# Nikronic/ndr

Hardware: AMD Instinct MI355X
Metric: matrix-free SpMV GVoxel/s (Q1 fp64, 512x512x512); CG-MG iterations/s reported in cg_mg (higher is better)
Workload: dtype f64; 1 GPU; K(rho) u on a 512x512x512 voxel grid, trilinear hexahedra, fp64, seeded U[0,1] densities (SIMP p=3, Emin=1e-4), u ~ N(0,1); parallelism=1 GPU

## Files before the change

### __graft_entry__.py

```python
import os
import subprocess
import sys

ROOT = os.path.dirname(os.path.abspath(__file__))
if ROOT not in sys.path:
    sys.path.insert(0, ROOT)


def build():
    csrc = os.path.join(ROOT, "ndr_amd", "csrc")
    subprocess.check_call(["make", "-C", csrc, "-j4"])
    for src, kernels in (("kernels_q2", ["k_apply_q2_marchILi0"]),
                         ("kernels_l1_merged", ["k_l1_mergedILi0E", "k_l1_mergedILi1E", "k_l1_mergedILi2E", "k_l1_pair_rowsILi0E", "k_l1_pair_rowsILi1E"]),
                         ("kernels_gs_march", ["k_gs_march_mf0ILi%dELi%dELi%dEEE" % (a, f, m) for a in (0, 1) for f in (0, 1) for m in (0, 1)])):
        asm = os.path.join(csrc, src + ".isa.s")
        subprocess.check_call(["/opt/rocm/bin/hipcc", "-O3", "-std=c++17", "-fPIC", "--offload-arch=gfx950", "-ffp-contract=on",
                               "-S", "--cuda-device-only", "-o", asm, os.path.join(csrc, src + ".hip")],
                              stderr=subprocess.DEVNULL)
        for k in kernels:
            subprocess.check_call([sys.executable, os.path.join(ROOT, "tools", "check_sload_pipeline.py"), asm, k])
    from oracle import vfem_oracle
    vfem_oracle.build_lib()
    from ndr_amd import _lib
    lib = _lib.load()
    assert lib.vfem_version() >= 100
    import ndr_amd


def smoke():
    import numpy as np
    sys.path.insert(0, os.path.join(ROOT, "tests"))
    from helpers import BC_CANTILEVER, make_hip, make_oracle, seeded_density
    from oracle import vfem_oracle as vo
    ne, dom = (32, 16, 16), ([0, 0, 0], [2, 1, 1])
    rho = seeded_density(ne, 88, "proxy")
    t = make_hip(ne, dom, BC_CANTILEVER, rho)
    o = make_oracle(ne, dom, BC_CANTILEVER, rho)
    u = np.random.default_rng(0).standard_normal((o.num_nodes, 3))
    err = np.abs(t.applyK(u) - o.apply_k(u)).max() / np.abs(o.apply_k(u)).max()
    assert err < 1e-11, err
    f = o.build_load_vector()
    mg = t.multigridSolver(2)
    ug = mg.preconditionedConjugateGradient(np.zeros_like(f), f, 100, 1e-6, None, 1, 2, True)
    omg = vo.OracleMG(o, 2, nthreads=4)
    uo = omg.pcg(np.zeros_like(f), f, 100, 1e-6, 1, 2, True)
    cg, co = float(np.sum(f * ug)), float(np.sum(f * uo))
    assert abs(cg - co) < 1e-8 * abs(co), (cg, co)
    assert mg.last_iterations == omg.last_iters
    print("smoke ok: apply err %.2e, compliance %.9f (oracle %.9f), %d PCG iterations" % (err, cg, co, mg.last_iterations))


if __name__ == "__main__":
    build()
    if len(sys.argv) > 1 and sys.argv[1] == "smoke":
        smoke()
```

### include/vfem.h

```cpp
#ifndef VFEM_H
#define VFEM_H

#include <stddef.h>
#include <stdint.h>

#ifdef __cplusplus
extern "C" {
#endif

typedef struct vfem_sim vfem_sim;
typedef struct vfem_mg  vfem_mg;
typedef struct vfem_mlp vfem_mlp;
typedef struct vfem_gsim vfem_gsim;
typedef struct vfem_hom_mg vfem_hom_mg;
typedef struct vfem_gmg vfem_gmg;

const char *vfem_last_error(void);
int  vfem_device_count(void);
int  vfem_set_device(int device);
int  vfem_version(void);

enum {
    VFEM_OPT_APPLY_PLANES = 0,
    VFEM_OPT_GS_VARIANT   = 2,
    VFEM_OPT_APPLY_IMPL   = 4,
    VFEM_OPT_Q2_IMPL      = 6,
    VFEM_OPT_DMA_CHUNKS   = 7,
    VFEM_OPT_DMA_STRIP    = 9,
    VFEM_OPT_DMA_LX       = 11,
    VFEM_OPT_GS_PAIR      = 10,
    VFEM_OPT_L1_DIAG      = 12,
    VFEM_OPT_GS_RESIDENT  = 13,
    VFEM_OPT_L1_SPLIT     = 15,
    VFEM_OPT_STENCIL_SPLIT = 18,
    VFEM_OPT_GS_MARCH     = 19,
    VFEM_OPT_GS_MARCH_CHUNKS = 20,
    VFEM_OPT_L1_STORED    = 21,
    VFEM_OPT_L1_MERGED    = 22,
    VFEM_OPT_Q2_GS_IMPL   = 16,
    VFEM_OPT_TRANSFER_AXIS = 17,
    VFEM_OPT_Q2_L1_VIRTUAL = 14
};

int vfem_malloc(void **ptr, size_t bytes);
int vfem_free(void *ptr);
int vfem_copy_h2d(void *dst, const void *src_host, size_t bytes, void *stream);
int vfem_copy_d2h(void *dst_host, const void *src, size_t bytes, void *stream);
int vfem_copy_d2d(void *dst, const void *src, size_t bytes, void *stream);
int vfem_memset(void *dst, int value, size_t bytes, void *stream);
int vfem_stream_sync(void *stream);

int vfem_sim_create(vfem_sim **out, const double bbox_min_host[3], const double bbox_max_host[3],
                    const int64_t nelems_host[3]);
int vfem_sim_destroy(vfem_sim *sim);
int64_t vfem_sim_num_nodes(const vfem_sim *sim);
int64_t vfem_sim_num_elements(const vfem_sim *sim);

int vfem_sim_set_isotropic(vfem_sim *sim, double young, double poisson);
int vfem_sim_set_elasticity_tensor(vfem_sim *sim, const double D_host[36]);
enum {
    VFEM_PATH_MODE_SPACE    = 1,
    VFEM_PATH_GS_RESIDENT   = 2,
    VFEM_PATH_K0_MIRROR     = 4,
    VFEM_PATH_L1_MIRROR     = 8,
    VFEM_PATH_Q2_MODE_SPACE = 16
};
int vfem_sim_tensor_paths(const vfem_sim *sim);
int vfem_sim_set_simp(vfem_sim *sim, double E0, double Emin, double gamma);
int vfem_sim_set_option(vfem_sim *sim, int key, int value);
int vfem_sim_k0(const vfem_sim *sim, double *K0_host);

int vfem_sim_set_dirichlet(vfem_sim *sim, const uint8_t *mask_host, const double *values_host);
int vfem_sim_set_loads(vfem_sim *sim, const double *f, void *stream);
int vfem_sim_build_load_vector(const vfem_sim *sim, double *f, void *stream);

int vfem_sim_set_densities(vfem_sim *sim, const double *rho, void *stream);
int vfem_sim_set_uniform_density(vfem_sim *sim, double rho, void *stream);
int vfem_sim_get_densities(const vfem_sim *sim, double *rho, void *stream);

int vfem_sim_apply_k(const vfem_sim *sim, const double *u, double *out, int variant, void *stream);
int vfem_sim_apply_k_planes(const vfem_sim *sim, const double *u, double *out, int64_t plane_lo, int64_t plane_hi, void *stream);
int vfem_sim_compliance_gradient(const vfem_sim *sim, const double *u, double *g, void *stream);
int vfem_compliance(const vfem_sim *sim, const double *f, const double *u, double *value_host, void *stream);

int vfem_mg_create(vfem_mg **out, vfem_sim *fine, int num_coarsening_levels);
int vfem_mg_destroy(vfem_mg *mg);

typedef struct {
    int64_t nx;
    int64_t elem_extra_lo;
    int64_t elem_extra_hi;
    int64_t xshift;
    int32_t xparity;
} vfem_slab_level;
int vfem_sim_create_padded(vfem_sim **out, const double bbox_min_host[3], const double bbox_max_host[3], const int64_t nelems_host[3],
                           int64_t extra_lo, int64_t extra_hi);
int64_t vfem_sim_num_stored_elements(const vfem_sim *sim);
int vfem_mg_create_slab(vfem_mg **out, vfem_sim *fine_local, int n_levels, const vfem_slab_level *levels_host,
                        const uint8_t *const *masks_host);
int vfem_mg_create_partial(vfem_mg **out, vfem_sim *fine, int num_coarsening_levels, int first_active_level);
int vfem_mg_smooth_colors(vfem_mg *mg, int level, double *u, const double *b, int forward, int first, int count, void *stream);
int vfem_mg_can_smooth_planes(vfem_mg *mg, int level);
int vfem_mg_smooth_group_planes(vfem_mg *mg, int level, double *u, const double *b, int forward, int group, int64_t plane_lo, int64_t plane_hi,
                                void *stream);
int vfem_mg_cycle_from_level(vfem_mg *mg, int level, double *x, const double *b, int num_smoothing_steps, int fmg, void *stream);
int vfem_mg_num_levels(const vfem_mg *mg);
int vfem_mg_level_dims(const vfem_mg *mg, int level, int64_t nelems_host[3]);
int64_t vfem_mg_level_num_nodes(const vfem_mg *mg, int level);
int vfem_mg_level_dirichlet_mask(const vfem_mg *mg, int level, uint8_t *mask_host);
int vfem_mg_set_symmetric_gauss_seidel(vfem_mg *mg, int symmetric);
int vfem_mg_tensor_paths(const vfem_mg *mg);
const double *vfem_mg_field_ptr(const vfem_mg *mg, int which, int level);

int vfem_mg_update_operators(vfem_mg *mg, void *stream);
int vfem_mg_export_level_ke(vfem_mg *mg, int level, int64_t child_first_layer, int64_t count_x, double *ke_out, void *stream);
int vfem_mg_import_level_ke(vfem_mg *mg, int level, const double *ke, void *stream);
int vfem_mg_apply_k(vfem_mg *mg, int level, const double *u, double *out, void *stream);
int vfem_mg_residual(vfem_mg *mg, int level, const double *u, const double *b, double *r, void *stream);
int vfem_mg_smooth(vfem_mg *mg, int level, double *u, const double *b, int forward, void *stream);
int vfem_mg_smooth_sweeps(vfem_mg *mg, int level, double *u, const double *b, int forward, int sweeps, void *stream);
int vfem_mg_zero_dirichlet(vfem_mg *mg, int level, double *u, void *stream);
int vfem_mg_restrict(vfem_mg *mg, int fine_level, const double *fine, double *coarse, void *stream);
int vfem_mg_interpolate(vfem_mg *mg, int fine_level, const double *coarse, double *fine, int accumulate, void *stream);
int vfem_mg_coarsest_solve(vfem_mg *mg, const double *b, double *x, void *stream);
enum { VFEM_COARSEST_AUTO = 0, VFEM_COARSEST_DENSE = 1, VFEM_COARSEST_PLANES = 2 };
int vfem_mg_set_coarsest_solver(vfem_mg *mg, int mode);
int64_t vfem_mg_coarsest_bytes(const vfem_mg *mg);
int vfem_dense_spd_inverse(int64_t n, double *A, void *stream);

int vfem_band_spd_factor(int64_t n, int64_t w, double *band, void *stream);
int vfem_band_spd_solve(int64_t n, int64_t w, const double *factor, double *x, int64_t nrhs, void *stream);
int vfem_sim_direct_solve(vfem_sim *sim, const double *f, double *u, void *stream);
int64_t vfem_sim_direct_factorizations(const vfem_sim *sim);
int64_t vfem_sim_direct_band_bytes(const vfem_sim *sim);
int vfem_gsim_direct_solve(vfem_gsim *sim, const double *f, double *u, void *stream);
int64_t vfem_gsim_direct_factorizations(const vfem_gsim *sim);
int64_t vfem_gsim_direct_band_bytes(const vfem_gsim *sim);

int vfem_mg_solve(vfem_mg *mg, double *x, const double *f, int num_steps, int num_smoothing_steps,
                  int stiffness_updated, int zero_dirichlet, int fmg, void *stream);

typedef void (*vfem_residual_cb)(void *user, int iteration, double residual_norm);
int vfem_mg_pcg(vfem_mg *mg, double *x, const double *b, int max_iter, double tol,
                int mg_iterations, int mg_smoothing_iterations, int fmg,
                vfem_residual_cb residual_cb, void *cb_user,
                int *iterations_out_host, double *relres_out_host, void *stream);

typedef struct {
    int64_t n_planes, plane_nodes;
    int64_t first_owned, last_owned;
    int64_t xoffn;
    int32_t gl, gr;
    double *x, *b, *r;
} vfem_dist_level;
typedef int (*vfem_halo_fn)(void *user, int level, double *field, int left, int right, int phase);
typedef int (*vfem_allreduce_fn)(void *user, double *device_buffer, int64_t n);
int vfem_mg_pcg_slab(vfem_mg *local, vfem_mg *replicated, int first_replicated_level, const vfem_dist_level *levels_host, int rank,
                     int world, double *replicated_x, double *replicated_b, double *x, const double *b, double *work_d, double *work_Ad,
                     double *scalars8, int max_iter, double tol, int mg_iterations, int mg_smoothing_iterations, int full_multigrid,
                     int overlap_sweeps, vfem_halo_fn halo, vfem_allreduce_fn allreduce, void *callback_user,
                     vfem_residual_cb residual_cb, void *residual_user, int *iterations_out, double *relres_out, void *stream);

int vfem_gsim_create(vfem_gsim **out, int dim, int degree, const double *bbox_min_host, const double *bbox_max_host,
                     const int64_t *nelems_host);
int vfem_gsim_create_padded(vfem_gsim **out, int dim, int degree, const double *bbox_min_host, const double *bbox_max_host,
                            const int64_t *nelems_host, int64_t elem_extra_lo, int64_t elem_extra_hi);
int64_t vfem_gsim_num_stored_elements(const vfem_gsim *sim);
int vfem_gsim_destroy(vfem_gsim *sim);
int64_t vfem_gsim_num_nodes(const vfem_gsim *sim);
int64_t vfem_gsim_num_elements(const vfem_gsim *sim);
int vfem_gsim_ke_size(const vfem_gsim *sim);
int vfem_gsim_set_isotropic(vfem_gsim *sim, double young, double poisson);
int vfem_gsim_set_elasticity_tensor(vfem_gsim *sim, const double *D_host, int n);
int vfem_gsim_tensor_paths(const vfem_gsim *sim);
int vfem_gsim_set_simp(vfem_gsim *sim, double E0, double Emin, double gamma);
int vfem_gsim_k0(const vfem_gsim *sim, double *K0_host);
int vfem_gsim_set_dirichlet(vfem_gsim *sim, const uint8_t *mask_host, const double *values_host);
int vfem_gsim_set_densities(vfem_gsim *sim, const double *rho, void *stream);
int vfem_gsim_get_densities(const vfem_gsim *sim, double *rho, void *stream);
int vfem_gsim_set_option(vfem_gsim *sim, int key, int value);
int vfem_gsim_apply_k(const vfem_gsim *sim, const double *u, double *out, void *stream);
int vfem_gsim_compliance_gradient(const vfem_gsim *sim, const double *u, double *g, void *stream);
int vfem_gsim_compliance(const vfem_gsim *sim, const double *f, const double *u, double *value_host, void *stream);
int vfem_gmg_create(vfem_gmg **out, vfem_gsim *fine, int num_coarsening_levels);
int vfem_gmg_create_slab(vfem_gmg **out, vfem_gsim *fine_local, int n_levels, const vfem_slab_level *levels_host,
                         const uint8_t *const *masks_host);
int vfem_gmg_create_partial(vfem_gmg **out, vfem_gsim *fine, int num_coarsening_levels, int first_active_level);
int vfem_gmg_smooth_colors(vfem_gmg *mg, int level, double *u, const double *b, int forward, int first, int count, void *stream);
int vfem_gmg_cycle_from_level(vfem_gmg *mg, int level, double *x, const double *b, int num_smoothing_steps, int fmg, void *stream);
int vfem_gmg_export_level_ke(vfem_gmg *mg, int level, int64_t child_first_layer, int64_t count_x, double *ke_out, void *stream);
int vfem_gmg_import_level_ke(vfem_gmg *mg, int level, const double *ke, void *stream);
int vfem_gmg_destroy(vfem_gmg *mg);
int vfem_gmg_num_levels(const vfem_gmg *mg);
int vfem_gmg_level_dims(const vfem_gmg *mg, int level, int64_t nelems_host[3]);
int64_t vfem_gmg_level_num_nodes(const vfem_gmg *mg, int level);
int vfem_gmg_level_dirichlet_mask(const vfem_gmg *mg, int level, uint8_t *mask_host);
int vfem_gmg_set_symmetric_gauss_seidel(vfem_gmg *mg, int symmetric);
int vfem_gmg_update_operators(vfem_gmg *mg, void *stream);
int vfem_gmg_apply_k(vfem_gmg *mg, int level, const double *u, double *out, void *stream);
int vfem_gmg_residual(vfem_gmg *mg, int level, const double *u, const double *b, double *r, void *stream);
int vfem_gmg_smooth(vfem_gmg *mg, int level, double *u, const double *b, int forward, void *stream);
int vfem_gmg_zero_dirichlet(vfem_gmg *mg, int level, double *u, void *stream);
int vfem_gmg_restrict(vfem_gmg *mg, int fine_level, const double *fine, double *coarse, void *stream);
// ... 79 lines not shown
```

### ndr_amd/_lib.py

```python
import ctypes
import os
from ctypes import POINTER, c_char_p, c_double, c_float, c_int, c_int64, c_size_t, c_void_p

_HERE = os.path.dirname(os.path.abspath(__file__))
LIB_PATH = os.environ.get("VFEM_LIB") or os.path.join(_HERE, "csrc", "libvfem.so")
_lib = None

RESIDUAL_CB = ctypes.CFUNCTYPE(None, c_void_p, c_int, c_double)


class _SL(ctypes.Structure):
    _fields_ = [("nx", c_int64), ("elem_extra_lo", c_int64), ("elem_extra_hi", c_int64), ("xshift", c_int64), ("xparity", ctypes.c_int32)]


class _DL(ctypes.Structure):
    _fields_ = [("n_planes", c_int64), ("plane_nodes", c_int64), ("first_owned", c_int64), ("last_owned", c_int64), ("xoffn", c_int64),
                ("gl", ctypes.c_int32), ("gr", ctypes.c_int32), ("x", c_void_p), ("b", c_void_p), ("r", c_void_p)]

_HOM = [c_int, POINTER(c_int64), POINTER(c_double), POINTER(c_double), POINTER(c_double), c_double, c_void_p]

SIGNATURES = {
    "vfem_last_error": (c_char_p, []),
    "vfem_device_count": (c_int, []),
    "vfem_set_device": (c_int, [c_int]),
    "vfem_version": (c_int, []),
    "vfem_malloc": (c_int, [POINTER(c_void_p), c_size_t]),
    "vfem_free": (c_int, [c_void_p]),
    "vfem_copy_h2d": (c_int, [c_void_p, c_void_p, c_size_t, c_void_p]),
    "vfem_copy_d2h": (c_int, [c_void_p, c_void_p, c_size_t, c_void_p]),
    "vfem_copy_d2d": (c_int, [c_void_p, c_void_p, c_size_t, c_void_p]),
    "vfem_memset": (c_int, [c_void_p, c_int, c_size_t, c_void_p]),
    "vfem_stream_sync": (c_int, [c_void_p]),
    "vfem_sim_create": (c_int, [POINTER(c_void_p), POINTER(c_double), POINTER(c_double), POINTER(c_int64)]),
    "vfem_sim_destroy": (c_int, [c_void_p]),
    "vfem_sim_num_nodes": (c_int64, [c_void_p]),
    "vfem_sim_num_elements": (c_int64, [c_void_p]),
    "vfem_sim_set_isotropic": (c_int, [c_void_p, c_double, c_double]),
    "vfem_sim_set_elasticity_tensor": (c_int, [c_void_p, c_void_p]),
    "vfem_sim_tensor_paths": (c_int, [c_void_p]),
    "vfem_sim_set_simp": (c_int, [c_void_p, c_double, c_double, c_double]),
    "vfem_sim_set_option": (c_int, [c_void_p, c_int, c_int]),
    "vfem_sim_k0": (c_int, [c_void_p, c_void_p]),
    "vfem_sim_set_dirichlet": (c_int, [c_void_p, c_void_p, c_void_p]),
    "vfem_sim_set_loads": (c_int, [c_void_p, c_void_p, c_void_p]),
    "vfem_sim_build_load_vector": (c_int, [c_void_p, c_void_p, c_void_p]),
    "vfem_sim_set_densities": (c_int, [c_void_p, c_void_p, c_void_p]),
    "vfem_sim_set_uniform_density": (c_int, [c_void_p, c_double, c_void_p]),
    "vfem_sim_get_densities": (c_int, [c_void_p, c_void_p, c_void_p]),
    "vfem_sim_apply_k": (c_int, [c_void_p, c_void_p, c_void_p, c_int, c_void_p]),
    "vfem_sim_apply_k_planes": (c_int, [c_void_p, c_void_p, c_void_p, c_int64, c_int64, c_void_p]),
    "vfem_sim_compliance_gradient": (c_int, [c_void_p, c_void_p, c_void_p, c_void_p]),
    "vfem_compliance": (c_int, [c_void_p, c_void_p, c_void_p, POINTER(c_double), c_void_p]),
    "vfem_mg_create": (c_int, [POINTER(c_void_p), c_void_p, c_int]),
    "vfem_mg_destroy": (c_int, [c_void_p]),
    "vfem_sim_create_padded": (c_int, [POINTER(c_void_p), POINTER(c_double), POINTER(c_double), POINTER(c_int64), c_int64, c_int64]),
    "vfem_sim_num_stored_elements": (c_int64, [c_void_p]),
    "vfem_mg_create_slab": (c_int, [POINTER(c_void_p), c_void_p, c_int, c_void_p, POINTER(c_void_p)]),
    "vfem_mg_create_partial": (c_int, [POINTER(c_void_p), c_void_p, c_int, c_int]),
    "vfem_mg_smooth_colors": (c_int, [c_void_p, c_int, c_void_p, c_void_p, c_int, c_int, c_int, c_void_p]),
    "vfem_mg_can_smooth_planes": (c_int, [c_void_p, c_int]),
    "vfem_mg_smooth_group_planes": (c_int, [c_void_p, c_int, c_void_p, c_void_p, c_int, c_int, c_int64, c_int64, c_void_p]),
    "vfem_mg_cycle_from_level": (c_int, [c_void_p, c_int, c_void_p, c_void_p, c_int, c_int, c_void_p]),
    "vfem_mg_num_levels": (c_int, [c_void_p]),
    "vfem_mg_level_dims": (c_int, [c_void_p, c_int, POINTER(c_int64)]),
    "vfem_mg_level_num_nodes": (c_int64, [c_void_p, c_int]),
    "vfem_mg_level_dirichlet_mask": (c_int, [c_void_p, c_int, c_void_p]),
    "vfem_mg_set_symmetric_gauss_seidel": (c_int, [c_void_p, c_int]),
    "vfem_mg_tensor_paths": (c_int, [c_void_p]),
    "vfem_mg_field_ptr": (c_void_p, [c_void_p, c_int, c_int]),
    "vfem_mg_update_operators": (c_int, [c_void_p, c_void_p]),
    "vfem_mg_export_level_ke": (c_int, [c_void_p, c_int, c_int64, c_int64, c_void_p, c_void_p]),
    "vfem_mg_import_level_ke": (c_int, [c_void_p, c_int, c_void_p, c_void_p]),
    "vfem_mg_apply_k": (c_int, [c_void_p, c_int, c_void_p, c_void_p, c_void_p]),
    "vfem_mg_residual": (c_int, [c_void_p, c_int, c_void_p, c_void_p, c_void_p, c_void_p]),
    "vfem_mg_smooth": (c_int, [c_void_p, c_int, c_void_p, c_void_p, c_int, c_void_p]),
    "vfem_mg_smooth_sweeps": (c_int, [c_void_p, c_int, c_void_p, c_void_p, c_int, c_int, c_void_p]),
    "vfem_mg_zero_dirichlet": (c_int, [c_void_p, c_int, c_void_p, c_void_p]),
    "vfem_mg_restrict": (c_int, [c_void_p, c_int, c_void_p, c_void_p, c_void_p]),
    "vfem_mg_interpolate": (c_int, [c_void_p, c_int, c_void_p, c_void_p, c_int, c_void_p]),
    "vfem_mg_coarsest_solve": (c_int, [c_void_p, c_void_p, c_void_p, c_void_p]),
    "vfem_mg_set_coarsest_solver": (c_int, [c_void_p, c_int]),
    "vfem_mg_coarsest_bytes": (c_int64, [c_void_p]),
    "vfem_dense_spd_inverse": (c_int, [c_int64, c_void_p, c_void_p]),
    "vfem_band_spd_factor": (c_int, [c_int64, c_int64, c_void_p, c_void_p]),
    "vfem_band_spd_solve": (c_int, [c_int64, c_int64, c_void_p, c_void_p, c_int64, c_void_p]),
    "vfem_sim_direct_solve": (c_int, [c_void_p, c_void_p, c_void_p, c_void_p]),
    "vfem_sim_direct_factorizations": (c_int64, [c_void_p]),
    "vfem_sim_direct_band_bytes": (c_int64, [c_void_p]),
    "vfem_gsim_direct_solve": (c_int, [c_void_p, c_void_p, c_void_p, c_void_p]),
    "vfem_gsim_direct_factorizations": (c_int64, [c_void_p]),
    "vfem_gsim_direct_band_bytes": (c_int64, [c_void_p]),
    "vfem_mg_solve": (c_int, [c_void_p, c_void_p, c_void_p, c_int, c_int, c_int, c_int, c_int, c_void_p]),
    "vfem_mg_pcg": (c_int, [c_void_p, c_void_p, c_void_p, c_int, c_double, c_int, c_int, c_int,
                            RESIDUAL_CB, c_void_p, POINTER(c_int), POINTER(c_double), c_void_p]),
    "vfem_mlp_forward_grid_range": (c_int, [c_void_p, POINTER(c_int64), POINTER(c_double), POINTER(c_double), c_int64, c_int64,
                                            c_void_p, c_void_p, c_void_p]),
    "vfem_mlp_forward_grid_range_f32": (c_int, [c_void_p, POINTER(c_int64), POINTER(c_double), POINTER(c_double), c_int64, c_int64,
                                                c_void_p, c_void_p, c_void_p]),
    "vfem_mlp_backward": (c_int, [c_void_p, c_void_p, c_int64, c_void_p, c_float, c_void_p, c_void_p, c_void_p, c_void_p, c_void_p, c_void_p]),
    "vfem_mlp_backward_grid": (c_int, [c_void_p, POINTER(c_int64), POINTER(c_double), POINTER(c_double), c_void_p, c_float,
                                       c_void_p, c_void_p, c_void_p, c_void_p, c_void_p, c_void_p]),
    "vfem_mlp_backward_grid_range": (c_int, [c_void_p, POINTER(c_int64), POINTER(c_double), POINTER(c_double), c_int64, c_int64, c_void_p,
                                             c_float, c_void_p, c_void_p, c_void_p, c_void_p, c_void_p, c_void_p]),
    "vfem_adam_step": (c_int, [c_int64, c_void_p, c_void_p, c_void_p, c_void_p, c_float, c_float, c_float, c_float, c_int, c_void_p]),
    "vfem_gsim_create": (c_int, [POINTER(c_void_p), c_int, c_int, POINTER(c_double), POINTER(c_double), POINTER(c_int64)]),
    "vfem_gsim_create_padded": (c_int, [POINTER(c_void_p), c_int, c_int, POINTER(c_double), POINTER(c_double), POINTER(c_int64),
                                        c_int64, c_int64]),
    "vfem_gsim_num_stored_elements": (c_int64, [c_void_p]),
    "vfem_gmg_create_slab": (c_int, [POINTER(c_void_p), c_void_p, c_int, c_void_p, POINTER(c_void_p)]),
    "vfem_gmg_create_partial": (c_int, [POINTER(c_void_p), c_void_p, c_int, c_int]),
    "vfem_gmg_smooth_colors": (c_int, [c_void_p, c_int, c_void_p, c_void_p, c_int, c_int, c_int, c_void_p]),
    "vfem_gmg_cycle_from_level": (c_int, [c_void_p, c_int, c_void_p, c_void_p, c_int, c_int, c_void_p]),
    "vfem_gmg_export_level_ke": (c_int, [c_void_p, c_int, c_int64, c_int64, c_void_p, c_void_p]),
    "vfem_gmg_import_level_ke": (c_int, [c_void_p, c_int, c_void_p, c_void_p]),
    "vfem_gsim_destroy": (c_int, [c_void_p]),
    "vfem_gsim_num_nodes": (c_int64, [c_void_p]),
    "vfem_gsim_num_elements": (c_int64, [c_void_p]),
    "vfem_gsim_ke_size": (c_int, [c_void_p]),
    "vfem_gsim_set_isotropic": (c_int, [c_void_p, c_double, c_double]),
    "vfem_gsim_set_elasticity_tensor": (c_int, [c_void_p, c_void_p, c_int]),
    "vfem_gsim_tensor_paths": (c_int, [c_void_p]),
    "vfem_gsim_set_simp": (c_int, [c_void_p, c_double, c_double, c_double]),
    "vfem_gsim_k0": (c_int, [c_void_p, c_void_p]),
    "vfem_gsim_set_dirichlet": (c_int, [c_void_p, c_void_p, c_void_p]),
    "vfem_gsim_set_densities": (c_int, [c_void_p, c_void_p, c_void_p]),
    "vfem_gsim_get_densities": (c_int, [c_void_p, c_void_p, c_void_p]),
    "vfem_gsim_set_option": (c_int, [c_void_p, c_int, c_int]),
    "vfem_gsim_apply_k": (c_int, [c_void_p, c_void_p, c_void_p, c_void_p]),
    "vfem_gsim_compliance_gradient": (c_int, [c_void_p, c_void_p, c_void_p, c_void_p]),
    "vfem_gsim_compliance": (c_int, [c_void_p, c_void_p, c_void_p, POINTER(c_double), c_void_p]),
    "vfem_gmg_create": (c_int, [POINTER(c_void_p), c_void_p, c_int]),
    "vfem_gmg_destroy": (c_int, [c_void_p]),
    "vfem_gmg_num_levels": (c_int, [c_void_p]),
    "vfem_gmg_level_dims": (c_int, [c_void_p, c_int, POINTER(c_int64)]),
    "vfem_gmg_level_num_nodes": (c_int64, [c_void_p, c_int]),
    "vfem_gmg_level_dirichlet_mask": (c_int, [c_void_p, c_int, c_void_p]),
    "vfem_gmg_set_symmetric_gauss_seidel": (c_int, [c_void_p, c_int]),
    "vfem_gmg_update_operators": (c_int, [c_void_p, c_void_p]),
    "vfem_gmg_apply_k": (c_int, [c_void_p, c_int, c_void_p, c_void_p, c_void_p]),
    "vfem_gmg_residual": (c_int, [c_void_p, c_int, c_void_p, c_void_p, c_void_p, c_void_p]),
    "vfem_gmg_smooth": (c_int, [c_void_p, c_int, c_void_p, c_void_p, c_int, c_void_p]),
    "vfem_gmg_zero_dirichlet": (c_int, [c_void_p, c_int, c_void_p, c_void_p]),
    "vfem_gmg_restrict": (c_int, [c_void_p, c_int, c_void_p, c_void_p, c_void_p]),
    "vfem_gmg_interpolate": (c_int, [c_void_p, c_int, c_void_p, c_void_p, c_int, c_void_p]),
    "vfem_gmg_solve": (c_int, [c_void_p, c_void_p, c_void_p, c_int, c_int, c_int, c_int, c_int, c_void_p]),
    "vfem_gmg_pcg": (c_int, [c_void_p, c_void_p, c_void_p, c_int, c_double, c_int, c_int, c_int, RESIDUAL_CB, c_void_p,
                             POINTER(c_int), POINTER(c_double), c_void_p]),
    "vfem_box_filter": (c_int, [POINTER(c_int64), c_int, c_void_p, c_void_p, c_int, c_void_p]),
    "vfem_box_filter_slab": (c_int, [POINTER(c_int64), c_int64, c_int64, c_int64, c_int64, c_int, c_void_p, c_void_p, c_int,
                                     c_void_p]),
    "vfem_projection": (c_int, [c_int64, c_double, c_void_p, c_void_p, c_void_p]),
    "vfem_projection_backprop": (c_int, [c_int64, c_double, c_void_p, c_void_p, c_void_p, c_void_p]),
    "vfem_oc_candidate": (c_int, [c_int64, c_void_p, c_void_p, c_void_p, c_double, c_double, c_void_p, c_void_p]),
    "vfem_mean": (c_int, [c_int64, c_void_p, POINTER(c_double), c_void_p]),
    "vfem_langelaar_apply": (c_int, [POINTER(c_int64), c_double, c_double, c_double, c_void_p, c_void_p, c_void_p, c_void_p]),
    "vfem_langelaar_backprop": (c_int, [POINTER(c_int64), c_double, c_double, c_double, c_void_p, c_void_p, c_void_p, c_void_p,
                                        c_void_p, c_void_p, c_void_p]),
    "vfem_mg_pcg_slab": (c_int, [c_void_p, c_void_p, c_int, c_void_p, c_int, c_int, c_void_p, c_void_p, c_void_p, c_void_p, c_void_p, c_void_p,
                                 c_void_p, c_int, c_double, c_int, c_int, c_int, c_int, c_void_p, c_void_p, c_void_p, RESIDUAL_CB, c_void_p,
# ... 66 lines not shown
```

### ndr_amd/csrc/coef_rows.h

```cpp
#pragma once
#include "device_utils.h"
#include "l1_merged_core.h"

namespace vfem {

template <int OFF>
__device__ __forceinline__ void srow_issue(const double *p, d8_t &a, double &b) {
    asm volatile("s_load_dwordx16 %0, %2, %3\n\ts_load_dwordx2 %1, %2, %4" : "=&s"(a), "=&s"(b) : "s"(p), "n"(OFF), "n"(OFF + 64));
}
__device__ __forceinline__ void srow_wait(d8_t &a, double &b) { asm volatile("s_waitcnt lgkmcnt(0)" : "+s"(a), "+s"(b)); }
__device__ __forceinline__ void srow_wait(d8_t &a, double &b, double &tie) { asm volatile("s_waitcnt lgkmcnt(0)" : "+s"(a), "+s"(b), "+v"(tie)); }

template <bool MID> constexpr int row_pos(int w) { return MID ? (w == 3 ? 0 : w == 2 ? 1 : w == 0 ? 2 : 3) : 7 - w; }
template <bool MID> constexpr int row_kind(int pos) { return MID ? (pos == 0 ? 3 : pos == 1 ? 2 : pos == 2 ? 0 : 1) : 7 - pos; }

template <int NROWS, class SEQ>
struct RowPipe {
    const double *tab;
    d8_t a0, a1;
    double b0, b1;
    __device__ __forceinline__ void prime() { srow_issue<SEQ::at(0)>(tab, a0, b0); }
    template <int R>
    __device__ __forceinline__ void take(double c[9], double &tie) {
        static_assert(R >= 0 && R < NROWS, "row outside the sequence");
        if constexpr (R % 2 == 0) {
            srow_wait(a0, b0, tie);
            if constexpr (R + 1 < NROWS) srow_issue<SEQ::at(R + 1 < NROWS ? R + 1 : 0)>(tab, a1, b1);
            c[0] = a0[0]; c[1] = a0[1]; c[2] = a0[2]; c[3] = a0[3]; c[4] = a0[4]; c[5] = a0[5]; c[6] = a0[6]; c[7] = a0[7]; c[8] = b0;
        } else {
            srow_wait(a1, b1, tie);
            if constexpr (R + 1 < NROWS) srow_issue<SEQ::at(R + 1 < NROWS ? R + 1 : 0)>(tab, a0, b0);
            c[0] = a1[0]; c[1] = a1[1]; c[2] = a1[2]; c[3] = a1[3]; c[4] = a1[4]; c[5] = a1[5]; c[6] = a1[6]; c[7] = a1[7]; c[8] = b1;
        }
    }
    template <int R>
    __device__ __forceinline__ void take(double c[9]) {
        static_assert(R >= 0 && R < NROWS, "row outside the sequence");
        if constexpr (R % 2 == 0) {
            srow_wait(a0, b0);
            if constexpr (R + 1 < NROWS) srow_issue<SEQ::at(R + 1 < NROWS ? R + 1 : 0)>(tab, a1, b1);
            c[0] = a0[0]; c[1] = a0[1]; c[2] = a0[2]; c[3] = a0[3]; c[4] = a0[4]; c[5] = a0[5]; c[6] = a0[6]; c[7] = a0[7]; c[8] = b0;
        } else {
            srow_wait(a1, b1);
            if constexpr (R + 1 < NROWS) srow_issue<SEQ::at(R + 1 < NROWS ? R + 1 : 0)>(tab, a0, b0);
            c[0] = a1[0]; c[1] = a1[1]; c[2] = a1[2]; c[3] = a1[3]; c[4] = a1[4]; c[5] = a1[5]; c[6] = a1[6]; c[7] = a1[7]; c[8] = b1;
        }
    }
};

template <bool MID>
struct L1PartRows { static constexpr int at(int r) { return ((r / 4) * 8 + row_kind<MID>(r % 4)) * l1m::TAB_ROW * 8; } };
template <bool MID>
struct DevCoef {
    RowPipe<32, L1PartRows<MID>> pipe;
    __device__ __forceinline__ explicit DevCoef(const double *tab) : pipe{tab} {}
    __device__ __forceinline__ void prime() { pipe.prime(); }
    template <int G, int W>
    __device__ __forceinline__ void get(double c[9]) { pipe.template take<G * 4 + row_pos<MID>(W)>(c); }
};

struct L0NodeRows {
    static constexpr int at(int r) { return (r < 4 ? 7 - r : r < 8 ? row_kind<true>(r - 4) : 7 - (r - 8)) * l1m::TAB_ROW * 8; }
};
template <bool MID, int BASE, class Hook>
struct L0Coef {
    RowPipe<12, L0NodeRows> &pipe;
    double &tie;
    Hook after_first;
    template <int G, int W>
    __device__ __forceinline__ void get(double c[9]) {
        static_assert(G == 0, "level 0 has one class");
        pipe.template take<BASE + row_pos<MID>(W)>(c, tie);
        after_first(std::integral_constant<int, row_pos<MID>(W)>{});
    }
};
template <bool MID, int BASE, class Hook>
__device__ __forceinline__ L0Coef<MID, BASE, Hook> l0_coef(RowPipe<12, L0NodeRows> &pipe, double &tie, Hook hook) { return L0Coef<MID, BASE, Hook>{pipe, tie, hook}; }


}
```

### ndr_amd/csrc/generic.hip

```cpp
#include "mg_cycle.h"
#include "device_utils.h"
#include "q2_modes.h"
#include "gs_colors.h"

#include <algorithm>
#include <cmath>
#include <cstring>
#include <memory>

namespace vfem {

struct GDims {
    int N, p;
    int ne[3], nn[3];
    int npe, ke;
    long long nnodes, nelems;
};

static GDims make_gdims(int N, int p, const long long *ne) {
    GDims d{};
    d.N = N; d.p = p; d.npe = 1; d.nnodes = 1; d.nelems = 1;
    for (int a = 0; a < 3; ++a) {
        d.ne[a] = a < N ? (int) ne[a] : 1;
        d.nn[a] = a < N ? p * d.ne[a] + 1 : 1;
// ... 841 lines not shown
        throw Error("the element matrices of the first active level have not been imported (vfem_gmg_import_level_ke)");
    const int l_first = mg->first_active > 0 ? mg->first_active + 1 : 1;
    const int l_last = mg->slab ? mg->L - 1 : mg->L;
    mg->l1_virtual = N == 3 && sim->d.p == 2 && mg->first_active == 0 && mg->external_ke_level != 0 && mg->L >= 2 &&
                     (sim->q2_l1_virtual == 1 ||
                      (sim->q2_l1_virtual == 2 && (double) stored_dims(mg, 1).nelems * 81 * 81 * sizeof(double) > 1.5e9));
    if (mg->l1_virtual) mg->lv[1].Ke.release();
    for (int l = l_first; l <= l_last; ++l) {
        GLevel &lv = mg->lv[l];
        const size_t kk = (size_t) lv.d.ke * lv.d.ke;
        const GDims cd = stored_dims(mg, l), fd = stored_dims(mg, l - 1);
        if (fd.ne[0] != 2 * cd.ne[0]) throw Error("stored element layers of consecutive levels must halve exactly");
        if (mg->l1_virtual && l == 1) continue;
        lv.Ke.alloc((size_t) cd.nelems * kk);
        if (mg->l1_virtual && l == 2) { coarsen_through_virtual_level1(mg, 0, cd.ne[0], lv.Ke.p, s); continue; }
        const bool from_moduli = l == 1 && mg->external_ke_level != 0;
        g_coarsen(mg, fd, cd, from_moduli, from_moduli ? sim->E.p : mg->lv[l - 1].Ke.p, lv.Ke.p, s);
    }
    if (mg->slab) { mg->operators_valid = true; return; }
    GLevel &cl = mg->lv[mg->L];
    const GDims &d = cl.d;
    const long long n = (long long) N * d.nnodes;
    if (mg->L > 0) mg->coarsest.refuse_if_too_large(n, nullptr);
    else if (n > DENSE_COARSEST_MAX_DOFS) {
        mg->coarsest.release();
        mg->operators_valid = true;
        return;
    }
    const size_t kk = (size_t) d.ke * d.ke;
    std::vector<double> Ke((size_t) d.nelems * kk);
    if (mg->L == 0 && mg->external_ke_level != 0) {
        std::vector<double> E((size_t) d.nelems);
        VFEM_HIP(hipMemcpyAsync(E.data(), sim->E_local(), E.size() * sizeof(double), hipMemcpyDeviceToHost, s));
        VFEM_HIP(hipStreamSynchronize(s));
        for (long long e = 0; e < d.nelems; ++e)
            for (size_t q = 0; q < kk; ++q) Ke[e * kk + q] = E[e] * sim->K0[q];
    } else {
        VFEM_HIP(hipMemcpyAsync(Ke.data(), cl.Ke_local(), Ke.size() * sizeof(double), hipMemcpyDeviceToHost, s));
        VFEM_HIP(hipStreamSynchronize(s));
    }
    std::vector<double> A((size_t) n * n, 0.0);
    const int q1 = d.p + 1;
    std::vector<long long> dofs(d.ke);
    for (long long e = 0; e < d.nelems; ++e) {
        int eb[3] = {0, 0, 0};
        { long long m = e; for (int a = N - 1; a >= 0; --a) { eb[a] = d.p * (int) (m % d.ne[a]); m /= d.ne[a]; } }
        for (int ln = 0; ln < d.npe; ++ln) {
            int m = ln, g[3] = {0, 0, 0};
            for (int a = N - 1; a >= 0; --a) { g[a] = eb[a] + m % q1; m /= q1; }
            long long node = g[0];
            for (int a = 1; a < N; ++a) node = node * d.nn[a] + g[a];
            for (int c = 0; c < N; ++c) dofs[N * ln + c] = N * node + c;
        }
        for (int i = 0; i < d.ke; ++i)
            for (int j = 0; j < d.ke; ++j) A[(size_t) dofs[i] * n + dofs[j]] += Ke[e * kk + (size_t) i * d.ke + j];
    }
    for (long long r = 0; r < n; ++r)
        if ((cl.hmask[r / N] >> (r % N)) & 1) {
            for (long long c = 0; c < n; ++c) { A[(size_t) r * n + c] = 0.0; A[(size_t) c * n + r] = 0.0; }
            A[(size_t) r * n + r] = 1.0;
        }
    double *Adev = mg->coarsest.dense_matrix(n, s);
    VFEM_HIP(hipStreamSynchronize(s));
    VFEM_HIP(hipMemcpy(Adev, A.data(), A.size() * sizeof(double), hipMemcpyHostToDevice));
    mg->coarsest.factor_dense(N, cl.mask.p, s);
    VFEM_HIP(hipStreamSynchronize(s));
    mg->operators_valid = true;
}

namespace {
struct GenericOps {
    vfem_gmg *mg;
    hipStream_t s;
    GLevel &lv(int l) const { return mg->lv[l]; }

    int last_level() const { return mg->L; }
    void last_level_cycle(bool) { mg->coarsest.solve(b(mg->L), x(mg->L), s); }
    bool symmetric() const { return mg->symmetric_gs; }
    double *x(int l) const { return lv(l).x.p; }
    double *b(int l) const { return lv(l).b.p; }
    void enforce_dirichlet(int l, bool residual_system, bool) {
        g_dirichlet(lv(l).d, lv(l).mask.p, (l == 0 && !residual_system) ? mg->fine->dvals.p : nullptr, x(l), s);
    }
    void smooth(int l, int forward, int n) { for (int i = 0; i < n; ++i) gmg_smooth(mg, l, x(l), b(l), forward, s); }
    void residual(int l) { gmg_apply(mg, l, x(l), b(l), 1, lv(l).r.p, s); }
    void restrict_residual(int l) { gmg_restrict(mg, l, lv(l).r.p, b(l + 1), s); lv(l + 1).x.zero(s); }
    void restrict_rhs(int l) { gmg_restrict(mg, l, b(l), b(l + 1), s); }
    void prolong_correction(int l) { gmg_prolong(mg, l, x(l + 1), x(l), 1, s); }
    bool prolong_start(int l, bool) { gmg_prolong(mg, l, x(l + 1), x(l), 0, s); return false; }

    long long n_dofs() const { return (long long) lv(0).d.N * lv(0).d.nnodes; }
    mg_cycle::CgWork cg() const { return {n_dofs(), mg->pd.p, mg->pAd.p, mg->scal.p, s}; }
    double *s_vector(bool preconditioned) const { return preconditioned ? x(0) : mg->ps.p; }
    void dot(const double *a, const double *b, double *out) { launch_dot(n_dofs(), a, b, mg->scratch.p, out, s); }
    void initial_residual(const double *x, const double *b, double *r) { gmg_apply(mg, 0, x, b, 1, r, s); }
    void shift_and_dot_rs(const double *r, double *sv, double *sc) {
        g_dirichlet(lv(0).d, lv(0).mask.p, nullptr, sv, s);
        launch_shift_scalar(sc, s);
        dot(r, sv, sc + 0);
    }
    void apply_dot(const double *d, double *Ad, double *out) { gmg_apply(mg, 0, d, nullptr, 2, Ad, s); dot(d, Ad, out); }
    void step_dot(double *x, double *r, const double *d, const double *Ad, double *sc) { launch_pcg_step(n_dofs(), x, r, d, Ad, sc, s); dot(r, r, sc + 3); }
};
}

extern "C" {

int vfem_gsim_create_padded(vfem_gsim **out, int dim, int degree, const double *bbmin, const double *bbmax, const int64_t *ne,
                            int64_t ex_lo, int64_t ex_hi) {
    VFEM_TRY
    if (dim != 2 && dim != 3) throw Error("dimension must be 2 or 3");
    if (degree != 1 && degree != 2) throw Error("No template instantiation matching degreesPerDimension!");
    long long n[3] = {1, 1, 1};
    for (int a = 0; a < dim; ++a) {
        if (ne[a] < 1 || ne[a] > 4096) throw Error("elements per dimension must be in [1, 4096]");
        n[a] = ne[a];
    }
    std::unique_ptr<vfem_gsim> sim(new vfem_gsim);
    sim->d = make_gdims(dim, degree, n);
    for (int a = 0; a < dim; ++a) {
        sim->h[a] = (bbmax[a] - bbmin[a]) / (double) ne[a];
        if (!(sim->h[a] > 0)) throw Error("empty domain bounding box");
    }
    sim->update_k0();
    if (ex_lo < 0 || ex_hi < 0 || ((ex_lo || ex_hi) && dim != 3)) throw Error("element padding needs a 3-D grid and non-negative layer counts");
    sim->ex_lo = ex_lo; sim->ex_hi = ex_hi;
    sim->rho.alloc((size_t) sim->stored_elems()); sim->rho.zero(nullptr);
    sim->E.alloc((size_t) sim->stored_elems());
    sim->update_E(nullptr);
    sim->hmask.assign((size_t) sim->d.nnodes, 0);
    sim->dmask.alloc((size_t) sim->d.nnodes); sim->dmask.zero(nullptr);
    sim->dvals.alloc((size_t) sim->d.nnodes * dim); sim->dvals.zero(nullptr);
    VFEM_HIP(hipDeviceSynchronize());
    *out = sim.release();
    VFEM_CATCH
}
int vfem_gsim_create(vfem_gsim **out, int dim, int degree, const double *bbmin, const double *bbmax, const int64_t *ne) {
    return vfem_gsim_create_padded(out, dim, degree, bbmin, bbmax, ne, 0, 0);
}
int vfem_gsim_destroy(vfem_gsim *sim) { VFEM_TRY delete sim; VFEM_CATCH }
int64_t vfem_gsim_num_stored_elements(const vfem_gsim *sim) { return sim->stored_elems(); }
int64_t vfem_gsim_num_nodes(const vfem_gsim *sim) { return sim->d.nnodes; }
int64_t vfem_gsim_num_elements(const vfem_gsim *sim) { return sim->d.nelems; }
int vfem_gsim_ke_size(const vfem_gsim *sim) { return sim->d.ke; }
int vfem_gsim_set_isotropic(vfem_gsim *sim, double young, double poisson) {
    VFEM_TRY
    sim->lambda = sim->d.N == 2 ? poisson * young / (1.0 - poisson * poisson)
                                : poisson * young / ((1.0 + poisson) * (1.0 - 2.0 * poisson));
    sim->mu = young / (2.0 + 2.0 * poisson);
    sim->general_tensor = false;
    sim->update_k0();
    ++sim->operator_version;
    VFEM_CATCH
}
int vfem_gsim_set_elasticity_tensor(vfem_gsim *sim, const double *D, int n) {
    VFEM_TRY
    if (n != (sim->d.N == 3 ? 6 : 3)) throw Error("the flattened tensor of a " + std::to_string(sim->d.N) + "-D simulator is " +
                                                  (sim->d.N == 3 ? "6 x 6" : "3 x 3"));
    check_flattened_tensor(D, n);
    for (int i = 0; i < n; ++i)
        for (int j = 0; j < n; ++j) sim->D[i * n + j] = 0.5 * (D[i * n + j] + D[j * n + i]);
    sim->general_tensor = true;
    sim->update_k0();
    ++sim->operator_version;
    VFEM_CATCH
}
int vfem_gsim_tensor_paths(const vfem_gsim *sim) { return sim->q2_fast ? VFEM_PATH_Q2_MODE_SPACE : 0; }
// ... 327 lines not shown
```

### ndr_amd/csrc/gs_colors.h

```cpp
#pragma once
#include <type_traits>

namespace vfem {

struct GsColor { int start[3], inc[3], cnt[3]; };

template <class F>
void for_each_gs_color(int N, int p, const int nn[3], int forward, int first, int count, F &&f) {
    int ncol = 1;
    for (int a = 0; a < N; ++a) ncol *= p + 1;
    for (int i = first; i < first + count && i < ncol; ++i) {
        int m = forward ? i : ncol - 1 - i;
        GsColor col{{0, 0, 0}, {1, 1, 1}, {1, 1, 1}};
        bool empty = false;
        for (int a = N - 1; a >= 0; --a) {
            const int la = m % (p + 1); m /= p + 1;
            col.start[a] = la;
            col.inc[a] = (1 + (la == 0 || la == p ? 1 : 0)) * p;
            col.cnt[a] = la > nn[a] - 1 ? 0 : (nn[a] - 1 - la) / col.inc[a] + 1;
            empty = empty || col.cnt[a] == 0;
        }
        if (!empty) f(col);
    }
}

template <class F>
void with_bits3(int bits, F &&f) {
    auto pick = [](bool bit, auto &&g) { if (!bit) g(std::integral_constant<int, 0>{}); else g(std::integral_constant<int, 1>{}); };
    pick(bits & 4, [&](auto x) { pick(bits & 2, [&](auto y) { pick(bits & 1, [&](auto z) { f(x, y, z); }); }); });
}
inline int parity_bits(const GsColor &c) { return 4 * (c.start[0] & 1) + 2 * (c.start[1] & 1) + (c.start[2] & 1); }

}
```

### ndr_amd/csrc/hom_mg.hip

```cpp
#include "hom_mg.h"
#include "mg_cycle.h"

#include <memory>

using namespace vfem;

struct HomMgLevel {
    HomGrid g;
    DevBuf<double> A;
    DevBuf<double> Dinv;
    DevBuf<double> x, b, r;
};

struct vfem_hom_mg {
    HomCall call;
    std::vector<HomMgLevel> lv;
    DevBuf<double> Minv0, r0;
    DevBuf<uint8_t> pin;
    CoarsestSolver coarsest;
    int N() const { return call.p.N; }
    int L() const { return (int) lv.size() - 1; }
    HomBlocks blocks(int l) const { return l == 0 ? HomBlocks{call.p.stencil, call.p.E} : HomBlocks{lv[l].A.p, nullptr}; }
    HomDinv dinv(int l) const {
        const long long nn = (long long) N() * N();
        return l == 0 ? HomDinv{Minv0.p, nn, 1} : HomDinv{lv[l].Dinv.p, 1, lv[l].g.pn};
    }
    size_t vec(int l) const { return (size_t) lv[l].g.S * lv[l].g.pn * lv[l].g.N; }
    long long bytes() const {
        size_t n = call.tables.n + Minv0.n + r0.n;
        for (const HomMgLevel &v : lv) n += v.A.n + v.Dinv.n + v.x.n + v.b.n + v.r.n;
        return (long long) (n * sizeof(double)) + coarsest.bytes() + (long long) pin.n;
    }
};

namespace {

std::string dims_text(const HomGrid &g) {
    std::string t = std::to_string(g.n[0]);
    for (int d = 1; d < g.N; ++d) t += "x" + std::to_string(g.n[d]);
    return t;
}

bool can_colour(const HomGrid &g) {
    for (int d = 0; d < g.N; ++d)
        if (g.n[d] % 2) return false;
    return true;
}

void check_level(const vfem_hom_mg *h, int l, const char *who, int last) {
    if (!h) throw Error(std::string(who) + ": null handle");
    if (l < 0 || l > last) throw Error(std::string(who) + ": level " + std::to_string(l) + " out of range");
}

void sweep(vfem_hom_mg *h, int l, double *x, const double *b, int forward, hipStream_t s) {
    const int nc = 1 << h->N();
    for (int k = 0; k < nc; ++k)
        launch_hom_mg_sweep_colour(h->lv[l].g, h->blocks(l), h->dinv(l), forward ? k : nc - 1 - k, x, b, s);
}

struct HomOps {
    vfem_hom_mg *h;
    const double *B;
    double *X;
    hipStream_t s;
    int last_level() const { return h->L(); }
    bool symmetric() const { return true; }
    const HomGrid &g(int l) const { return h->lv[l].g; }
    double *x(int l) const { return l == 0 ? X : h->lv[l].x.p; }
    const double *b(int l) const { return l == 0 ? B : h->lv[l].b.p; }
    double *r(int l) const { return l == 0 ? h->r0.p : h->lv[l].r.p; }
    void last_level_cycle(bool) {
        if (h->coarsest.held != CoarsestSolver::DENSE) throw Error("the coarsest level holds no dense inverse");
        launch_hom_mg_gemv(g(h->L()), h->coarsest.Ainv.p, b(h->L()), x(h->L()), s);
    }
    void enforce_dirichlet(int, bool, bool) {}
    void smooth(int l, int forward, int n) { for (int k = 0; k < n; ++k) sweep(h, l, x(l), b(l), forward, s); }
    void residual(int l) { launch_hom_mg_residual(g(l), h->blocks(l), x(l), b(l), r(l), s); }
    void restrict_residual(int l) {
        launch_hom_mg_restrict(g(l), g(l + 1), r(l), h->lv[l + 1].b.p, s);
        if (l + 1 < h->L()) VFEM_HIP(hipMemsetAsync(x(l + 1), 0, h->vec(l + 1) * sizeof(double), s));
    }
    void prolong_correction(int l) { launch_hom_mg_prolong_add(g(l), g(l + 1), x(l + 1), x(l), s); }
};

void cycle_from_zero(vfem_hom_mg *h, const double *B, double *X, int smoothing, hipStream_t s) {
    if (h->L() > 0) VFEM_HIP(hipMemsetAsync(X, 0, h->vec(0) * sizeof(double), s));
    HomOps o{h, B, X, s};
    mg_cycle::vcycle(o, 0, smoothing, true);
}

void check_smoothing(int smoothing, const char *who) {
    if (smoothing < 1 || smoothing > 16) throw Error(std::string(who) + ": smoothing must be in [1, 16]");
}

}

extern "C" {

int vfem_hom_mg_create(vfem_hom_mg **out, int dim, const int64_t *nelems_host, const double *K0_host, const double *L_host,
                       const double *D_host, double vol, const double *E, int max_coarsenings, void *stream) {
    VFEM_TRY
    if (!out) throw Error("vfem_hom_mg_create: null argument");
    *out = nullptr;
    hipStream_t s = S(stream);
    std::unique_ptr<vfem_hom_mg> h(new vfem_hom_mg);
    hom_setup(h->call, "vfem_hom_mg_create", dim, nelems_host, K0_host, L_host, D_host, vol, E, s);
    const HomProblem &p = h->call.p;
    const int N = p.N;
    HomGrid g = p;
    std::string sizes = dims_text(g);
    h->lv.emplace_back();
    h->lv.back().g = g;
    while (max_coarsenings < 0 || (int) h->lv.size() - 1 < max_coarsenings) {
        bool ok = true;
        for (int d = 0; d < N; ++d) ok = ok && g.n[d] % 2 == 0 && g.n[d] >= 4;
        if (!ok) break;
        g.pn = 1;
        for (int d = 0; d < N; ++d) { g.n[d] /= 2; g.pn *= g.n[d]; }
        h->lv.emplace_back();
        h->lv.back().g = g;
        sizes += ", " + dims_text(g);
    }
    const int L = h->L();
    const long long nc = (long long) g.pn * N;
    if (nc > DENSE_COARSEST_MAX_DOFS)
        throw Error("vfem_hom_mg_create: the coarsest level of the hierarchy " + sizes + " has " + std::to_string(nc) +
                    " dofs, above the limit of " + std::to_string(DENSE_COARSEST_MAX_DOFS) +
                    " of the dense coarsest-level solve (a level is coarsened only while every extent is even and at least 4)");
    const int noff = N == 2 ? 9 : 27;
    if (L > 0) {
        h->Minv0.alloc((size_t) p.pn * N * N);
        h->r0.alloc(h->vec(0));
        launch_hom_jacobi(p, h->Minv0.p, s);
    }
    for (int l = 1; l <= L; ++l) {
        HomMgLevel &v = h->lv[l];
        v.A.alloc((size_t) noff * N * N * v.g.pn);
        v.Dinv.alloc((size_t) N * N * v.g.pn);
        v.x.alloc(h->vec(l));
        v.b.alloc(h->vec(l));
        if (l < L) v.r.alloc(h->vec(l));
        launch_hom_mg_galerkin(h->lv[l - 1].g, v.g, h->blocks(l - 1), v.A.p, s);
        launch_hom_mg_dinv(v.g, v.A.p, v.Dinv.p, s);
    }
    std::vector<uint8_t> mask((size_t) g.pn, 0);
    mask[0] = (uint8_t) ((1 << N) - 1);
    h->pin.alloc(mask.size());
    VFEM_HIP(hipMemcpyAsync(h->pin.p, mask.data(), mask.size(), hipMemcpyHostToDevice, s));
    double *M = h->coarsest.dense_matrix(nc, s);
    launch_hom_mg_dense(g, h->blocks(L), M, s);
    h->coarsest.factor_dense(N, h->pin.p, s);
    VFEM_HIP(hipStreamSynchronize(s));
    h->coarsest.work = DenseWork();
    *out = h.release();
    VFEM_CATCH
}

int vfem_hom_mg_destroy(vfem_hom_mg *h) {
    VFEM_TRY
// ... 81 lines not shown
```

### ndr_amd/csrc/kernels_l1_merged.hip

```cpp
#include "vfem_internal.h"
#include "device_utils.h"
#include "l1_merged_core.h"
#include "coef_rows.h"


namespace vfem {

namespace {

typedef unsigned int u4_t __attribute__((ext_vector_type(4)));
typedef unsigned int u2_t __attribute__((ext_vector_type(2)));

constexpr unsigned OOB = 0x7ffffff0u;

__device__ __forceinline__ __amdgpu_buffer_rsrc_t plane_rsrc(const double *base, long long plane_doubles, int plane, int planes) {
    const bool ok = plane >= 0 && plane < planes;
    const double *p = base + (long long) (ok ? plane : 0) * plane_doubles;
    return __builtin_amdgcn_make_buffer_rsrc(const_cast<double *>(p), 0, ok ? (int) (plane_doubles * 8) : 0, 0x00020000);
}

__device__ __forceinline__ void load_nodes(__amdgpu_buffer_rsrc_t r, const Dims &d, int j, int k, double (&un)[3][9]) {
#pragma unroll
    for (int oy = -1; oy <= 1; ++oy)
#pragma unroll
        for (int oz = -1; oz <= 1; ++oz) {
            const int jj = j + oy, kk = k + oz;
            const bool ok = jj >= 0 && jj < d.NY && kk >= 0 && kk < d.NZ;
            const unsigned off = ok ? (unsigned) (jj * d.NZ + kk) * 24u : OOB;
#ifdef L1M_NOLOAD
            const u4_t v = {off, 0x3ff00000u, off, 0x3ff00000u}; const u2_t w = {off, 0x3ff00000u}; (void) r;
#else
            const u4_t v = __builtin_amdgcn_raw_buffer_load_b128(r, off, 0, 0);
            const u2_t w = __builtin_amdgcn_raw_buffer_load_b64(r, off + 16, 0, 0);
#endif
            un[oy + 1][3 * (oz + 1) + 0] = mkd(v.x, v.y);
            un[oy + 1][3 * (oz + 1) + 1] = mkd(v.z, v.w);
            un[oy + 1][3 * (oz + 1) + 2] = mkd(w.x, w.y);
        }
}
typedef double d2_t __attribute__((ext_vector_type(2)));
struct ModuliLds {
    double (*sE)[16][64];
    int lane;
    template <int G>
    __device__ __forceinline__ void window(int px, double (&a)[2][2]) const {
        constexpr int gy = (G >> 1) & 1, gz = G & 1;
#pragma unroll
        for (int dy = 0; dy < 2; ++dy)
#pragma unroll
            for (int dz = 0; dz < 2; ++dz) a[dy][dz] = sE[px][4 * l1m::class_index(dy, gy) + l1m::class_index(dz, gz)][lane];
    }
};
__device__ __forceinline__ void stage_moduli(__amdgpu_buffer_rsrc_t r, const unsigned (&off)[4][2], double (*plane)[64], int lane) {
    u4_t v[4][2];
#pragma unroll
    for (int py = 0; py < 4; ++py)
#pragma unroll
        for (int h = 0; h < 2; ++h) {
#ifdef L1M_NOLOAD
            v[py][h] = u4_t{off[py][h], 0x3ff00000u, off[py][h] + 1, 0x3ff00000u}; (void) r;
#else
            v[py][h] = __builtin_amdgcn_raw_buffer_load_b128(r, off[py][h], 0, 0);
#endif
        }
#pragma unroll
    for (int py = 0; py < 4; ++py)
#pragma unroll
        for (int h = 0; h < 2; ++h) {
            plane[4 * py + 2 * h][lane] = mkd(v[py][h].x, v[py][h].y);
            plane[4 * py + 2 * h + 1][lane] = mkd(v[py][h].z, v[py][h].w);
        }
}

template <int SIDE, int G>
__device__ __forceinline__ void side_classes(const ModuliLds &m, const double (&un)[3][9], DevCoef<false> &cf, double S[3]) {
#ifdef L1M_NOCOMP
    if constexpr (G == 0) { for (auto &r : un) for (double v : r) S[1] += v; }
#else
    double a[2][2];
    m.template window<G>(SIDE ? 2 + ((G >> 2) & 1) : 1 - ((G >> 2) & 1), a);
    l1m::side_class<SIDE, G>(a, un, cf, S);
#endif
    if constexpr (G + 1 < 8) side_classes<SIDE, G + 1>(m, un, cf, S);
}
template <int G>
__device__ __forceinline__ void mid_classes(const ModuliLds &m, const double (&un)[3][9], DevCoef<true> &cf, double S[3], double M[6]) {
#ifdef L1M_NOCOMP
    if constexpr (G == 0) { for (auto &r : un) for (double v : r) S[1] += v; M[0] = M[3] = M[5] = 1.0; }
#else
    double a0[2][2], a1[2][2];
    m.template window<G>(1 - ((G >> 2) & 1), a0);
    m.template window<G>(2 + ((G >> 2) & 1), a1);
    l1m::mid_class<G>(a0, a1, un, cf, S, M);
#endif
    if constexpr (G + 1 < 8) mid_classes<G + 1>(m, un, cf, S, M);
}

template <int MODE>
__device__ __forceinline__ void node_group(const Dims &d, const double *__restrict__ tab, const double *__restrict__ E, const double *u,
                                           const double *__restrict__ b, const uint8_t *__restrict__ mask, double *out, int i, int j, int k,
                                           bool live, int role, int lane, int forward, double (&part)[2][3][64], double (*sE)[16][64]) {
    double un[3][9];
    load_nodes(plane_rsrc(u, 3LL * d.NY * d.NZ, i + role - 1, d.NX), d, j, k, un);
    const long long n = ((long long) i * d.NY + j) * d.NZ + k;
    double bn[3] = {0.0, 0.0, 0.0};
    uint8_t mk8 = 0;
    if (MODE != 1 && role == 1) {
#pragma unroll
        for (int c = 0; c < 3; ++c) bn[c] = b[3 * n + c];
        mk8 = mask ? mask[n] : 0;
    }
    if (role != 1) {
        unsigned eoff[4][2];
        const int nzf = 2 * d.nz;
#pragma unroll
        for (int py = 0; py < 4; ++py)
#pragma unroll
            for (int h = 0; h < 2; ++h) {
                const bool ok = (py < 2 ? j >= 1 : j <= d.ny - 1) && (h == 0 ? k >= 1 : k <= d.nz - 1);
                eoff[py][h] = ok ? (unsigned) ((2 * j - 2 + py) * nzf + 2 * k - 2 + 2 * h) * 8u : OOB;
            }
        const long long eplane = 4LL * d.ny * d.nz;
        const int p0 = role == 0 ? 0 : 2;
        const bool ok = role == 0 ? i > 0 : i < d.NX - 1;
        stage_moduli(plane_rsrc(E, eplane, ok ? 2 * i - 2 + p0 : -1, 2 * d.nx), eoff, sE[p0], lane);
        stage_moduli(plane_rsrc(E, eplane, ok ? 2 * i - 1 + p0 : -1, 2 * d.nx), eoff, sE[p0 + 1], lane);
    }
    __syncthreads();
    const ModuliLds m{sE, lane};
    double S[3] = {0.0, 0.0, 0.0}, M6[6] = {0.0, 0.0, 0.0, 0.0, 0.0, 0.0};
    if (role == 1) {
        DevCoef<true> cf(tab);
#ifndef L1M_NOCOMP
        cf.prime();
#endif
        mid_classes<0>(m, un, cf, S, M6);
    } else if (role == 0) {
        DevCoef<false> cf(tab);
#ifndef L1M_NOCOMP
        cf.prime();
#endif
        side_classes<0, 0>(m, un, cf, S);
    } else {
        DevCoef<false> cf(tab);
#ifndef L1M_NOCOMP
        cf.prime();
#endif
        side_classes<1, 0>(m, un, cf, S);
    }
    if (role != 1) {
#pragma unroll
        for (int c = 0; c < 3; ++c) part[role >> 1][c][lane] = S[c];
    }
    __syncthreads();
    if (role != 1 || !live) return;
#pragma unroll
    for (int c = 0; c < 3; ++c) S[c] = (part[0][c][lane] + S[c]) + part[1][c][lane];
    const double uc[3] = {un[1][3], un[1][4], un[1][5]};
    const double M[9] = {M6[0], M6[1], M6[2], M6[1], M6[3], M6[4], M6[2], M6[4], M6[5]};
    if (MODE == 1) {
#pragma unroll
        for (int c = 0; c < 3; ++c) out[3 * n + c] = S[c] + (M[3 * c] * uc[0] + M[3 * c + 1] * uc[1] + M[3 * c + 2] * uc[2]);
        return;
    }
    double bms[3];
#pragma unroll
    for (int c = 0; c < 3; ++c) bms[c] = bn[c] - (S[c] + (M[3 * c] * uc[0] + M[3 * c + 1] * uc[1] + M[3 * c + 2] * uc[2]));
    if (MODE == 2) {
#pragma unroll
        for (int c = 0; c < 3; ++c) out[3 * n + c] = ((mk8 >> c) & 1) ? 0.0 : bms[c];
        return;
    }
    double ud[3];
    gs_solve(bms, M, mk8, forward != 0, ud);
#pragma unroll
    for (int c = 0; c < 3; ++c) out[3 * n + c] = uc[c] + ud[c];
}

#ifndef L1M_WAVES
#define L1M_WAVES 3
#endif
template <int MODE>
__global__ void __launch_bounds__(192, L1M_WAVES) k_l1_merged(Dims d, const double *__restrict__ tab, const double *__restrict__ E,
                                                   const double *u, const double *__restrict__ b, const uint8_t *__restrict__ mask,
                                                   double *out, int cx, int cy, int cz, int forward, int ka, int kskip) {
    __shared__ double part[2][3][64];
    __shared__ double sE[4][16][64];
    const int lane = threadIdx.x, role = __builtin_amdgcn_readfirstlane(threadIdx.y);
    int i, j, k;
    bool live;
    if (MODE == 0) {
        const int cnty = (d.NY - 1 - cy) / 2 + 1, cntz = (d.NZ - 1 - cz) / 2 + 1 - kskip;
        const int q = blockIdx.x * 64 + lane;
        live = q < cnty * cntz;
        const int qq = live ? q : cnty * cntz - 1, jq = qq / cntz, r = qq - jq * cntz;
        k = 2 * (r < ka ? r : r + kskip) + cz; j = 2 * jq + cy; i = 2 * blockIdx.z + cx;
    } else {
        const int q = blockIdx.x * 64 + lane;
        live = q < d.NY * d.NZ;
        const int qq = live ? q : d.NY * d.NZ - 1;
        j = qq / d.NZ; k = qq - j * d.NZ; i = blockIdx.z;
    }
    node_group<MODE>(d, tab, E, u, b, mask, out, i, j, k, live, role, lane, forward, part, sE);
}

template <int FZ>
__global__ void __launch_bounds__(192, L1M_WAVES) k_l1_pair_rows(Dims d, const double *__restrict__ tab, const double *__restrict__ E, double *u,
                                                                 const double *__restrict__ b, const uint8_t *__restrict__ mask, int cx, int cy,
                                                                 int nseg) {
    __shared__ double part[2][3][64];
    __shared__ double sE[4][16][64];
    const int lane = threadIdx.x, role = __builtin_amdgcn_readfirstlane(threadIdx.y);
    const int i = 2 * blockIdx.z + cx, j = 2 * blockIdx.y + cy;
#pragma unroll 1
    for (int s = 0; s < 2 * nseg; ++s) {
        const int k = (FZ == 0 ? 2 : 1) + 128 * (s >> 1) + 2 * lane - (s & 1);
        const bool live = k >= 0 && k < d.NZ;
        node_group<0>(d, tab, E, u, b, mask, u, i, j, live ? k : FZ, live, role, lane, FZ == 0, part, sE);
        __builtin_amdgcn_fence(__ATOMIC_RELEASE, "workgroup");
        __syncthreads();
        __builtin_amdgcn_fence(__ATOMIC_ACQUIRE, "workgroup");
    }
}

}

void build_l1_merged_table(const double *cK0_0, double *tab ) { l1m::build_table(cK0_0, tab); }

bool l1_merged_usable(const Dims &d) {
    return d.nx >= 1 && d.ny >= 1 && d.nz >= 1 && 24LL * d.NY * d.NZ < 0x7f000000LL && 32LL * d.ny * d.nz < 0x7f000000LL;
}

void launch_l1_merged_sweep(const Dims &d, const double *tab, const double *E, double *u, const double *b, const uint8_t *mask,
                            int forward, int xparity, int first, int count, hipStream_t s, int pair) {
    for (int ci = first; ci < first + count; ++ci) {
        const int lni = forward ? ci : 7 - ci;
        const int cx = ((lni >> 2) & 1) ^ (xparity & 1), cy = (lni >> 1) & 1, cz = lni & 1;
        if (cx > d.NX - 1 || cy > d.NY - 1 || cz > d.NZ - 1) continue;
        const int cntx = (d.NX - 1 - cx) / 2 + 1, cnty = (d.NY - 1 - cy) / 2 + 1, cntz = (d.NZ - 1 - cz) / 2 + 1;
        const int fz = cz, ka = fz == 0 ? 1 : 0, nseg = (cntz - ka) / 64;
        if (pair && ci % 2 == 0 && ci + 1 < first + count && nseg >= 1) {
            const int walked = 64 * nseg, cntb = (d.NZ - 1 - (1 - fz)) / 2 + 1;
            if (cntz > walked)
                k_l1_merged<0><<<dim3((cnty * (cntz - walked) + 63) / 64, 1, cntx), dim3(64, 3, 1), 0, s>>>(d, tab, E, u, b, mask, u, cx, cy, fz, forward, ka, walked);
            if (fz == 0) k_l1_pair_rows<0><<<dim3(1, cnty, cntx), dim3(64, 3, 1), 0, s>>>(d, tab, E, u, b, mask, cx, cy, nseg);
            else         k_l1_pair_rows<1><<<dim3(1, cnty, cntx), dim3(64, 3, 1), 0, s>>>(d, tab, E, u, b, mask, cx, cy, nseg);
            if (cntb > walked)
                k_l1_merged<0><<<dim3((cnty * (cntb - walked) + 63) / 64, 1, cntx), dim3(64, 3, 1), 0, s>>>(d, tab, E, u, b, mask, u, cx, cy, 1 - fz, forward, 0, walked);
            ++ci;
            continue;
        }
        k_l1_merged<0><<<dim3((cnty * cntz + 63) / 64, 1, cntx), dim3(64, 3, 1), 0, s>>>(d, tab, E, u, b, mask, u, cx, cy, cz, forward, 0, 0);
    }
    VFEM_HIP(hipGetLastError());
}

void launch_l1_merged_apply(const Dims &d, const double *tab, const double *E, const double *u, const double *b, const uint8_t *mask,
                            int res, double *out, hipStream_t s) {
    const dim3 grd((d.NY * d.NZ + 63) / 64, 1, d.NX), blk(64, 3, 1);
    if (res) k_l1_merged<2><<<grd, blk, 0, s>>>(d, tab, E, u, b, mask, out, 0, 0, 0, 0, 0, 0);
    else     k_l1_merged<1><<<grd, blk, 0, s>>>(d, tab, E, u, b, mask, out, 0, 0, 0, 0, 0, 0);
    VFEM_HIP(hipGetLastError());
}

}
```

### ndr_amd/csrc/kernels_mg.hip

```cpp
#include "vfem_internal.h"
#include "device_utils.h"
#include "gs_coef.h"


#include <algorithm>
#include <cmath>
#include <type_traits>
#include <utility>

namespace vfem {

__device__ __forceinline__ long long nidx(const Dims &d, int i, int j, int k) {
    return ((long long) i * d.NY + j) * d.NZ + k;
}
__device__ __forceinline__ long long eidx(const Dims &d, int i, int j, int k) {
    return ((long long) i * d.ny + j) * d.nz + k;
}

template <int KIND, bool WITH_M>
__device__ __forceinline__ void mf_node(const Dims &d, const double *__restrict__ K, const double *__restrict__ E,
                                        const double *__restrict__ u, int i, int j, int k, double S[3], double M[9]) {
    S[0] = S[1] = S[2] = 0.0;
    if (WITH_M) {
#pragma unroll
        for (int q = 0; q < 9; ++q) M[q] = 0.0;
    }
    const long long sx = (long long) d.NY * d.NZ, sy = d.NZ;
#pragma unroll
    for (int slot = 0; slot < 8; ++slot) {
        const int di = (slot >> 2) & 1, dj = (slot >> 1) & 1, dk = slot & 1;
        const int ex = i - 1 + di, ey = j - 1 + dj, ez = k - 1 + dk;
        if (ex < 0 || ex >= d.nx || ey < 0 || ey >= d.ny || ez < 0 || ez >= d.nz) continue;
        const int li = ((1 - di) * 2 + (1 - dj)) * 2 + (1 - dk);
        const long long base = nidx(d, ex, ey, ez);
        double ue[24];
#pragma unroll
        for (int m = 0; m < 8; ++m) {
            const long long nm = base + ((m >> 2) & 1) * sx + ((m >> 1) & 1) * sy + (m & 1);
            ue[3 * m + 0] = u[3 * nm + 0];
            ue[3 * m + 1] = u[3 * nm + 1];
            ue[3 * m + 2] = u[3 * nm + 2];
        }
        if (KIND == 0) {
            const double Ee = E[eidx(d, ex, ey, ez)];
#pragma unroll
            for (int r = 0; r < 3; ++r) {
                const double *row = K + (3 * li + r) * 24;
                double acc = 0.0;
#pragma unroll
                for (int c = 0; c < 24; ++c) acc = fma(row[c], ue[c], acc);
                S[r] = fma(Ee, acc, S[r]);
                if (WITH_M) {
#pragma unroll
                    for (int c = 0; c < 3; ++c) M[r * 3 + c] = fma(Ee, row[3 * li + c], M[r * 3 + c]);
                }
            }
        } else {
            const long long nyf = 2LL * d.ny, nzf = 2LL * d.nz;
            for (int f = 0; f < 8; ++f) {
                const int fx = (f >> 2) & 1, fy = (f >> 1) & 1, fz = f & 1;
                const double Ef = E[((2LL * ex + fx) * nyf + (2LL * ey + fy)) * nzf + (2LL * ez + fz)];
                const double *Kf = K + f * 576;
#pragma unroll
                for (int r = 0; r < 3; ++r) {
                    const double *row = Kf + (3 * li + r) * 24;
                    double acc = 0.0;
#pragma unroll
                    for (int c = 0; c < 24; ++c) acc = fma(row[c], ue[c], acc);
                    S[r] = fma(Ef, acc, S[r]);
                    if (WITH_M) {
#pragma unroll
                        for (int c = 0; c < 3; ++c) M[r * 3 + c] = fma(Ef, row[3 * li + c], M[r * 3 + c]);
                    }
                }
            }
        }
    }
}

template <int KIND, bool RES>
__global__ void __launch_bounds__(256) k_apply_gather(Dims d, const double *__restrict__ K, const double *__restrict__ E,
                                                      const double *__restrict__ u, const double *__restrict__ b,
                                                      const uint8_t *__restrict__ mask, double *__restrict__ out) {
    const int q = blockIdx.x * 256 + threadIdx.y * 64 + threadIdx.x;
    if (q >= d.NY * d.NZ) return;
// ... 618 lines not shown
#pragma unroll
            for (int q = 0; q < 9; ++q) A[q] = a[(long long) q * scnt];
#pragma unroll
            for (int r = 0; r < 3; ++r) S[r] += A[3 * r] * u0 + A[3 * r + 1] * u1 + A[3 * r + 2] * u2;
        }
        return;
    }
    static_for<27>([&](auto nbc) {
        constexpr int nb = decltype(nbc)::value, di = nb / 9 - 1, dj = (nb / 3) % 3 - 1, dk = nb % 3 - 1;
        int ii = i + di, jj = j + dj, kk = k + dk;
        if (di < 0) ii = ii < 0 ? 0 : ii;
        if (di > 0) ii = ii > d.NX - 1 ? d.NX - 1 : ii;
        if (dj < 0) jj = jj < 0 ? 0 : jj;
        if (dj > 0) jj = jj > d.NY - 1 ? d.NY - 1 : jj;
        if (dk < 0) kk = kk < 0 ? 0 : kk;
        if (dk > 0) kk = kk > d.NZ - 1 ? d.NZ - 1 : kk;
        const long long m = nidx(d, ii, jj, kk);
        const double u0 = u[3 * m], u1 = u[3 * m + 1], u2 = u[3 * m + 2];
        const double *a = St + sbase + (long long) nb * 9 * scnt;
        double A[9];
#pragma unroll
        for (int q = 0; q < 9; ++q) A[q] = a[(long long) q * scnt];
#pragma unroll
        for (int r = 0; r < 3; ++r) S[r] += A[3 * r] * u0 + A[3 * r + 1] * u1 + A[3 * r + 2] * u2;
        if (WITH_M && nb == 13) {
#pragma unroll
            for (int q = 0; q < 9; ++q) M[q] = A[q];
            if (uself) { uself[0] = u0; uself[1] = u1; uself[2] = u2; }
        }
    });
}

template <bool RES>
__global__ void __launch_bounds__(256) k_apply_stencil(Dims d, const double *__restrict__ St, const double *__restrict__ u,
                                                       const double *__restrict__ b, const uint8_t *__restrict__ mask,
                                                       double *__restrict__ out) {
    const int q = blockIdx.x * 256 + threadIdx.y * 64 + threadIdx.x;
    if (q >= d.NY * d.NZ) return;
    const int j = q / d.NZ, k = q - j * d.NZ, i = blockIdx.z;
    const long long n = nidx(d, i, j, k);
    double S[3], M[9];
    stencil_node<false>(d, St, u, i, j, k, n, S, M);
    if (RES) {
        const uint8_t m = mask ? mask[n] : 0;
#pragma unroll
        for (int c = 0; c < 3; ++c) out[3 * n + c] = ((m >> c) & 1) ? 0.0 : b[3 * n + c] - S[c];
    } else {
#pragma unroll
        for (int c = 0; c < 3; ++c) out[3 * n + c] = S[c];
    }
}

void launch_apply_stencil(const Dims &d, const double *S, const double *u, const double *b, const uint8_t *mask,
                          int res, double *out, hipStream_t s) {
    dim3 blk(64, 4, 1), grd((d.NY * d.NZ + 255) / 256, 1, d.NX);
    if (res) k_apply_stencil<true><<<grd, blk, 0, s>>>(d, S, u, b, mask, out);
    else     k_apply_stencil<false><<<grd, blk, 0, s>>>(d, S, u, b, mask, out);
    VFEM_HIP(hipGetLastError());
}

__global__ void __launch_bounds__(256) k_gs_color_stencil(Dims d, const double *__restrict__ St, double *__restrict__ u,
                                                          const double *__restrict__ b, const uint8_t *__restrict__ mask,
                                                          int cx, int cy, int cz, int forward) {
    const int cntx = (d.NX - 1 - cx) / 2 + 1, cnty = (d.NY - 1 - cy) / 2 + 1, cntz = (d.NZ - 1 - cz) / 2 + 1;
    const long long q = (long long) blockIdx.x * 256 + threadIdx.y * 64 + threadIdx.x;
    if (q >= (long long) cntx * cnty * cntz) return;
    const int iq = (int) (q / ((long long) cnty * cntz)), rem = (int) (q - (long long) iq * cnty * cntz), jq = rem / cntz;
    const int i = 2 * iq + cx, j = 2 * jq + cy, k = 2 * (rem - jq * cntz) + cz;
    const long long n = nidx(d, i, j, k);
    double bv[3], uself[3];
#pragma unroll
    for (int c = 0; c < 3; ++c) bv[c] = b[3 * n + c];
    const uint8_t mk = mask[n];
    double S[3], M[9];
    stencil_node<true>(d, St, u, i, j, k, n, S, M, uself);
    double bms[3], ud[3];
#pragma unroll
    for (int c = 0; c < 3; ++c) bms[c] = bv[c] - S[c];
    gs_solve(bms, M, mk, forward != 0, ud);
#pragma unroll
    for (int c = 0; c < 3; ++c) u[3 * n + c] = uself[c] + ud[c];
}

template <int W>
__device__ __forceinline__ void stencil_plane(const Dims &d, const double *__restrict__ St, const double *__restrict__ u, int i, int j, int k,
                                              long long sbase, long long scnt, double S[3], double M[9], double uself[3]) {
    static_for<9>([&](auto tc) {
        constexpr int nb = 9 * W + decltype(tc)::value, di = W - 1, dj = (nb / 3) % 3 - 1, dk = nb % 3 - 1;
        int ii = i + di, jj = j + dj, kk = k + dk;
        if (di < 0) ii = ii < 0 ? 0 : ii;
        if (di > 0) ii = ii > d.NX - 1 ? d.NX - 1 : ii;
        if (dj < 0) jj = jj < 0 ? 0 : jj;
        if (dj > 0) jj = jj > d.NY - 1 ? d.NY - 1 : jj;
        if (dk < 0) kk = kk < 0 ? 0 : kk;
        if (dk > 0) kk = kk > d.NZ - 1 ? d.NZ - 1 : kk;
        const long long m = nidx(d, ii, jj, kk);
        const double u0 = u[3 * m], u1 = u[3 * m + 1], u2 = u[3 * m + 2];
        const double *a = St + sbase + (long long) nb * 9 * scnt;
        double A[9];
#pragma unroll
        for (int q = 0; q < 9; ++q) A[q] = a[(long long) q * scnt];
#pragma unroll
        for (int r = 0; r < 3; ++r) S[r] += A[3 * r] * u0 + A[3 * r + 1] * u1 + A[3 * r + 2] * u2;
        if (nb == 13) {
#pragma unroll
            for (int q = 0; q < 9; ++q) M[q] = A[q];
            uself[0] = u0; uself[1] = u1; uself[2] = u2;
        }
    });
}
__global__ void __launch_bounds__(192) k_gs_color_stencil_split(Dims d, const double *__restrict__ St, double *__restrict__ u,
                                                                const double *__restrict__ b, const uint8_t *__restrict__ mask,
                                                                int cx, int cy, int cz, int forward) {
    __shared__ double part[2][3][64];
    const int lane = threadIdx.x, w = __builtin_amdgcn_readfirstlane(threadIdx.y);
    const int cntx = (d.NX - 1 - cx) / 2 + 1, cnty = (d.NY - 1 - cy) / 2 + 1, cntz = (d.NZ - 1 - cz) / 2 + 1;
    const unsigned q0 = blockIdx.x * 64u + (unsigned) lane, total = (unsigned) cntx * (unsigned) cnty * (unsigned) cntz;
    const bool live = q0 < total;
    const unsigned q = live ? q0 : total - 1u, pc = (unsigned) cnty * (unsigned) cntz;
    const int iq = (int) (q / pc), rem = (int) (q - (unsigned) iq * pc), jq = rem / cntz;
    const int i = 2 * iq + cx, j = 2 * jq + cy, k = 2 * (rem - jq * cntz) + cz;
    const long long n = nidx(d, i, j, k);
    long long sbase, scnt;
    cm_index(d, i, j, k, sbase, scnt);
    double S[3] = {0.0, 0.0, 0.0}, M[9], uself[3] = {0.0, 0.0, 0.0};
    if (w == 0) stencil_plane<0>(d, St, u, i, j, k, sbase, scnt, S, M, uself);
    else if (w == 1) stencil_plane<1>(d, St, u, i, j, k, sbase, scnt, S, M, uself);
    else stencil_plane<2>(d, St, u, i, j, k, sbase, scnt, S, M, uself);
    if (w != 1) {
#pragma unroll
        for (int c = 0; c < 3; ++c) part[w >> 1][c][lane] = S[c];
    }
    __syncthreads();
    if (w != 1 || !live) return;
#pragma unroll
    for (int c = 0; c < 3; ++c) S[c] = (part[0][c][lane] + S[c]) + part[1][c][lane];
    double bms[3], ud[3];
#pragma unroll
    for (int c = 0; c < 3; ++c) bms[c] = b[3 * n + c] - S[c];
    gs_solve(bms, M, mask[n], forward != 0, ud);
#pragma unroll
    for (int c = 0; c < 3; ++c) u[3 * n + c] = uself[c] + ud[c];
}

__global__ void __launch_bounds__(256) k_stencil_node_major(long long ntiles, const double *__restrict__ St, double *__restrict__ Sn) {
    const long long t = (long long) blockIdx.x * 256 + threadIdx.x;
    if (t >= ntiles * 243 * 64) return;
    const long long tile = t / (243 * 64);
    const int e = (int) ((t / 64) % 243), lane = (int) (t % 64);
    Sn[(tile * 64 + lane) * 243 + e] = St[t];
}
void launch_stencil_node_major(const Dims &d, const double *St, double *Sn, hipStream_t s) {
    const long long ntiles = stencil_storage_doubles(d) / (243 * 64);
    k_stencil_node_major<<<dim3((unsigned) ((ntiles * 243 * 64 + 255) / 256)), dim3(256), 0, s>>>(ntiles, St, Sn);
    VFEM_HIP(hipGetLastError());
}

__global__ void __launch_bounds__(256) k_gs_color_stencil_wave(Dims d, const double *__restrict__ Sn, double *__restrict__ u,
                                                               const double *__restrict__ b, const uint8_t *__restrict__ mask,
                                                               int cx, int cy, int cz, int forward) {
    const int cnty = (d.NY - 1 - cy) / 2 + 1, cntz = (d.NZ - 1 - cz) / 2 + 1;
    const int kq = blockIdx.x * 4 + threadIdx.y, jq = blockIdx.y, iq = blockIdx.z;
    if (kq >= cntz) return;
    const int lane = threadIdx.x;
    const int i = 2 * iq + cx, j = 2 * jq + cy, k = 2 * kq + cz;
    const long long n = nidx(d, i, j, k);
    const double *row = Sn + (cm_colour_start(d, cx, cy, cz) + ((long long) iq * cnty + jq) * cntz + kq) * 243;
    const double bn0 = b[3 * n], bn1 = b[3 * n + 1], bn2 = b[3 * n + 2], un0 = u[3 * n], un1 = u[3 * n + 1], un2 = u[3 * n + 2];
    const uint8_t fixed = mask[n];
    double p0 = 0.0, p1 = 0.0, p2 = 0.0, centre = 0.0;
#pragma unroll
    for (int sidx = 0; sidx < 4; ++sidx) {
        const int e = lane + 64 * sidx;
        if (e < 243) {
            const int nb = e / 9, qq = e - 9 * nb, r = qq / 3, c = qq - 3 * r;
            const int ii = min(max(i + nb / 9 - 1, 0), d.NX - 1), jj = min(max(j + (nb / 3) % 3 - 1, 0), d.NY - 1), kk = min(max(k + nb % 3 - 1, 0), d.NZ - 1);
            const double a = row[e];
            const double t = a * u[3 * nidx(d, ii, jj, kk) + c];
            p0 += r == 0 ? t : 0.0; p1 += r == 1 ? t : 0.0; p2 += r == 2 ? t : 0.0;
            if (sidx == 1) centre = a;
        }
    }
#pragma unroll
    for (int o = 32; o > 0; o >>= 1) { p0 += __shfl_xor(p0, o); p1 += __shfl_xor(p1, o); p2 += __shfl_xor(p2, o); }
    double M[9];
#pragma unroll
    for (int qq = 0; qq < 9; ++qq) M[qq] = __shfl(centre, 53 + qq);
    if (lane != 0) return;
    double bms[3] = {bn0 - p0, bn1 - p1, bn2 - p2}, ud[3];
    gs_solve(bms, M, fixed, forward != 0, ud);
    u[3 * n] = un0 + ud[0]; u[3 * n + 1] = un1 + ud[1]; u[3 * n + 2] = un2 + ud[2];
}

void launch_gs_sweep_stencil(const Dims &d, const double *S, double *u, const double *b, const uint8_t *mask,
                             int forward, int xparity, int first, int count, hipStream_t s, const double *Sn, int stencil_split) {
    for (int ci = first; ci < first + count; ++ci) {
        const int lni = forward ? ci : 7 - ci;
        const int cx = ((lni >> 2) & 1) ^ (xparity & 1), cy = (lni >> 1) & 1, cz = lni & 1;
        if (cx > d.NX - 1) continue;
        const int cntx = (d.NX - 1 - cx) / 2 + 1, cnty = (d.NY - 1 - cy) / 2 + 1, cntz = (d.NZ - 1 - cz) / 2 + 1;
        const long long cnt = (long long) cntx * cnty * cntz;
        dim3 blk(64, 4, 1), grd((unsigned) ((cnt + 255) / 256), 1, 1);
        if (Sn) k_gs_color_stencil_wave<<<dim3((unsigned) ((cntz + 3) / 4), (unsigned) cnty, (unsigned) cntx), blk, 0, s>>>(d, Sn, u, b, mask, cx, cy, cz, forward);
        else if (stencil_split && cnt < (1LL << 31)) k_gs_color_stencil_split<<<dim3((unsigned) ((cnt + 63) / 64)), dim3(64, 3, 1), 0, s>>>(d, S, u, b, mask, cx, cy, cz, forward);
        else k_gs_color_stencil<<<grd, blk, 0, s>>>(d, S, u, b, mask, cx, cy, cz, forward);
    }
    VFEM_HIP(hipGetLastError());
}

__global__ void __launch_bounds__(256) k_restrict(Dims c, int FX, int shift, const double *__restrict__ fine,
                                                  double *__restrict__ coarse, double *__restrict__ zeroed) {
    const int k = blockIdx.x * 64 + threadIdx.x, j = blockIdx.y * 4 + threadIdx.y, i = 2 * blockIdx.z;
    if (j >= c.NY) return;
    const int FY = 2 * c.ny + 1, FZ = 2 * c.nz + 1;
    const bool live = k < c.NZ, lo = live && k > 0, hi = live && 2 * k + 1 < FZ, first = threadIdx.x == 0;
    const bool second = i + 1 < c.NX;
    double a[3] = {0.0, 0.0, 0.0}, a2[3] = {0.0, 0.0, 0.0};
#pragma unroll
    for (int pl = 0; pl < 5; ++pl) {
        const int fi = 2 * i + shift - 1 + pl;
        if (fi < 0 || fi >= FX || (pl > 2 && !second)) continue;
#pragma unroll
        for (int dj = -1; dj <= 1; ++dj) {
            const int fj = 2 * j + dj;
            if (fj < 0 || fj >= FY) continue;
            const double *p = fine + 3 * (((long long) fi * FY + fj) * FZ + (live ? 2 * k : 0));
            double f0[3], f1[3], fm[3];
#pragma unroll
            for (int cc = 0; cc < 3; ++cc) {
                f0[cc] = p[cc];
                f1[cc] = hi ? p[3 + cc] : 0.0;
            }
#pragma unroll
            for (int cc = 0; cc < 3; ++cc) {
                fm[cc] = lane_below(f1[cc]);
                if (first && lo) fm[cc] = p[cc - 3];
            }
            if (pl <= 2) {
                const double w = (pl != 1 ? 0.5 : 1.0) * (dj ? 0.5 : 1.0);
#pragma unroll
                for (int cc = 0; cc < 3; ++cc) {
                    if (lo) a[cc] = fma(0.5 * w, fm[cc], a[cc]);
                    a[cc] = fma(w, f0[cc], a[cc]);
                    if (hi) a[cc] = fma(0.5 * w, f1[cc], a[cc]);
                }
            }
            if (pl >= 2 && second) {
                const double w = (pl != 3 ? 0.5 : 1.0) * (dj ? 0.5 : 1.0);
#pragma unroll
                for (int cc = 0; cc < 3; ++cc) {
                    if (lo) a2[cc] = fma(0.5 * w, fm[cc], a2[cc]);
                    a2[cc] = fma(w, f0[cc], a2[cc]);
                    if (hi) a2[cc] = fma(0.5 * w, f1[cc], a2[cc]);
                }
            }
        }
    }
    if (!live) return;
    const long long n = nidx(c, i, j, k);
    coarse[3 * n] = a[0]; coarse[3 * n + 1] = a[1]; coarse[3 * n + 2] = a[2];
    if (zeroed) { zeroed[3 * n] = 0.0; zeroed[3 * n + 1] = 0.0; zeroed[3 * n + 2] = 0.0; }
    if (second) {
        const long long n2 = nidx(c, i + 1, j, k);
        coarse[3 * n2] = a2[0]; coarse[3 * n2 + 1] = a2[1]; coarse[3 * n2 + 2] = a2[2];
        if (zeroed) { zeroed[3 * n2] = 0.0; zeroed[3 * n2 + 1] = 0.0; zeroed[3 * n2 + 2] = 0.0; }
    }
}

void launch_restrict(const Dims &c, int fineNX, int shift, const double *fine, double *coarse, hipStream_t s, double *zeroed) {
    dim3 blk(64, 4, 1), grd((c.NZ + 63) / 64, (c.NY + 3) / 4, (c.NX + 1) / 2);
    k_restrict<<<grd, blk, 0, s>>>(c, fineNX, shift, fine, coarse, zeroed);
    VFEM_HIP(hipGetLastError());
}

template <bool ACC>
__global__ void __launch_bounds__(256) k_prolong_rows(Dims c, int shift, const double *__restrict__ coarse, double *__restrict__ fine,
                                                      const uint8_t *__restrict__ fixed) {
    __shared__ __align__(16) double sh[4][384];
    const int FY = 2 * c.ny + 1, FZ = 2 * c.nz + 1;
    const int lane = threadIdx.x, wv = __builtin_amdgcn_readfirstlane(threadIdx.y);
    const int j = blockIdx.y * 4 + wv, i = blockIdx.z, chunk = blockIdx.x;
    if (j >= FY) return;
    const int ig = i - shift;
    const int i0 = ig >> 1, j0 = j >> 1, oi = ig & 1, oj = j & 1;
    const int k0 = 64 * chunk + lane;
    const bool live = k0 < c.NZ, up = k0 + 1 < c.NZ;
    const double w0 = (oi ? 0.5 : 1.0) * (oj ? 0.5 : 1.0), w1 = 0.5 * w0;
// ... 414 lines not shown
```

### ndr_amd/csrc/mg.hip

```cpp
#include "mg_cycle.h"

#include <algorithm>
#include <cstring>
#include <memory>

using namespace vfem;

void vfem::coarsen_dirichlet_mask(int N, int p, const int fine_nn[3], const std::vector<uint8_t> &fm, const int coarse_ne[3],
                                  std::vector<uint8_t> &cm) {
    long long nf_total = 1, nc_total = 1;
    int cnn[3] = {1, 1, 1};
    for (int a = 0; a < N; ++a) { cnn[a] = p * coarse_ne[a] + 1; nf_total *= fine_nn[a]; nc_total *= cnn[a]; }
    cm.assign((size_t) nc_total, 0);
    for (long long nf = 0; nf < nf_total; ++nf) {
        const uint8_t m = fm[nf];
        if (!m) continue;
        int g[3] = {0, 0, 0};
        { long long q = nf; for (int a = N - 1; a >= 0; --a) { g[a] = (int) (q % fine_nn[a]); q /= fine_nn[a]; } }
        int lo[3] = {0, 0, 0}, hi[3] = {0, 0, 0};
        bool any = false;
        for (int a = 0; a < N; ++a) {
            const int e = std::min(g[a] / (2 * p), coarse_ne[a] - 1), t = g[a] - 2 * p * e;
            if (t == 0) { lo[a] = hi[a] = p * e; any = true; }
            else if (t == 2 * p) { lo[a] = hi[a] = p * e + p; any = true; }
            else { lo[a] = p * e; hi[a] = p * e + p; }
        }
        if (!any) throw Error("Dirichlet constraints on internal nodes are not supported");
        for (int a0 = lo[0]; a0 <= hi[0]; ++a0)
            for (int a1 = lo[1]; a1 <= hi[1]; ++a1)
                for (int a2 = lo[2]; a2 <= hi[2]; ++a2) {
                    const int gg[3] = {a0, a1, a2};
                    long long node = gg[0];
                    for (int a = 1; a < N; ++a) node = node * cnn[a] + gg[a];
                    cm[node] |= m;
                }
    }
}

void vfem::galerkin_project(const double *K, int ke, int N, int npe, const double *Phi, double *T, double *out) {
    for (int i = 0; i < ke; ++i)
        for (int j = 0; j < ke; ++j) {
            const int m = j / N, b = j % N;
            double v = 0.0;
            for (int qn = 0; qn < npe; ++qn) v += K[(size_t) i * ke + N * qn + b] * Phi[qn * npe + m];
            T[(size_t) i * ke + j] = v;
        }
    for (int i = 0; i < ke; ++i)
        for (int j = 0; j < ke; ++j) {
            const int n = i / N, a = i % N;
            double v = 0.0;
            for (int pn = 0; pn < npe; ++pn) v += Phi[pn * npe + n] * T[(size_t) (N * pn + a) * ke + j];
            out[(size_t) i * ke + j] = v;
        }
}


static const double *level_K(const vfem_mg *mg, int l) {
    return l == 0 ? mg->fine->dK0.p : mg->cK0.p;
}
static const double *level_E(const vfem_mg *mg, int l) {
    const vfem_sim *sim = mg->fine;
    if (l == 0) return sim->Ep();
    return sim->E.p + 2 * mg->lv[1].ex_lo * (long long) sim->d.ny * sim->d.nz;
}

static bool level_uses_stencil(const vfem_mg *mg, int l) {
    const MgLevel &L = mg->lv[l];
    return L.kind == OP_STENCIL || (l == 1 && L.kind == OP_MF1 && mg->fine->tune.l1_stored == 1 && L.S.p);
}
static bool level_uses_half_stencil(const vfem_mg *mg, int l) {
    const MgLevel &L = mg->lv[l];
    return l == 1 && L.kind == OP_MF1 && mg->fine->tune.l1_stored == 2 && L.Sh.p;
}

static bool level_uses_merged_rows(const vfem_mg *mg, int l) {
    const MgLevel &L = mg->lv[l];
    return l == 1 && L.kind == OP_MF1 && mg->mf1_sym && mg->fine->tune.l1_merged && mg->fine->tune.gs_variant == 0 && mg->l1mtab.p &&
           l1_merged_usable(L.d);
}

void vfem::mg_apply(vfem_mg *mg, int l, const double *u, const double *b, int res, double *out, hipStream_t s) {
    MgLevel &L = mg->lv[l];
    if (level_uses_half_stencil(mg, l)) launch_apply_stencil_half(L.d, L.Sh.p, u, b, L.maskp, res, out, s);
    else if (level_uses_stencil(mg, l)) launch_apply_stencil(L.d, L.S.p, u, b, L.maskp, res, out, s);
    else if (L.kind == OP_MF0 && mg->fine->fast_ok) {
        const vfem_sim *sim = mg->fine;
        const Tuning &t = sim->tune;
        if (t.apply_impl == 0 &&
            launch_apply_dma(L.d, sim->Dm, level_E(mg, 0), sim->E.p + sim->n_store(), u, out, s, 0, -1, t.dma_chunks, t.dma_strip,
                             res ? b : nullptr, res ? L.maskp : nullptr, t.dma_lx)) return;
        launch_apply_fast(L.d, sim->Dm, level_E(mg, 0), u, b, L.maskp, res, out, s, t.apply_pd);
    }
    else if (level_uses_merged_rows(mg, l)) launch_l1_merged_apply(L.d, mg->l1mtab.p, level_E(mg, l), u, b, L.maskp, res, out, s);
    else launch_apply_gather(L.d, L.kind, level_K(mg, l), level_E(mg, l), u, b, L.maskp, res, out, s);
}

void vfem::mg_smooth(vfem_mg *mg, int l, double *u, const double *b, int forward, hipStream_t s, int first, int count) {
    MgLevel &L = mg->lv[l];
    if (level_uses_half_stencil(mg, l)) launch_gs_sweep_stencil_half(L.d, L.Sh.p, u, b, L.maskp, forward, L.xparity, first, count, s);
    else if (level_uses_stencil(mg, l)) launch_gs_sweep_stencil(L.d, L.S.p, u, b, L.maskp, forward, L.xparity, first, count, s, L.Sn.p, mg->fine->tune.stencil_split);
    else if (level_uses_merged_rows(mg, l)) launch_l1_merged_sweep(L.d, mg->l1mtab.p, level_E(mg, l), u, b, L.maskp, forward, L.xparity, first, count, s,
                                                                   mg->fine->tune.l1_merged == 2);
    else launch_gs_sweep_mf(L.d, L.kind, level_K(mg, l), l == 0 ? mg->fine->dGsTab.p : mg->mf1diag.p, level_E(mg, l), u, b, L.maskp,
                            forward, L.xparity, first, count, s, mg->fine->tune, mg->mf1_sym,
                            (l == 1 && mg->fine->tune.l1_diag) ? L.Mdiag.p : nullptr);
}

static bool gs_march_wanted(const MgLevel &L, const Tuning &t) {
    return t.gs_march == 2 || (t.gs_march == 1 && L.d.nn >= 800000);
}

static const double *march_table(const vfem_sim *sim) {
    return sim->k0_mirror_ok ? sim->dGsTab.p + GS_TABLE_DOUBLES + 84 : nullptr;
}

static bool level0_marches(const vfem_mg *mg, int l) {
    const vfem_sim *sim = mg->fine;
    const Tuning &t = sim->tune;
    return l == 0 && mg->lv[0].kind == OP_MF0 && gs_march_wanted(mg->lv[0], t) && t.gs_variant == 0 && t.gs_resident && sim->dGsTab.p &&
           sim->k0_mirror_ok;
}

static void gs_solve_data(vfem_mg *mg, hipStream_t s) {
    MgLevel &L = mg->lv[0];
    const vfem_sim *sim = mg->fine;
    if (L.gs_sd.p && L.gs_sd_version == sim->operator_version) return;
    L.gs_sd.reserve((size_t) L.d.nn * 3);
    launch_gs_solve_data(L.d, sim->dK0.p, level_E(mg, 0), L.maskp, L.gs_sd.p, s);
    L.gs_sd_version = sim->operator_version;
}

static void mg_smooth_n(vfem_mg *mg, int l, double *u, const double *b, int forward, int n, hipStream_t s) {
    MgLevel &L = mg->lv[l];
    const vfem_sim *sim = mg->fine;
    const Tuning &t = sim->tune;
    if (!(level0_marches(mg, l) && n > 0)) {
        for (int i = 0; i < n; ++i) mg_smooth(mg, l, u, b, forward, s);
        return;
    }
    L.tmp.reserve((size_t) L.d.nn * 3);
    gs_solve_data(mg, s);
    double *cur[2] = {u, u};
    for (int i = 0; i < n; ++i)
        for (int half = 0; half < 2; ++half) {
            const int cx = forward ? half : 1 - half;
            const int cxl = cx ^ (L.xparity & 1);
            if (cxl > L.d.NX - 1) continue;
            double *dst = cur[cxl] == u ? L.tmp.p : u;
            if (!launch_gs_march_mf0(L.d, march_table(sim), level_E(mg, 0), cur[cxl], cur[1 - cxl], dst, b, L.gs_sd.p,
                                     cxl, forward, t.gs_march_chunks, s, 0, -1)) {
                for (int par = 0; par < 2; ++par)
                    if (cur[par] != u) { launch_copy_planes(L.d, par, cur[par], u, s); cur[par] = u; }
                mg_smooth(mg, l, u, b, forward, s, 4 * half, 4);
                continue;
            }
            cur[cxl] = dst;
        }
    for (int par = 0; par < 2; ++par)
        if (cur[par] != u) launch_copy_planes(L.d, par, cur[par], u, s);
}

bool vfem::mg_smooth_half(vfem_mg *mg, int l, double *u, const double *b, int forward, int half, hipStream_t s, int plane_lo, int plane_hi) {
    MgLevel &L = mg->lv[l];
    const vfem_sim *sim = mg->fine;
    const Tuning &t = sim->tune;
    if (!level0_marches(mg, l)) return false;
    const int cx = forward ? half : 1 - half;
    const int cxl = cx ^ (L.xparity & 1);
    if (cxl > L.d.NX - 1) return true;
    L.tmp.reserve((size_t) L.d.nn * 3);
    gs_solve_data(mg, s);
    if (!launch_gs_march_mf0(L.d, march_table(sim), level_E(mg, 0), u, u, L.tmp.p, b, L.gs_sd.p,
                             cxl, forward, t.gs_march_chunks, s, plane_lo, plane_hi)) return false;
    launch_copy_planes(L.d, cxl, L.tmp.p, u, s, plane_lo, plane_hi);
    return true;
}

static void factor_coarsest(vfem_mg *mg, hipStream_t s) {
    const int L = mg->L;
    MgLevel &cl = mg->lv[L];
    CoarsestSolver &cs = mg->coarsest;
    const long long n = 3 * cl.d.nn;
    const bool planes = cs.wants_planes(n);
    cs.refuse_if_too_large(n, planes ? &cl.d : nullptr);
    const double *Sc = cl.S.p;
    DevBuf<double> tmpS;
    if (L < 2) {
        tmpS.alloc((size_t) stencil_storage_doubles(cl.d));
        launch_stencil_from_mf(cl.d, L == 0 ? OP_MF0 : OP_MF1, level_K(mg, L), level_E(mg, L), tmpS.p, s);
        Sc = tmpS.p;
    }
    if (planes) cs.factor_planes(cl.d, Sc, cl.maskp, s);
    else {
        launch_dense_from_stencil(cl.d, Sc, cl.maskp, cs.dense_matrix(n, s), s);
        cs.factor_dense(3, cl.maskp, s);
    }
    VFEM_HIP(hipStreamSynchronize(s));
}

static void build_reference_tables(vfem_mg *mg);

void vfem::update_operators(vfem_mg *mg, hipStream_t s) {
    vfem_sim *sim = mg->fine;
    if (mg->operators_valid && mg->operators_version == sim->operator_version) return;
    ScopedTimer tm("updateElementStiffnessMatrices");
    if (mg->material_version != sim->material_version) {
        VFEM_HIP(hipStreamSynchronize(s));
        build_reference_tables(mg);
    }
    const int L = mg->slab ? mg->L - 1 : mg->L;
    for (int l = mg->external_ke_level > 0 ? mg->external_ke_level + 1 : 2; l <= L; ++l) {
        MgLevel &lv = mg->lv[l];
        lv.Ke.alloc((size_t) lv.da.ne * 576);
        if (l == 2) launch_coarsen_ke(lv.da, 3, mg->c2K0.p, sim->E.p, nullptr, lv.Ke.p, s);
        else        launch_coarsen_ke(lv.da, 2, nullptr, nullptr, mg->lv[l - 1].Ke.p, lv.Ke.p, s);
    }
    if (mg->L >= 1 && mg->first_active <= 1 && mg->mf1_sym && sim->tune.l1_diag) {
        MgLevel &l1 = mg->lv[1];
        l1.Mdiag.alloc((size_t) l1.d.nn * 9);
        launch_mf1_diag(l1.d, mg->mf1diag.p, level_E(mg, 1), l1.Mdiag.p, s);
    }
    if (mg->L >= 1 && mg->first_active <= 1 && !mg->slab) {
        MgLevel &l1 = mg->lv[1];
        if (sim->tune.l1_stored == 1 && l1.kind == OP_MF1 && L >= 2) {
            l1.S.alloc((size_t) stencil_storage_doubles(l1.d));
            launch_stencil_from_mf(l1.d, OP_MF1, level_K(mg, 1), level_E(mg, 1), l1.S.p, s);
            l1.Sn.release();
            l1.Sh.release();
        } else if (sim->tune.l1_stored == 2 && l1.kind == OP_MF1 && L >= 2) {
            l1.Sh.alloc((size_t) stencil_half_storage_doubles(l1.d));
            launch_stencil_half_from_mf1(l1.d, level_K(mg, 1), level_E(mg, 1), l1.Sh.p, s);
            l1.S.release();
        } else if (l1.kind == OP_MF1) { l1.S.release(); l1.Sh.release(); }
    }
    for (int l = std::max(2, mg->first_active); l <= L; ++l) {
        MgLevel &lv = mg->lv[l];
        lv.S.alloc((size_t) stencil_storage_doubles(lv.d));
        launch_stencil_from_ke(lv.d, lv.Ke.p + lv.ex_lo * (long long) lv.d.ny * lv.d.nz * 576, lv.S.p, s);
        if (lv.d.nn <= WAVE_SWEEP_MAX_NODES) {
            lv.Sn.alloc((size_t) stencil_storage_doubles(lv.d));
            launch_stencil_node_major(lv.d, lv.S.p, lv.Sn.p, s);
        } else lv.Sn.release();
    }
    if (!mg->slab) factor_coarsest(mg, s);
    mg->operators_valid = true;
    mg->operators_version = sim->operator_version;
}

namespace {
struct TunedOps {
    vfem_mg *mg;
    hipStream_t s;
    MgLevel &lv(int l) const { return mg->lv[(size_t) l]; }

    int last_level() const { return mg->L; }
    void last_level_cycle(bool) { mg->coarsest.solve(lv(mg->L).b.p, lv(mg->L).x.p, s); }
    bool symmetric() const { return mg->symmetric_gs; }
    double *x(int l) const { return lv(l).x.p; }
    double *b(int l) const { return lv(l).b.p; }
    void enforce_dirichlet(int l, bool residual_system, bool dirichlet_zeroed) {
        if (!(dirichlet_zeroed && residual_system))
            launch_enforce_dirichlet(lv(l).d.nn, lv(l).maskp, l == 0 ? mg->fine->dvals.p : nullptr, x(l), residual_system ? 1 : 0, s);
    }
    void smooth(int l, int forward, int n) { mg_smooth_n(mg, l, x(l), b(l), forward, n, s); }
    void residual(int l) { mg_apply(mg, l, x(l), b(l), 1, lv(l).r.p, s); }
    void restrict_residual(int l) { launch_restrict(lv(l + 1).d, lv(l).d.NX, lv(l + 1).xshift, lv(l).r.p, b(l + 1), s, x(l + 1)); }
    void restrict_rhs(int l) { launch_restrict(lv(l + 1).d, lv(l).d.NX, lv(l + 1).xshift, b(l), b(l + 1), s); }
    void prolong_correction(int l) { launch_prolong(lv(l + 1).d, lv(l).d.NX, lv(l + 1).xshift, x(l + 1), x(l), 1, s); }
    bool prolong_start(int l, bool residual_system) {
        launch_prolong(lv(l + 1).d, lv(l).d.NX, lv(l + 1).xshift, x(l + 1), x(l), 0, s, residual_system ? lv(l).maskp : nullptr);
        return residual_system;
    }
    long long n_dofs() const { return 3 * lv(0).d.nn; }
    mg_cycle::CgWork cg() const { return {n_dofs(), mg->pd.p, mg->pAd.p, mg->scal.p, s}; }
    double *s_vector(bool preconditioned) const { return preconditioned ? x(0) : mg->ps.p; }
    void dot(const double *a, const double *b, double *out) { launch_dot(n_dofs(), a, b, mg->scratch.p, out, s); }
    void initial_residual(const double *x, const double *b, double *r) { mg_apply(mg, 0, x, b, 1, r, s); }
    void shift_and_dot_rs(const double *r, double *sv, double *sc) {
        launch_shift_scalar(sc, s);
        launch_dot_zero_dirichlet(n_dofs(), r, sv, lv(0).maskp, mg->scratch.p, sc + 0, s);
    }
    void apply_dot(const double *d, double *Ad, double *out) {
        mg_apply(mg, 0, d, nullptr, 0, Ad, s);
        launch_dot_zero_dirichlet(n_dofs(), d, Ad, lv(0).maskp, mg->scratch.p, out, s);
    }
    void step_dot(double *x, double *r, const double *d, const double *Ad, double *sc) { launch_pcg_step_dot(n_dofs(), x, r, d, Ad, sc, mg->scratch.p, sc + 3, s); }
};
}

void vfem::cycle_from_level(vfem_mg *mg, int l, int nsmooth, bool fmg, hipStream_t s) {
    TunedOps o{mg, s};
    mg_cycle::cycles(o, l, 1, nsmooth, true, fmg);
}

static void build_reference_tables(vfem_mg *mg) {
    vfem_sim *fine = mg->fine;
    double phi[8][64];
    for (int g = 0; g < 8; ++g)
        for (int fn = 0; fn < 8; ++fn)
            for (int cn = 0; cn < 8; ++cn) {
                double v = 1.0;
                for (int dd = 0; dd < 3; ++dd) {
                    const int sh = 2 - dd;
                    const double p = 0.5 * ((fn >> sh) & 1) + 0.5 * ((g >> sh) & 1);
                    v *= ((cn >> sh) & 1) ? p : (1.0 - p);
                }
                phi[g][fn * 8 + cn] = v;
            }
    std::vector<double> c(8 * 576), c2((size_t) 64 * 576), T(576);
    for (int g = 0; g < 8; ++g) galerkin_project(fine->K0, 24, 3, 8, phi[g], T.data(), c.data() + (size_t) g * 576);
    for (int g = 0; g < 8; ++g)
        for (int f = 0; f < 8; ++f)
            galerkin_project(c.data() + (size_t) f * 576, 24, 3, 8, phi[g], T.data(), c2.data() + (size_t) (g * 8 + f) * 576);
    mg->cK0.alloc(c.size());
    VFEM_HIP(hipMemcpy(mg->cK0.p, c.data(), c.size() * sizeof(double), hipMemcpyHostToDevice));
    mg->c2K0.alloc(c2.size());
    VFEM_HIP(hipMemcpy(mg->c2K0.p, c2.data(), c2.size() * sizeof(double), hipMemcpyHostToDevice));
    mg->mf1_sym = coarsened_matrices_are_mirror_images(c.data());
    {
        double dt[96];
        build_mf1_diag_table(c.data(), dt);
        mg->mf1diag.alloc(96);
        VFEM_HIP(hipMemcpy(mg->mf1diag.p, dt, sizeof(dt), hipMemcpyHostToDevice));
        double mt[L1M_TABLE_DOUBLES];
        build_l1_merged_table(c.data(), mt);
        mg->l1mtab.alloc(L1M_TABLE_DOUBLES);
        VFEM_HIP(hipMemcpy(mg->l1mtab.p, mt, sizeof(mt), hipMemcpyHostToDevice));
    }
    mg->material_version = fine->material_version;
}

static void finish_mg_create(vfem_mg *mg) {
    vfem_sim *fine = mg->fine;
    build_reference_tables(mg);
    for (int l = mg->first_active; l <= mg->L; ++l) {
        MgLevel &lv = mg->lv[(size_t) l];
        lv.x.alloc((size_t) lv.d.nn * 3); lv.b.alloc((size_t) lv.d.nn * 3); lv.r.alloc((size_t) lv.d.nn * 3);
        lv.x.zero(nullptr); lv.b.zero(nullptr); lv.r.zero(nullptr);
    }
    if (mg->first_active == 0 && !mg->slab) {
        const size_t n3 = (size_t) fine->d.nn * 3;
        mg->pd.alloc(n3); mg->pAd.alloc(n3); mg->ps.alloc(n3);
    }
    mg->scal.alloc(16); mg->scratch.alloc(REDUCE_SCRATCH_DOUBLES);
    mg->scal.zero(nullptr);
    VFEM_HIP(hipDeviceSynchronize());
}
// ... 95 lines not shown
int64_t vfem_mg_level_num_nodes(const vfem_mg *mg, int level) {
    if (level < 0 || level > mg->L) return -1;
    return mg->lv[(size_t) level].d.nn;
}
int vfem_mg_level_dirichlet_mask(const vfem_mg *mg, int level, uint8_t *mask_host) {
    VFEM_TRY
    const MgLevel &lv = mg->lv.at((size_t) level);
    std::memcpy(mask_host, lv.hmask.data(), lv.hmask.size());
    VFEM_CATCH
}
int vfem_mg_set_symmetric_gauss_seidel(vfem_mg *mg, int symmetric) { mg->symmetric_gs = symmetric != 0; return 0; }
int vfem_mg_tensor_paths(const vfem_mg *mg) {
    return vfem_sim_tensor_paths(mg->fine) | (mg->mf1_sym ? VFEM_PATH_L1_MIRROR : 0);
}
const double *vfem_mg_field_ptr(const vfem_mg *mg, int which, int level) {
    if (which == 2) return mg->lv[0].b.p;
    if (level < 0 || level > mg->L) return nullptr;
    return which == 0 ? mg->lv[(size_t) level].x.p : mg->lv[(size_t) level].b.p;
}

int vfem_mg_update_operators(vfem_mg *mg, void *stream) { VFEM_TRY update_operators(mg, S(stream)); VFEM_CATCH }

int vfem_mg_export_level_ke(vfem_mg *mg, int level, int64_t child_first_layer, int64_t count_x, double *ke_out, void *stream) {
    VFEM_TRY
    check_level(mg, level);
    if (level < 2) throw Error("element matrices exist from level 2 on (level 1 is virtual)");
    if (count_x < 0 || child_first_layer < 0) throw Error("negative layer range");
    update_operators(mg, S(stream));
    const MgLevel &lv = mg->lv[(size_t) level];
    const Dims c(count_x, lv.d.ny, lv.d.nz);
    if (level == 2) {
        const vfem_sim *sim = mg->fine;
        if (child_first_layer + 4 * count_x > sim->d.nx + sim->ex_lo + sim->ex_hi) throw Error("layer range outside the fine element array");
        launch_coarsen_ke(c, 3, mg->c2K0.p, sim->E.p + child_first_layer * (long long) sim->d.ny * sim->d.nz, nullptr, ke_out, S(stream));
    } else {
        const MgLevel &ch = mg->lv[(size_t) level - 1];
        if (!ch.Ke.p) throw Error("the child level holds no element matrices");
        if (child_first_layer + 2 * count_x > ch.da.nx) throw Error("layer range outside the child level's element array");
        launch_coarsen_ke(c, 2, nullptr, nullptr, ch.Ke.p + child_first_layer * (long long) ch.da.ny * ch.da.nz * 576, ke_out, S(stream));
    }
    VFEM_CATCH
}
int vfem_mg_import_level_ke(vfem_mg *mg, int level, const double *ke, void *stream) {
    VFEM_TRY
    check_level(mg, level);
    if (level < 2 || level != mg->first_active) throw Error("element matrices can be supplied for the first active level (>= 2) of a partial hierarchy");
    MgLevel &lv = mg->lv[(size_t) level];
    lv.Ke.alloc((size_t) lv.da.ne * 576);
    VFEM_HIP(hipMemcpyAsync(lv.Ke.p, ke, (size_t) lv.da.ne * 576 * sizeof(double), hipMemcpyDeviceToDevice, S(stream)));
    mg->external_ke_level = level;
    mg->operators_valid = false;
    VFEM_CATCH
}

int vfem_mg_apply_k(vfem_mg *mg, int level, const double *u, double *out, void *stream) {
    VFEM_TRY
    check_level(mg, level);
    if (level >= 1) update_operators(mg, S(stream));
    mg_apply(mg, level, u, nullptr, 0, out, S(stream));
    VFEM_CATCH
}
int vfem_mg_residual(vfem_mg *mg, int level, const double *u, const double *b, double *r, void *stream) {
    VFEM_TRY
    check_level(mg, level);
    if (level >= 1) update_operators(mg, S(stream));
    mg_apply(mg, level, u, b, 1, r, S(stream));
    VFEM_CATCH
}
int vfem_mg_smooth(vfem_mg *mg, int level, double *u, const double *b, int forward, void *stream) {
    VFEM_TRY
    check_level(mg, level);
    if (level >= 1) update_operators(mg, S(stream));
    mg_smooth_n(mg, level, u, b, forward, 1, S(stream));
    VFEM_CATCH
}
int vfem_mg_smooth_sweeps(vfem_mg *mg, int level, double *u, const double *b, int forward, int sweeps, void *stream) {
    VFEM_TRY
    check_level(mg, level);
    if (sweeps < 0) throw Error("negative sweep count");
    if (level >= 1) update_operators(mg, S(stream));
    mg_smooth_n(mg, level, u, b, forward, sweeps, S(stream));
    VFEM_CATCH
}
int vfem_mg_zero_dirichlet(vfem_mg *mg, int level, double *u, void *stream) {
    VFEM_TRY
    check_level(mg, level);
    launch_zero_dirichlet(mg->lv[(size_t) level].d.nn, mg->lv[(size_t) level].maskp, u, S(stream));
    VFEM_CATCH
}
int vfem_mg_restrict(vfem_mg *mg, int fine_level, const double *fine, double *coarse, void *stream) {
    VFEM_TRY
    check_level(mg, fine_level + 1);
    launch_restrict(mg->lv[(size_t) fine_level + 1].d, mg->lv[(size_t) fine_level].d.NX, mg->lv[(size_t) fine_level + 1].xshift, fine, coarse, S(stream));
    VFEM_CATCH
}
int vfem_mg_interpolate(vfem_mg *mg, int fine_level, const double *coarse, double *fine, int accumulate, void *stream) {
    VFEM_TRY
    check_level(mg, fine_level + 1);
    launch_prolong(mg->lv[(size_t) fine_level + 1].d, mg->lv[(size_t) fine_level].d.NX, mg->lv[(size_t) fine_level + 1].xshift, coarse, fine, accumulate, S(stream));
    VFEM_CATCH
}
int vfem_mg_coarsest_solve(vfem_mg *mg, const double *b, double *x, void *stream) {
    VFEM_TRY
    update_operators(mg, S(stream));
    mg->coarsest.solve(b, x, S(stream));
    VFEM_CATCH
}
int vfem_mg_set_coarsest_solver(vfem_mg *mg, int mode) {
    VFEM_TRY
    if (mg->coarsest.set_mode(mode)) mg->operators_valid = false;
    VFEM_CATCH
}
int64_t vfem_mg_coarsest_bytes(const vfem_mg *mg) {
    if (!mg->operators_valid || mg->slab) return 0;
    return mg->coarsest.bytes();
}

int vfem_mg_smooth_colors(vfem_mg *mg, int level, double *u, const double *b, int forward, int first, int count, void *stream) {
    VFEM_TRY
    check_level(mg, level);
    if (first < 0 || count < 0 || first + count > 8) throw Error("colour range out of [0, 8)");
    if (level >= 1) update_operators(mg, S(stream));
    if (first % 4 == 0 && count == 4 && mg_smooth_half(mg, level, u, b, forward, first / 4, S(stream))) return 0;
    mg_smooth(mg, level, u, b, forward, S(stream), first, count);
    VFEM_CATCH
}
int vfem_mg_can_smooth_planes(vfem_mg *mg, int level) {
    return (mg && level <= mg->L && level0_marches(mg, level)) ? 1 : 0;
}
int vfem_mg_smooth_group_planes(vfem_mg *mg, int level, double *u, const double *b, int forward, int group, int64_t plane_lo, int64_t plane_hi,
                                void *stream) {
    VFEM_TRY
    check_level(mg, level);
    if (group < 0 || group > 1) throw Error("colour group must be 0 or 1");
    if (plane_lo < 0 || plane_hi > mg->lv[(size_t) level].d.NX - 1) throw Error("plane range outside the level's node grid");
    if (plane_lo > plane_hi) return 0;
    if (!mg_smooth_half(mg, level, u, b, forward, group, S(stream), (int) plane_lo, (int) plane_hi))
        throw Error("plane-range sweeps need the marching finest-level kernel (vfem_mg_can_smooth_planes)");
    VFEM_CATCH
}
int vfem_mg_cycle_from_level(vfem_mg *mg, int level, double *x, const double *b, int nsmooth, int fmg, void *stream) {
    VFEM_TRY
    check_level(mg, level);
    if (level < mg->first_active) throw Error("level below the first active level of this hierarchy");
    if (mg->slab) throw Error("slab hierarchies are cycled by the distributed driver");
    hipStream_t s = S(stream);
    update_operators(mg, s);
    TunedOps o{mg, s};
    mg_cycle::cycles_on(o, level, 3 * mg->lv[(size_t) level].d.nn, x, b, 1, nsmooth, true, fmg != 0, s);
    VFEM_CATCH
}

int vfem_mg_solve(vfem_mg *mg, double *x, const double *f, int num_steps, int nsmooth, int stiffness_updated,
                  int zero_dirichlet, int fmg, void *stream) {
    VFEM_TRY
    ScopedTimer tm("MG Solver");
    hipStream_t s = S(stream);
    (void) stiffness_updated;
    update_operators(mg, s);
    if (num_steps == 0) return 0;
    TunedOps o{mg, s};
    mg_cycle::cycles_on(o, 0, o.n_dofs(), x, f, num_steps, nsmooth, zero_dirichlet != 0, fmg != 0, s);
    VFEM_CATCH
}

int vfem_mg_pcg(vfem_mg *mg, double *x, const double *b, int max_iter, double tol, int mg_iterations,
// ... 16 lines not shown
```

### ndr_amd/csrc/mg_cycle.h

```cpp
#pragma once
#include "vfem_host.h"

#include <cmath>

namespace vfem {
namespace mg_cycle {

struct CgWork { long long n; double *d, *Ad, *sc; hipStream_t s; };

template <class Ops> void vcycle(Ops &o, int l, int nsmooth, bool residual_system, bool dirichlet_zeroed = false) {
    if (l == o.last_level()) { o.last_level_cycle(false); return; }
    o.enforce_dirichlet(l, residual_system, dirichlet_zeroed);
    o.smooth(l, 1, nsmooth);
    o.residual(l);
    o.restrict_residual(l);
    vcycle(o, l + 1, nsmooth, true, true);
    o.prolong_correction(l);
    o.smooth(l, o.symmetric() ? 0 : 1, nsmooth);
}

template <class Ops> void full_multigrid(Ops &o, int l, int nsmooth, bool residual_system) {
    if (l == o.last_level()) { o.last_level_cycle(true); return; }
    o.restrict_rhs(l);
    full_multigrid(o, l + 1, nsmooth, residual_system);
    const bool zeroed = o.prolong_start(l, residual_system);
    vcycle(o, l, nsmooth, residual_system, zeroed);
}

template <class Ops> void cycles(Ops &o, int l, int n, int nsmooth, bool residual_system, bool fmg) {
    if (fmg) full_multigrid(o, l, nsmooth, residual_system);
    for (int i = fmg ? 1 : 0; i < n; ++i) vcycle(o, l, nsmooth, residual_system);
}

template <class Ops>
void cycles_on(Ops &o, int l, long long n, double *x, const double *b, int cycles_n, int nsmooth, bool residual_system, bool fmg, hipStream_t s) {
    const size_t bytes = (size_t) n * sizeof(double);
    VFEM_HIP(hipMemcpyAsync(o.b(l), b, bytes, hipMemcpyDeviceToDevice, s));
    if (!fmg) VFEM_HIP(hipMemcpyAsync(o.x(l), x, bytes, hipMemcpyDeviceToDevice, s));
    cycles(o, l, cycles_n, nsmooth, residual_system, fmg);
    VFEM_HIP(hipMemcpyAsync(x, o.x(l), bytes, hipMemcpyDeviceToDevice, s));
}

template <class Ops>
void pcg(Ops &o, double *x, const double *b, int max_iter, double tol, int mg_iterations, int mg_smoothing, bool fmg,
         vfem_residual_cb residual_cb, void *cb_user, int *iters_out, double *relres_out) {
    const CgWork w = o.cg();
    hipStream_t s = w.s;
    const size_t bytes = (size_t) w.n * sizeof(double);
    double *r = o.b(0), *d = w.d, *Ad = w.Ad, *sc = w.sc, *sv = o.s_vector(mg_smoothing != 0), host_sc[2];
    o.dot(b, b, sc + 4);
    o.initial_residual(x, b, r);
    o.dot(r, r, sc + 3);
    VFEM_HIP(hipMemcpyAsync(host_sc, sc + 3, 2 * sizeof(double), hipMemcpyDeviceToHost, s));
    VFEM_HIP(hipStreamSynchronize(s));
    double rr = host_sc[0], bb = host_sc[1];
    int it = 0;
    while (it < max_iter && rr > tol * tol * bb) {
        ++it;
        if (mg_smoothing == 0) {
            VFEM_HIP(hipMemcpyAsync(sv, r, bytes, hipMemcpyDeviceToDevice, s));
        } else {
            if (!fmg) VFEM_HIP(hipMemsetAsync(o.x(0), 0, bytes, s));
            cycles(o, 0, mg_iterations, mg_smoothing, true, fmg);
        }
        o.shift_and_dot_rs(r, sv, sc);
        launch_pcg_direction(w.n, sv, d, sc, it == 1, s);
        o.apply_dot(d, Ad, sc + 2);
        o.step_dot(x, r, d, Ad, sc);
        VFEM_HIP(hipMemcpyAsync(host_sc, sc + 3, sizeof(double), hipMemcpyDeviceToHost, s));
        VFEM_HIP(hipStreamSynchronize(s));
        rr = host_sc[0];
        if (!(rr == rr)) throw Error("PCG produced NaN residual");
        if (residual_cb) residual_cb(cb_user, it, std::sqrt(rr));
    }
    if (iters_out) *iters_out = it;
    if (relres_out) *relres_out = bb > 0 ? std::sqrt(rr / bb) : 0.0;
}

}
}
```

### ndr_amd/csrc/mg_slab.hip

```cpp
#include "mg_cycle.h"

using namespace vfem;

namespace {
struct DistDriver {
    vfem_mg *loc, *rep;
    int T, rank, world, nsmooth;
    bool overlap;
    const vfem_dist_level *g;
    double *xT, *bT, *work_d, *work_Ad, *scalars;
    vfem_halo_fn halo_fn;
    vfem_allreduce_fn allreduce_fn;
    void *user;
    hipStream_t s;

    void halo(int l, double *f, bool left = true, bool right = true, int phase = 0) {
        if (world == 1 || !(g[l].gl || g[l].gr)) return;
        if (halo_fn(user, l, f, left ? 1 : 0, right ? 1 : 0, phase) != 0) throw Error("halo exchange callback failed");
    }
    void allreduce(double *buf, long long n) {
        if (world > 1 && allreduce_fn(user, buf, (int64_t) n) != 0) throw Error("all-reduce callback failed");
    }
    void dot(const double *a, const double *b, double *out) {
        const vfem_dist_level &G = g[0];
        const long long lo = G.first_owned, hi = G.last_owned + (rank == world - 1 ? 1 : 0), per = 3 * G.plane_nodes;
        launch_dot((hi - lo) * per, a + lo * per, b + lo * per, loc->scratch.p, out, s);
        allreduce(out, 1);
    }
    void smooth_colors(int l, double *x, const double *b, int forward, int first) {
        if (!mg_smooth_half(loc, l, x, b, forward, first / 4, s)) mg_smooth(loc, l, x, b, forward, s, first, 4);
    }
    void smooth(int l, double *x, const double *b, int forward) {
        const vfem_dist_level &G = g[l];
        const bool by_planes = overlap && vfem_mg_can_smooth_planes(loc, l);
        for (int group = 0; group < 2; ++group) {
            const int cx = forward ? group : 1 - group;
            const bool send_left = G.gl && ((G.xoffn + G.first_owned + 1) & 1) == cx;
            const bool send_right = G.gr && ((G.xoffn + G.last_owned - 1) & 1) == cx;
            if (!(send_left || send_right) || world == 1) { smooth_colors(l, x, b, forward, 4 * group); continue; }
            if (!by_planes) {
                smooth_colors(l, x, b, forward, 4 * group);
                halo(l, x, send_left, send_right, 0);
                continue;
            }
            auto sweep = [&](long long lo, long long hi) {
                if (lo > hi) return;
                if (!mg_smooth_half(loc, l, x, b, forward, group, s, (int) lo, (int) hi)) throw Error("plane-range sweep unavailable");
            };
            const long long lo_plane = G.first_owned + 1, hi_plane = G.last_owned - 1;
            long long inner_lo = G.first_owned, inner_hi = G.last_owned;
            if (send_left) { sweep(lo_plane, lo_plane); inner_lo = lo_plane + 1; }
            if (send_right && !(send_left && hi_plane == lo_plane)) { sweep(hi_plane, hi_plane); inner_hi = hi_plane - 1; }
            else if (send_right) inner_hi = hi_plane - 1;
            halo(l, x, send_left, send_right, 1);
            sweep(inner_lo, inner_hi);
            halo(l, x, send_left, send_right, 2);
        }
    }
    void coarse_cycle(bool fmg) {
        const vfem_dist_level &G = g[T];
        MgLevel &R = rep->lv[(size_t) T];
        const long long lo = G.first_owned, hi = G.last_owned + (rank == world - 1 ? 1 : 0), per = 3 * G.plane_nodes;
        const size_t bytes = (size_t) R.d.nn * 3 * sizeof(double);
        VFEM_HIP(hipMemsetAsync(bT, 0, bytes, s));
        VFEM_HIP(hipMemcpyAsync(bT + (G.xoffn + lo) * per, G.b + lo * per, (size_t) ((hi - lo) * per) * sizeof(double), hipMemcpyDeviceToDevice, s));
        allreduce(bT, (long long) R.d.nn * 3);
        VFEM_HIP(hipMemcpyAsync(R.b.p, bT, bytes, hipMemcpyDeviceToDevice, s));
        if (!fmg) R.x.zero(s);
        cycle_from_level(rep, T, nsmooth, fmg, s);
        VFEM_HIP(hipMemcpyAsync(G.x, R.x.p + G.xoffn * per, (size_t) (G.n_planes * per) * sizeof(double), hipMemcpyDeviceToDevice, s));
    }
    MgLevel &lv(int l) const { return loc->lv[(size_t) l]; }
    int last_level() const { return T; }
    void last_level_cycle(bool fmg) { coarse_cycle(fmg); }
    bool symmetric() const { return loc->symmetric_gs; }
    double *x(int l) const { return g[l].x; }
    double *b(int l) const { return g[l].b; }
    void enforce_dirichlet(int l, bool, bool) { launch_zero_dirichlet(lv(l).d.nn, lv(l).maskp, x(l), s); }
    void smooth(int l, int forward, int n) { for (int i = 0; i < n; ++i) smooth(l, x(l), b(l), forward); }
    void residual(int l) { mg_apply(loc, l, x(l), b(l), 1, g[l].r, s); halo(l, g[l].r); }
    void restrict_residual(int l) { launch_restrict(lv(l + 1).d, lv(l).d.NX, lv(l + 1).xshift, g[l].r, b(l + 1), s, x(l + 1)); }
    void restrict_rhs(int l) { halo(l, b(l)); launch_restrict(lv(l + 1).d, lv(l).d.NX, lv(l + 1).xshift, b(l), b(l + 1), s); }
    void prolong_correction(int l) { launch_prolong(lv(l + 1).d, lv(l).d.NX, lv(l + 1).xshift, x(l + 1), x(l), 1, s); halo(l, x(l)); }
    bool prolong_start(int l, bool) { launch_prolong(lv(l + 1).d, lv(l).d.NX, lv(l + 1).xshift, x(l + 1), x(l), 0, s); halo(l, x(l)); return false; }

    long long n_dofs() const { return 3 * lv(0).d.nn; }
    mg_cycle::CgWork cg() const { return {n_dofs(), work_d, work_Ad, scalars, s}; }
    double *s_vector(bool) const { return x(0); }
    void initial_residual(double *x, const double *b, double *r) { halo(0, x); mg_apply(loc, 0, x, b, 1, r, s); }
    void shift_and_dot_rs(const double *r, double *sv, double *sc) {
        launch_zero_dirichlet(lv(0).d.nn, lv(0).maskp, sv, s);
        launch_shift_scalar(sc, s);
        dot(r, sv, sc + 0);
    }
    void apply_dot(double *d, double *Ad, double *out) {
        halo(0, d);
        mg_apply(loc, 0, d, nullptr, 0, Ad, s);
        launch_zero_dirichlet(lv(0).d.nn, lv(0).maskp, Ad, s);
        dot(d, Ad, out);
    }
    void step_dot(double *x, double *r, const double *d, const double *Ad, double *sc) { launch_pcg_step(n_dofs(), x, r, d, Ad, sc, s); dot(r, r, sc + 3); }
};
}
extern "C" {

int vfem_mg_pcg_slab(vfem_mg *local, vfem_mg *replicated, int first_replicated_level, const vfem_dist_level *levels, int rank, int world,
                     double *replicated_x, double *replicated_b, double *x, const double *b, double *work_d, double *work_Ad, double *scalars,
                     int max_iter, double tol, int mg_iterations, int mg_smoothing, int fmg, int overlap_sweeps,
                     vfem_halo_fn halo, vfem_allreduce_fn allreduce, void *cb_user, vfem_residual_cb residual_cb, void *residual_user,
                     int *iters_out, double *relres_out, void *stream) {
    VFEM_TRY
    if (!local || !local->slab) throw Error("vfem_mg_pcg_slab: the local hierarchy must come from vfem_mg_create_slab");
    const int T = first_replicated_level;
    if (T < 1 || T != local->L) throw Error("vfem_mg_pcg_slab: the local hierarchy must end at the first replicated level");
    if (!replicated || replicated->slab || T > replicated->L || T < replicated->first_active) throw Error("vfem_mg_pcg_slab: level not active in the replicated hierarchy");
    if (world > 1 && (!halo || !allreduce)) throw Error("vfem_mg_pcg_slab: callbacks missing");
    for (int l = 0; l <= T; ++l) {
        const MgLevel &L = local->lv[(size_t) l];
        if (levels[l].n_planes != L.d.NX || levels[l].plane_nodes != (int64_t) L.d.NY * L.d.NZ) throw Error("vfem_mg_pcg_slab: level geometry does not match the hierarchy");
        if (!levels[l].x || !levels[l].b || (l < T && !levels[l].r)) throw Error("vfem_mg_pcg_slab: work vector missing");
    }
    DistDriver D{local, replicated, T, rank, world, mg_smoothing, overlap_sweeps != 0, levels, replicated_x, replicated_b, work_d, work_Ad, scalars,
                 halo, allreduce, cb_user, S(stream)};
    launch_zero_dirichlet(local->lv[0].d.nn, local->lv[0].maskp, x, D.s);
    update_operators(local, D.s);
    update_operators(replicated, D.s);
    mg_cycle::pcg(D, x, b, max_iter, tol, mg_iterations, mg_smoothing, fmg != 0, residual_cb, residual_user, iters_out, relres_out);
    VFEM_CATCH
}

}
```

### ndr_amd/csrc/sim.hip

```cpp
#include "vfem_host.h"
#include "gs_coef.h"

#include <cmath>
#include <cstring>
#include <memory>

using namespace vfem;

void vfem_sim::update_k0() {
    static const double Mm[2][2] = {{1.0 / 3, 1.0 / 6}, {1.0 / 6, 1.0 / 3}};
    static const double Dd[2][2] = {{1.0, -1.0}, {-1.0, 1.0}};
    static const double Gg[2][2] = {{-0.5, -0.5}, {0.5, 0.5}};
    const double vol = h[0] * h[1] * h[2];
    auto I = [&](int n, int m, int p, int q) {
        double v = 1.0 / (h[p] * h[q]);
        for (int dd = 0; dd < 3; ++dd) {
            const int a = (n >> (2 - dd)) & 1, b = (m >> (2 - dd)) & 1;
            if (dd == p && dd == q) v *= Dd[a][b];
            else if (dd == p)       v *= Gg[a][b];
            else if (dd == q)       v *= Gg[b][a];
            else                    v *= Mm[a][b];
        }
        return v;
    };
// ... 118 lines not shown
int vfem_sim_create_padded(vfem_sim **out, const double bbmin[3], const double bbmax[3], const int64_t ne[3], int64_t extra_lo,
                           int64_t extra_hi) {
    VFEM_TRY
    for (int dd = 0; dd < 3; ++dd)
        if (ne[dd] < 1 || ne[dd] > 4096) throw Error("elements per dimension must be in [1, 4096]");
    if (extra_lo < 0 || extra_hi < 0) throw Error("negative padding");
    std::unique_ptr<vfem_sim> sim(new vfem_sim);
    sim->d = Dims(ne[0], ne[1], ne[2]);
    for (int dd = 0; dd < 3; ++dd) {
        sim->h[dd] = (bbmax[dd] - bbmin[dd]) / (double) ne[dd];
        if (!(sim->h[dd] > 0)) throw Error("empty domain bounding box");
    }
    sim->update_k0();
    sim->ex_lo = extra_lo; sim->ex_hi = extra_hi;
    sim->rho.alloc((size_t) sim->n_store());   sim->rho.zero(nullptr);
    sim->E.alloc((size_t) sim->n_store());
    launch_simp(sim->n_store(), sim->rho.p, sim->E0, sim->Emin, sim->gamma, sim->E.p, nullptr);
    sim->dmask.alloc((size_t) sim->d.nn); sim->dmask.zero(nullptr);
    sim->dvals.alloc((size_t) sim->d.nn * 3); sim->dvals.zero(nullptr);
    sim->loads.alloc((size_t) sim->d.nn * 3); sim->loads.zero(nullptr);
    sim->hmask.assign((size_t) sim->d.nn, 0);
    sim->hvals.assign((size_t) sim->d.nn * 3, 0.0);
    VFEM_HIP(hipDeviceSynchronize());
    *out = sim.release();
    VFEM_CATCH
}
int vfem_sim_create(vfem_sim **out, const double bbmin[3], const double bbmax[3], const int64_t ne[3]) {
    return vfem_sim_create_padded(out, bbmin, bbmax, ne, 0, 0);
}
int vfem_sim_destroy(vfem_sim *sim) { VFEM_TRY delete sim; VFEM_CATCH }
int64_t vfem_sim_num_nodes(const vfem_sim *sim) { return sim->d.nn; }
int64_t vfem_sim_num_elements(const vfem_sim *sim) { return sim->d.ne; }
int64_t vfem_sim_num_stored_elements(const vfem_sim *sim) { return sim->n_store(); }

int vfem_sim_set_isotropic(vfem_sim *sim, double young, double poisson) {
    VFEM_TRY
    sim->lambda = poisson * young / ((1.0 + poisson) * (1.0 - 2.0 * poisson));
    sim->mu = young / (2.0 + 2.0 * poisson);
    sim->general_tensor = false;
    sim->update_k0();
    ++sim->operator_version;
    VFEM_CATCH
}
int vfem_sim_set_elasticity_tensor(vfem_sim *sim, const double D[36]) {
    VFEM_TRY
    check_flattened_tensor(D, 6);
    for (int i = 0; i < 6; ++i)
        for (int j = 0; j < 6; ++j) sim->D[i * 6 + j] = 0.5 * (D[i * 6 + j] + D[j * 6 + i]);
    sim->general_tensor = true;
    sim->update_k0();
    ++sim->operator_version;
    VFEM_CATCH
}
int vfem_sim_tensor_paths(const vfem_sim *sim) {
    return (sim->fast_ok ? VFEM_PATH_MODE_SPACE : 0) | (sim->gs_resident_ok ? VFEM_PATH_GS_RESIDENT : 0) |
           (sim->k0_mirror_ok ? VFEM_PATH_K0_MIRROR : 0);
}
int vfem_sim_set_simp(vfem_sim *sim, double E0, double Emin, double gamma) {
    VFEM_TRY
    sim->E0 = E0; sim->Emin = Emin; sim->gamma = gamma;
    ++sim->operator_version;
    launch_simp(sim->n_store(), sim->rho.p, E0, Emin, gamma, sim->E.p, nullptr);
    VFEM_HIP(hipDeviceSynchronize());
    VFEM_CATCH
}
int vfem_sim_set_option(vfem_sim *sim, int key, int value) {
    VFEM_TRY
    Tuning &t = sim->tune;
    switch (key) {
        case VFEM_OPT_APPLY_PLANES:  if (value < 2 || value > 4) throw Error("planes in flight must be 2..4"); t.apply_pd = value; break;
        case VFEM_OPT_GS_VARIANT:    t.gs_variant = value != 0; break;
        case VFEM_OPT_APPLY_IMPL:    t.apply_impl = value != 0; break;
        case VFEM_OPT_DMA_CHUNKS:    if (value < 0) throw Error("negative chunk count"); t.dma_chunks = value; break;
        case VFEM_OPT_DMA_STRIP:     if (value < 0 || value > 2) throw Error("strip mode must be 0..2"); t.dma_strip = value; break;
        case VFEM_OPT_DMA_LX:        if (value < 0 || value > 2) throw Error("line-exclusive tiling mode must be 0..2"); t.dma_lx = value; break;
        case VFEM_OPT_GS_PAIR:       t.gs_pair = value != 0; break;
        case VFEM_OPT_GS_RESIDENT:   t.gs_resident = (value != 0 && sim->gs_resident_ok) ? 1 : 0; break;
        case VFEM_OPT_L1_SPLIT:      if (value != 1 && value != 2 && value != 4 && value != 8) throw Error("level-1 slot split 1, 2, 4 or 8"); t.l1_split = value; break;
        case VFEM_OPT_STENCIL_SPLIT: t.stencil_split = value != 0; break;
        case VFEM_OPT_GS_MARCH:      if (value < 0 || value > 2) throw Error("marching sweep mode 0..2"); t.gs_march = value; break;
        case VFEM_OPT_GS_MARCH_CHUNKS: if (value < 0) throw Error("negative chunk count"); t.gs_march_chunks = value; break;
        case VFEM_OPT_L1_STORED:     if (value < 0 || value > 2) throw Error("level-1 storage mode 0..2"); t.l1_stored = value; ++sim->operator_version; break;
        case VFEM_OPT_L1_MERGED:     if (value < 0 || value > 2) throw Error("level-1 row mode 0..2"); t.l1_merged = value; break;
        case VFEM_OPT_L1_DIAG:       t.l1_diag = value != 0; ++sim->operator_version; break;
        default: throw Error("unknown simulator option " + std::to_string(key));
    }
    VFEM_CATCH
}
int vfem_sim_k0(const vfem_sim *sim, double *K0_host) {
    VFEM_TRY std::memcpy(K0_host, sim->K0, sizeof(sim->K0)); VFEM_CATCH
}
int vfem_sim_set_dirichlet(vfem_sim *sim, const uint8_t *mask_host, const double *values_host) {
    VFEM_TRY
    sim->hmask.assign(mask_host, mask_host + sim->d.nn);
    sim->nonzero_dirichlet = false;
    if (values_host) {
        sim->hvals.assign(values_host, values_host + 3 * sim->d.nn);
        for (long long n = 0; n < sim->d.nn; ++n)
            for (int c = 0; c < 3; ++c)
                if (((sim->hmask[n] >> c) & 1) && sim->hvals[3 * n + c] != 0.0) sim->nonzero_dirichlet = true;
    } else sim->hvals.assign((size_t) sim->d.nn * 3, 0.0);
    ++sim->operator_version;
    VFEM_HIP(hipMemcpy(sim->dmask.p, sim->hmask.data(), (size_t) sim->d.nn, hipMemcpyHostToDevice));
    VFEM_HIP(hipMemcpy(sim->dvals.p, sim->hvals.data(), (size_t) sim->d.nn * 3 * sizeof(double), hipMemcpyHostToDevice));
    VFEM_CATCH
}
int vfem_sim_set_loads(vfem_sim *sim, const double *f, void *stream) {
    VFEM_TRY
    VFEM_HIP(hipMemcpyAsync(sim->loads.p, f, (size_t) sim->d.nn * 3 * sizeof(double), hipMemcpyDeviceToDevice, S(stream)));
    VFEM_CATCH
}
int vfem_sim_build_load_vector(const vfem_sim *sim, double *f, void *stream) {
    VFEM_TRY
    VFEM_HIP(hipMemcpyAsync(f, sim->loads.p, (size_t) sim->d.nn * 3 * sizeof(double), hipMemcpyDeviceToDevice, S(stream)));
    VFEM_CATCH
}
int vfem_sim_set_densities(vfem_sim *sim, const double *rho, void *stream) {
    VFEM_TRY
    VFEM_HIP(hipMemcpyAsync(sim->rho.p, rho, (size_t) sim->n_store() * sizeof(double), hipMemcpyDeviceToDevice, S(stream)));
    ++sim->operator_version;
    launch_simp(sim->n_store(), sim->rho.p, sim->E0, sim->Emin, sim->gamma, sim->E.p, S(stream));
    VFEM_CATCH
}
int vfem_sim_set_uniform_density(vfem_sim *sim, double rho, void *stream) {
    VFEM_TRY
    if (rho > 1.0 || rho < 0.0)
        throw Error("Density value (" + std::to_string(rho) + ") has to be in between 0 and 1");
    ++sim->operator_version;
    launch_fill(sim->n_store(), rho, sim->rho.p, S(stream));
    launch_simp(sim->n_store(), sim->rho.p, sim->E0, sim->Emin, sim->gamma, sim->E.p, S(stream));
    VFEM_CATCH
}
int vfem_sim_get_densities(const vfem_sim *sim, double *rho, void *stream) {
    VFEM_TRY
    VFEM_HIP(hipMemcpyAsync(rho, sim->rho.p, (size_t) sim->n_store() * sizeof(double), hipMemcpyDeviceToDevice, S(stream)));
    VFEM_CATCH
}
int vfem_sim_apply_k(const vfem_sim *sim, const double *u, double *out, int variant, void *stream) {
    VFEM_TRY
    ScopedTimer tm("applyK");
    if (variant != 1 && sim->fast_ok) {
        bool done = false;
        if (variant == 0 && sim->tune.apply_impl == 0)
            done = launch_apply_dma(sim->d, sim->Dm, sim->Ep(), sim->E.p + sim->n_store(), u, out, S(stream), 0, -1,
                                    sim->tune.dma_chunks, sim->tune.dma_strip, nullptr, nullptr, sim->tune.dma_lx);
        if (!done) launch_apply_fast(sim->d, sim->Dm, sim->Ep(), u, nullptr, nullptr, 0, out, S(stream), sim->tune.apply_pd);
    }
    else launch_apply_gather(sim->d, OP_MF0, sim->dK0.p, sim->Ep(), u, nullptr, nullptr, 0, out, S(stream));
    VFEM_CATCH
}
int vfem_sim_apply_k_planes(const vfem_sim *sim, const double *u, double *out, int64_t plane_lo, int64_t plane_hi, void *stream) {
    VFEM_TRY
    if (plane_lo < 0 || plane_hi > sim->d.NX - 1) throw Error("plane range outside the node grid");
    if (plane_lo > plane_hi) return 0;
    if (!sim->fast_ok) throw Error("plane-range apply needs the mode-space kernel (box voxels, isotropic or grid-aligned orthotropic tensor)");
    if (!launch_apply_dma(sim->d, sim->Dm, sim->Ep(), sim->E.p + sim->n_store(), u, out, S(stream), (int) plane_lo, (int) plane_hi,
                          sim->tune.dma_chunks, sim->tune.dma_strip, nullptr, nullptr, sim->tune.dma_lx))
        throw Error("plane-range apply needs 8-byte aligned device buffers");
    VFEM_CATCH
}
int vfem_sim_compliance_gradient(const vfem_sim *sim, const double *u, double *g, void *stream) {
    VFEM_TRY
    launch_compliance_gradient(sim->d, sim->dK0.p, sim->rhop(), sim->E0, sim->Emin, sim->gamma, u, g, S(stream));
    VFEM_CATCH
}
int vfem_compliance(const vfem_sim *sim, const double *f, const double *u, double *value_host, void *stream) {
// ... 19 lines not shown
```

### ndr_amd/csrc/vfem_host.h

```cpp
#pragma once
#include "vfem_internal.h"

#include <chrono>

#define VFEM_TRY try {
#define VFEM_CATCH                                                                              \
    } catch (const std::exception &e) { vfem::set_error(e.what()); return 1; }                  \
      catch (...) { vfem::set_error("unknown error"); return 1; }                               \
    return 0;

static inline hipStream_t S(void *s) { return (hipStream_t) s; }

namespace vfem {

void timer_add(const char *name, double seconds);
struct ScopedTimer {
    const char *name;
    std::chrono::steady_clock::time_point t0;
    explicit ScopedTimer(const char *n) : name(n), t0(std::chrono::steady_clock::now()) {}
    ~ScopedTimer() { timer_add(name, std::chrono::duration<double>(std::chrono::steady_clock::now() - t0).count()); }
};

constexpr size_t REDUCE_SCRATCH_DOUBLES = 2048;
double compliance(long long n, const double *f, const double *u, hipStream_t s);

void check_flattened_tensor(const double *D, int n);

void galerkin_project(const double *K, int ke, int N, int npe, const double *Phi, double *scratch, double *out);

void coarsen_dirichlet_mask(int N, int p, const int fine_nn[3], const std::vector<uint8_t> &fine_mask, const int coarse_ne[3],
                            std::vector<uint8_t> &coarse_mask);

void mg_apply(vfem_mg *mg, int l, const double *u, const double *b, int res, double *out, hipStream_t s);
void mg_smooth(vfem_mg *mg, int l, double *u, const double *b, int forward, hipStream_t s, int first = 0, int count = 8);
bool mg_smooth_half(vfem_mg *mg, int l, double *u, const double *b, int forward, int half, hipStream_t s, int plane_lo = 0, int plane_hi = -1);
void update_operators(vfem_mg *mg, hipStream_t s);
void cycle_from_level(vfem_mg *mg, int l, int nsmooth, bool fmg, hipStream_t s);

}
```

### ndr_amd/csrc/vfem_internal.h

```cpp
#pragma once
#include <hip/hip_runtime.h>
#include <cstdint>
#include <cstdio>
#include <stdexcept>
#include <string>
#include <vector>

#include "../../include/vfem.h"

namespace vfem {

void set_error(const std::string &msg);

struct Error : std::runtime_error { using std::runtime_error::runtime_error; };

#define VFEM_HIP(expr)                                                                         \
    do {                                                                                       \
        hipError_t e_ = (expr);                                                                \
        if (e_ != hipSuccess)                                                                  \
            throw ::vfem::Error(std::string(#expr) + ": " + hipGetErrorString(e_));            \
    } while (0)

struct Dims {
    int nx, ny, nz;
    int NX, NY, NZ;
    long long nn, ne;
    Dims() = default;
    Dims(long long ex, long long ey, long long ez)
        : nx((int) ex), ny((int) ey), nz((int) ez), NX((int) ex + 1), NY((int) ey + 1), NZ((int) ez + 1),
          nn((ex + 1) * (ey + 1) * (ez + 1)), ne(ex * ey * ez) {}
};

template <class T>
struct DevBuf {
    T *p = nullptr;
    size_t n = 0;
    DevBuf() = default;
    DevBuf(const DevBuf &) = delete;
    DevBuf &operator=(const DevBuf &) = delete;
    DevBuf(DevBuf &&o) noexcept : p(o.p), n(o.n) { o.p = nullptr; o.n = 0; }
    DevBuf &operator=(DevBuf &&o) noexcept { if (this != &o) { release(); p = o.p; n = o.n; o.p = nullptr; o.n = 0; } return *this; }
    ~DevBuf() { release(); }
    void release() { if (p) { (void) hipFree(p); p = nullptr; n = 0; } }
    void alloc(size_t count) {
        if (count == n && p) return;
        release();
        if (count == 0) return;
        VFEM_HIP(hipMalloc((void **) &p, count * sizeof(T)));
        n = count;
    }
    void reserve(size_t count) { if (!(p && n >= count)) alloc(count); }
    void zero(hipStream_t s) { if (p) VFEM_HIP(hipMemsetAsync(p, 0, n * sizeof(T), s)); }
};

enum OpKind {
    OP_MF0 = 0,
    OP_MF1 = 1,
    OP_STENCIL = 2,
};

void launch_simp(long long n, const double *rho, double E0, double Emin, double gamma, double *E, hipStream_t s);
void launch_fill(long long n, double v, double *x, hipStream_t s);

void launch_apply_gather(const Dims &d, OpKind kind, const double *K, const double *E, const double *u,
                         const double *b, const uint8_t *mask, int res, double *out, hipStream_t s);
void launch_apply_stencil(const Dims &d, const double *S, const double *u, const double *b, const uint8_t *mask,
                          int res, double *out, hipStream_t s);
struct Tuning {
    int apply_impl = 0;
    int apply_pd = 2;
    int dma_chunks = 0;
    int dma_strip = 1;
    int dma_lx = 0;
    int gs_variant = 0;
    int gs_pair = 1;
    int gs_resident = 0;
    int l1_split = 4;
    int stencil_split = 1;
    int gs_march = 1;
    int gs_march_chunks = 0;
    int l1_stored = 0;
    int l1_merged = 2;
    int l1_diag = 0;
};
#ifdef VFEM_ABLATION
extern int g_ablate_apply, g_ablate_store, g_ablate_mlp;
inline int ablate_apply() { return g_ablate_apply; }
inline int ablate_store() { return g_ablate_store; }
inline int ablate_mlp() { return g_ablate_mlp; }
#else
constexpr int ablate_apply() { return 0; }
constexpr int ablate_store() { return 0; }
constexpr int ablate_mlp() { return 0; }
#endif

void launch_apply_fast(const Dims &d, const double *Dm_host, const double *E, const double *u, const double *b,
                       const uint8_t *mask, int mode, double *out, hipStream_t s, int planes_in_flight = 2);
bool launch_apply_dma(const Dims &d, const double *Dm_host, const double *E, const double *E_alloc_end, const double *u,
                      double *out, hipStream_t s, int plane_lo = 0, int plane_hi = -1, int chunks = 0, int strip = 1,
                      const double *rhs = nullptr, const uint8_t *fixed = nullptr, int line_exclusive = 0);

void launch_gs_sweep_mf(const Dims &d, OpKind kind, const double *K, const double *gs_tab, const double *E, double *u,
                        const double *b, const uint8_t *mask, int forward, int xparity, int first, int count, hipStream_t s,
                        const Tuning &tune, bool mf1_sym, const double *mf1_diag = nullptr);
bool launch_gs_march_mf0(const Dims &d, const double *neighbour_kind_table, const double *E, const double *uR, const double *uO, double *dst, const double *b,
                         const double *solve_data, int cxl, int forward, int chunks, hipStream_t s, int plane_lo = 0, int plane_hi = -1);
void launch_gs_solve_data(const Dims &d, const double *K0, const double *E, const uint8_t *mask, double *sd, hipStream_t s);
void launch_copy_planes(const Dims &d, int par, const double *src, double *dst, hipStream_t s, int plane_lo = 0, int plane_hi = -1);
void launch_mf1_diag(const Dims &d, const double *Dtab, const double *E, double *Mdiag, hipStream_t s);
void build_gs_table(const double *K0, double *tab );
constexpr int GS_TABLE_DOUBLES = 72 * 12;
bool build_gs_coef(const double *K0, double *coef );
bool coarsened_matrices_are_mirror_images(const double *cK0_host );
void build_mf1_diag_table(const double *cK0_0, double *tab );
constexpr int L1M_TABLE_DOUBLES = 8 * 8 * 12;
void build_l1_merged_table(const double *cK0_0, double *tab );
bool l1_merged_usable(const Dims &d);
void launch_l1_merged_sweep(const Dims &d, const double *tab, const double *E, double *u, const double *b, const uint8_t *mask,
                            int forward, int xparity, int first, int count, hipStream_t s, int pair = 1);
void launch_l1_merged_apply(const Dims &d, const double *tab, const double *E, const double *u, const double *b, const uint8_t *mask,
                            int res, double *out, hipStream_t s);
void launch_gs_sweep_stencil(const Dims &d, const double *S, double *u, const double *b, const uint8_t *mask,
                             int forward, int xparity, int first, int count, hipStream_t s, const double *S_node_major = nullptr,
                             int stencil_split = 1);
long long stencil_half_storage_doubles(const Dims &d);
void launch_stencil_half_from_mf1(const Dims &d, const double *cK0, const double *Efine, double *Sh, hipStream_t s);
void launch_gs_sweep_stencil_half(const Dims &d, const double *Sh, double *u, const double *b, const uint8_t *mask,
                                  int forward, int xparity, int first, int count, hipStream_t s);
void launch_apply_stencil_half(const Dims &d, const double *Sh, const double *u, const double *b, const uint8_t *mask, int res, double *out,
                               hipStream_t s);
void launch_stencil_node_major(const Dims &d, const double *St, double *Sn, hipStream_t s);
constexpr long long WAVE_SWEEP_MAX_NODES = 40000;

void launch_restrict(const Dims &coarse, int fineNX, int shift, const double *fine, double *coarse_out, hipStream_t s, double *zeroed = nullptr);
void launch_prolong(const Dims &coarse, int fineNX, int shift, const double *coarse_in, double *fine, int accumulate, hipStream_t s,
                    const uint8_t *fixed = nullptr);

void launch_zero_dirichlet(long long nn, const uint8_t *mask, double *u, hipStream_t s);
void launch_enforce_dirichlet(long long nn, const uint8_t *mask, const double *vals, double *u, int zero, hipStream_t s);

void launch_coarsen_ke(const Dims &c, int mode, const double *cK0, const double *Efine, const double *Kef,
                       double *Kec, hipStream_t s);
long long stencil_storage_doubles(const Dims &d);
void launch_stencil_from_ke(const Dims &d, const double *Ke, double *S, hipStream_t s);
void launch_stencil_from_mf(const Dims &d, OpKind kind, const double *K, const double *E, double *S, hipStream_t s);
void launch_dense_from_stencil(const Dims &d, const double *S, const uint8_t *mask, double *A, hipStream_t s);
void launch_dense_finish_inverse(long long n, int N, const uint8_t *mask, double *A, hipStream_t s);
void launch_plane_rows_from_stencil(const Dims &d, const double *S, const uint8_t *mask, double *R, hipStream_t s);
void launch_gemv_sym(long long n, const double *A, const double *x, double *y, hipStream_t s);

void launch_compliance_gradient(const Dims &d, const double *K0, const double *rho, double E0, double Emin,
                                double gamma, const double *u, double *g, hipStream_t s);

void launch_dot(long long n, const double *a, const double *b, double *scratch, double *out, hipStream_t s);
void launch_dot_zero_dirichlet(long long n3, const double *a, double *b_masked_in_place, const uint8_t *mask, double *scratch, double *out, hipStream_t s);
void launch_pcg_step_dot(long long n3, double *x, double *r, const double *dv, const double *Ad, const double *sc, double *scratch,
                         double *rr_out, hipStream_t s);
void launch_pcg_direction(long long n, const double *sv, double *dv, const double *sc, int first, hipStream_t s);
void launch_pcg_step(long long n, double *x, double *r, const double *dv, const double *Ad, const double *sc,
                     hipStream_t s);
void launch_shift_scalar(double *sc, hipStream_t s);

void launch_box_filter(int nx, int ny, int nz, int r, const double *in, double *out, int transpose, hipStream_t s);
void launch_box_filter_slab(int nx, int ny, int nz, int x_first, int nx_global, int out_first, int out_layers, int r,
                            const double *in, double *out, int transpose, hipStream_t s);
void launch_projection(long long n, double beta, const double *x, const double *g, double *out, int mode, hipStream_t s);
void launch_oc_candidate(long long n, const double *x0, const double *dJ, const double *dc, double lambda, double m, double *out, hipStream_t s);
void launch_sum(long long n, const double *a, double *scratch, double *out, hipStream_t s);
void launch_langelaar_apply(int nx, int ny, int nz, double eps, double p, double q, const double *in, double *out, double *smax,
                            hipStream_t s);
void launch_langelaar_backprop(int nx, int ny, int nz, double eps, double p, double q, const double *g, const double *vars,
                               const double *out, const double *smax, double *work, double *grad, hipStream_t s);

void launch_apply_q2(int nx, int ny, int nz, const double *K0, const double *E, const double *u, double *out, hipStream_t s);
void launch_apply_q2_pencil(int nx, int ny, int nz, const double *mode_table, const double *E, const double *u, double *out, hipStream_t s);
void launch_apply_q2_march(int nx, int ny, int nz, const double *mode_table, const double *E, const double *u, double *out, hipStream_t s);
void launch_gs_sweep_q2_level0(int nx, int ny, int nz, const double *K0, const double *E, double *u, const double *b,
                               const uint8_t *mask, int forward, hipStream_t s, int first = 0, int count = 27);
struct DenseWork { DevBuf<double> L, X, Tm, D; DevBuf<int> info; };
void dense_spd_inverse(long long n, double *A, DenseWork &w, hipStream_t s);
struct PlaneSolver {
    Dims d;
    DevBuf<double> T;
    DevBuf<double> R;
    DevBuf<double> W;
    DevBuf<double> z, t;
    long long m() const { return 3LL * d.NY * d.NZ; }
    long long bytes() const { return (long long) ((T.n + R.n) * sizeof(double)); }
    void release() { T.release(); R.release(); W.release(); z.release(); t.release(); }
};
constexpr long long PLANE_SPD_MAX_BYTES = 8LL << 30;
long long plane_spd_bytes_needed(const Dims &d);
void plane_spd_factor(PlaneSolver &ps, const Dims &d, const double *S, const uint8_t *mask, DenseWork &w, hipStream_t s);
void plane_spd_solve(PlaneSolver &ps, const double *b, double *x, hipStream_t s);
constexpr long long DENSE_COARSEST_MAX_DOFS = 40000;
struct CoarsestSolver {
    int mode = VFEM_COARSEST_AUTO;
    enum Held { NONE, DENSE, PLANES } held = NONE;
    long long n = 0;
    DevBuf<double> Ainv;
    DenseWork work;
    PlaneSolver planes;
    bool set_mode(int m);
    bool wants_planes(long long dofs) const { return mode == VFEM_COARSEST_PLANES || (mode == VFEM_COARSEST_AUTO && dofs > DENSE_COARSEST_MAX_DOFS); }
    void refuse_if_too_large(long long dofs, const Dims *plane_grid) const;
    double *dense_matrix(long long dofs, hipStream_t s);
    void factor_dense(int N, const uint8_t *mask, hipStream_t s);
// ... 137 lines not shown
```

Measured before the change: 79.69 GVoxel/s.

## Skip zero-neighbour terms in first coarse-level Gauss-Seidel sweep from zero start

When a coarse multigrid level starts from a zeroed iterate, the first forward Gauss-Seidel sweep now uses specialised kernels that skip neighbour blocks which are still zero for the current colour. This applies to the merged level-1 row kernels and the stencil path. The aim is to cut loads and flops during pre-smoothing in the V-cycle. It adds many template instantiations and a new option, and the SpMV throughput metric itself is likely unaffected.

```diff
diff --git a/__graft_entry__.py b/__graft_entry__.py
--- a/__graft_entry__.py
+++ b/__graft_entry__.py
@@ -11,7 +11,9 @@
     csrc = os.path.join(ROOT, "ndr_amd", "csrc")
     subprocess.check_call(["make", "-C", csrc, "-j4"])
     for src, kernels in (("kernels_q2", ["k_apply_q2_marchILi0"]),
-                         ("kernels_l1_merged", ["k_l1_mergedILi0E", "k_l1_mergedILi1E", "k_l1_mergedILi2E", "k_l1_pair_rowsILi0E", "k_l1_pair_rowsILi1E"]),
+                         ("kernels_l1_merged", ["k_l1_mergedILi0E", "k_l1_mergedILi1E", "k_l1_mergedILi2E", "k_l1_pair_rowsILi0E", "k_l1_pair_rowsILi1E"] +
+                          ["k_l1_merged_zsILi%dELb%dEEE" % (p, s) for p in (4, 12, 7, 15) for s in (0, 1) if (p, s) != (15, 1)] +
+                          ["k_l1_pair_rows_zsILi%dELb%dEEE" % (p, s) for p in (4, 7) for s in (0, 1)]),
                          ("kernels_gs_march", ["k_gs_march_mf0ILi%dELi%dELi%dEEE" % (a, f, m) for a in (0, 1) for f in (0, 1) for m in (0, 1)])):
         asm = os.path.join(csrc, src + ".isa.s")
         subprocess.check_call(["/opt/rocm/bin/hipcc", "-O3", "-std=c++17", "-fPIC", "--offload-arch=gfx950", "-ffp-contract=on",
diff --git a/include/vfem.h b/include/vfem.h
--- a/include/vfem.h
+++ b/include/vfem.h
@@ -37,6 +37,7 @@
     VFEM_OPT_GS_MARCH_CHUNKS = 20,
     VFEM_OPT_L1_STORED    = 21,
     VFEM_OPT_L1_MERGED    = 22,
+    VFEM_OPT_ZERO_START   = 23,
     VFEM_OPT_Q2_GS_IMPL   = 16,
     VFEM_OPT_TRANSFER_AXIS = 17,
     VFEM_OPT_Q2_L1_VIRTUAL = 14
@@ -119,6 +120,7 @@
 int vfem_mg_residual(vfem_mg *mg, int level, const double *u, const double *b, double *r, void *stream);
 int vfem_mg_smooth(vfem_mg *mg, int level, double *u, const double *b, int forward, void *stream);
 int vfem_mg_smooth_sweeps(vfem_mg *mg, int level, double *u, const double *b, int forward, int sweeps, void *stream);
+int vfem_mg_smooth_sweeps_from_zero(vfem_mg *mg, int level, double *u_out, const double *b, int sweeps, void *stream);
 int vfem_mg_zero_dirichlet(vfem_mg *mg, int level, double *u, void *stream);
 int vfem_mg_restrict(vfem_mg *mg, int fine_level, const double *fine, double *coarse, void *stream);
 int vfem_mg_interpolate(vfem_mg *mg, int fine_level, const double *coarse, double *fine, int accumulate, void *stream);
diff --git a/ndr_amd/_lib.py b/ndr_amd/_lib.py
--- a/ndr_amd/_lib.py
+++ b/ndr_amd/_lib.py
@@ -75,6 +75,7 @@
     "vfem_mg_residual": (c_int, [c_void_p, c_int, c_void_p, c_void_p, c_void_p, c_void_p]),
     "vfem_mg_smooth": (c_int, [c_void_p, c_int, c_void_p, c_void_p, c_int, c_void_p]),
     "vfem_mg_smooth_sweeps": (c_int, [c_void_p, c_int, c_void_p, c_void_p, c_int, c_int, c_void_p]),
+    "vfem_mg_smooth_sweeps_from_zero": (c_int, [c_void_p, c_int, c_void_p, c_void_p, c_int, c_void_p]),
     "vfem_mg_zero_dirichlet": (c_int, [c_void_p, c_int, c_void_p, c_void_p]),
     "vfem_mg_restrict": (c_int, [c_void_p, c_int, c_void_p, c_void_p, c_void_p]),
     "vfem_mg_interpolate": (c_int, [c_void_p, c_int, c_void_p, c_void_p, c_int, c_void_p]),
diff --git a/ndr_amd/csrc/coef_rows.h b/ndr_amd/csrc/coef_rows.h
--- a/ndr_amd/csrc/coef_rows.h
+++ b/ndr_amd/csrc/coef_rows.h
@@ -59,6 +59,27 @@
     __device__ __forceinline__ void get(double c[9]) { pipe.template take<G * 4 + row_pos<MID>(W)>(c); }
 };
 
+template <int PARTS>
+struct L1MidPartRows {
+    static_assert(PARTS > 0 && PARTS < 16, "parts of the middle part");
+    static constexpr int NR = (PARTS & 1) + ((PARTS >> 1) & 1) + ((PARTS >> 2) & 1) + ((PARTS >> 3) & 1);
+    static constexpr int rank(int pos) { int n = 0; for (int q = 0; q < pos; ++q) n += (PARTS >> q) & 1; return n; }
+    static constexpr int pos(int idx) { int q = 0; while (!((PARTS >> q) & 1) || rank(q) != idx) ++q; return q; }
+    static constexpr int at(int r) { return ((r / NR) * 8 + row_kind<true>(pos(r % NR))) * l1m::TAB_ROW * 8; }
+};
+template <int PARTS>
+struct DevCoefMidParts {
+    using Rows = L1MidPartRows<PARTS>;
+    RowPipe<8 * Rows::NR, Rows> pipe;
+    __device__ __forceinline__ explicit DevCoefMidParts(const double *tab) : pipe{tab} {}
+    __device__ __forceinline__ void prime() { pipe.prime(); }
+    template <int G, int W>
+    __device__ __forceinline__ void get(double c[9]) {
+        static_assert((PARTS >> row_pos<true>(W)) & 1, "row of a part that is left out");
+        pipe.template take<G * Rows::NR + Rows::rank(row_pos<true>(W))>(c);
+    }
+};
+
 struct L0NodeRows {
     static constexpr int at(int r) { return (r < 4 ? 7 - r : r < 8 ? row_kind<true>(r - 4) : 7 - (r - 8)) * l1m::TAB_ROW * 8; }
 };
diff --git a/ndr_amd/csrc/generic.hip b/ndr_amd/csrc/generic.hip
--- a/ndr_amd/csrc/generic.hip
+++ b/ndr_amd/csrc/generic.hip
@@ -947,7 +947,7 @@
     void enforce_dirichlet(int l, bool residual_system, bool) {
         g_dirichlet(lv(l).d, lv(l).mask.p, (l == 0 && !residual_system) ? mg->fine->dvals.p : nullptr, x(l), s);
     }
-    void smooth(int l, int forward, int n) { for (int i = 0; i < n; ++i) gmg_smooth(mg, l, x(l), b(l), forward, s); }
+    void smooth(int l, int forward, int n, bool ) { for (int i = 0; i < n; ++i) gmg_smooth(mg, l, x(l), b(l), forward, s); }
     void residual(int l) { gmg_apply(mg, l, x(l), b(l), 1, lv(l).r.p, s); }
     void restrict_residual(int l) { gmg_restrict(mg, l, lv(l).r.p, b(l + 1), s); lv(l + 1).x.zero(s); }
     void restrict_rhs(int l) { gmg_restrict(mg, l, b(l), b(l + 1), s); }
diff --git a/ndr_amd/csrc/gs_colors.h b/ndr_amd/csrc/gs_colors.h
--- a/ndr_amd/csrc/gs_colors.h
+++ b/ndr_amd/csrc/gs_colors.h
@@ -31,4 +31,15 @@
 }
 inline int parity_bits(const GsColor &c) { return 4 * (c.start[0] & 1) + 2 * (c.start[1] & 1) + (c.start[2] & 1); }
 
+inline unsigned gs_zero_start_blocks(int lni) {
+    unsigned blocks = 0;
+    for (int nb = 0; nb < 27; ++nb) {
+        const int w = (nb / 9 != 1 ? 4 : 0) | ((nb / 3) % 3 != 1 ? 2 : 0) | (nb % 3 != 1 ? 1 : 0);
+        const int top = w & 4 ? 4 : w & 2 ? 2 : w;
+        if (w == 0 || (lni & top)) blocks |= 1u << nb;
+    }
+    return blocks;
 }
+constexpr unsigned GS_ALL_BLOCKS = (1u << 27) - 1;
+
+}
diff --git a/ndr_amd/csrc/hom_mg.hip b/ndr_amd/csrc/hom_mg.hip
--- a/ndr_amd/csrc/hom_mg.hip
+++ b/ndr_amd/csrc/hom_mg.hip
@@ -74,7 +74,7 @@
         launch_hom_mg_gemv(g(h->L()), h->coarsest.Ainv.p, b(h->L()), x(h->L()), s);
     }
     void enforce_dirichlet(int, bool, bool) {}
-    void smooth(int l, int forward, int n) { for (int k = 0; k < n; ++k) sweep(h, l, x(l), b(l), forward, s); }
+    void smooth(int l, int forward, int n, bool ) { for (int k = 0; k < n; ++k) sweep(h, l, x(l), b(l), forward, s); }
     void residual(int l) { launch_hom_mg_residual(g(l), h->blocks(l), x(l), b(l), r(l), s); }
     void restrict_residual(int l) {
         launch_hom_mg_restrict(g(l), g(l + 1), r(l), h->lv[l + 1].b.p, s);
diff --git a/ndr_amd/csrc/kernels_l1_merged.hip b/ndr_amd/csrc/kernels_l1_merged.hip
--- a/ndr_amd/csrc/kernels_l1_merged.hip
+++ b/ndr_amd/csrc/kernels_l1_merged.hip
@@ -2,6 +2,7 @@
 #include "device_utils.h"
 #include "l1_merged_core.h"
 #include "coef_rows.h"
+#include "gs_colors.h"
 
 
 namespace vfem {
@@ -83,25 +84,27 @@
 #endif
     if constexpr (G + 1 < 8) side_classes<SIDE, G + 1>(m, un, cf, S);
 }
-template <int G>
-__device__ __forceinline__ void mid_classes(const ModuliLds &m, const double (&un)[3][9], DevCoef<true> &cf, double S[3], double M[6]) {
+template <int G, int PARTS = 15, class Coef>
+__device__ __forceinline__ void mid_classes(const ModuliLds &m, const double (&un)[3][9], Coef &cf, double S[3], double M[6]) {
 #ifdef L1M_NOCOMP
     if constexpr (G == 0) { for (auto &r : un) for (double v : r) S[1] += v; M[0] = M[3] = M[5] = 1.0; }
 #else
     double a0[2][2], a1[2][2];
     m.template window<G>(1 - ((G >> 2) & 1), a0);
     m.template window<G>(2 + ((G >> 2) & 1), a1);
-    l1m::mid_class<G>(a0, a1, un, cf, S, M);
-#endif
-    if constexpr (G + 1 < 8) mid_classes<G + 1>(m, un, cf, S, M);
-}
-
-template <int MODE>
+    l1m::mid_class_parts<G, PARTS>(a0, a1, un, cf, S, M);
+#endif
+    if constexpr (G + 1 < 8) mid_classes<G + 1, PARTS>(m, un, cf, S, M);
+}
+
+template <int MODE, int PARTS = 15, bool SIDES = true>
 __device__ __forceinline__ void node_group(const Dims &d, const double *__restrict__ tab, const double *__restrict__ E, const double *u,
                                            const double *__restrict__ b, const uint8_t *__restrict__ mask, double *out, int i, int j, int k,
                                            bool live, int role, int lane, int forward, double (&part)[2][3][64], double (*sE)[16][64]) {
+    static_assert(MODE == 0 || (PARTS == 15 && SIDES), "only a sweep starts from zero");
+    constexpr bool FROM_ZERO = PARTS != 15 || !SIDES;
     double un[3][9];
-    load_nodes(plane_rsrc(u, 3LL * d.NY * d.NZ, i + role - 1, d.NX), d, j, k, un);
+    if (SIDES || role == 1) load_nodes(plane_rsrc(u, 3LL * d.NY * d.NZ, i + role - 1, d.NX), d, j, k, un);
     const long long n = ((long long) i * d.NY + j) * d.NZ + k;
     double bn[3] = {0.0, 0.0, 0.0};
     uint8_t mk8 = 0;
@@ -130,11 +133,20 @@
     const ModuliLds m{sE, lane};
     double S[3] = {0.0, 0.0, 0.0}, M6[6] = {0.0, 0.0, 0.0, 0.0, 0.0, 0.0};
     if (role == 1) {
-        DevCoef<true> cf(tab);
+        if constexpr (PARTS == 15) {
+            DevCoef<true> cf(tab);
 #ifndef L1M_NOCOMP
-        cf.prime();
-#endif
-        mid_classes<0>(m, un, cf, S, M6);
+            cf.prime();
+#endif
+            mid_classes<0>(m, un, cf, S, M6);
+        } else {
+            DevCoefMidParts<PARTS> cf(tab);
+#ifndef L1M_NOCOMP
+            cf.prime();
+#endif
+            mid_classes<0, PARTS>(m, un, cf, S, M6);
+        }
+    } else if (!SIDES) {
     } else if (role == 0) {
         DevCoef<false> cf(tab);
 #ifndef L1M_NOCOMP
@@ -156,7 +168,7 @@
     if (role != 1 || !live) return;
 #pragma unroll
     for (int c = 0; c < 3; ++c) S[c] = (part[0][c][lane] + S[c]) + part[1][c][lane];
-    const double uc[3] = {un[1][3], un[1][4], un[1][5]};
+    const double uc[3] = {FROM_ZERO ? 0.0 : un[1][3], FROM_ZERO ? 0.0 : un[1][4], FROM_ZERO ? 0.0 : un[1][5]};
     const double M[9] = {M6[0], M6[1], M6[2], M6[1], M6[3], M6[4], M6[2], M6[4], M6[5]};
     if (MODE == 1) {
 #pragma unroll
@@ -223,6 +235,64 @@
     }
 }
 
+template <int PARTS, bool SIDES>
+__global__ void __launch_bounds__(192, L1M_WAVES) k_l1_merged_zs(Dims d, const double *__restrict__ tab, const double *__restrict__ E,
+                                                                 double *u, const double *__restrict__ b, const uint8_t *__restrict__ mask,
+                                                                 int cx, int cy, int cz, int ka, int kskip) {
+    __shared__ double part[2][3][64];
+    __shared__ double sE[4][16][64];
+    const int lane = threadIdx.x, role = __builtin_amdgcn_readfirstlane(threadIdx.y);
+    const int cnty = (d.NY - 1 - cy) / 2 + 1, cntz = (d.NZ - 1 - cz) / 2 + 1 - kskip;
+    const int q = blockIdx.x * 64 + lane;
+    const bool live = q < cnty * cntz;
+    const int qq = live ? q : cnty * cntz - 1, jq = qq / cntz, r = qq - jq * cntz;
+    const int k = 2 * (r < ka ? r : r + kskip) + cz, j = 2 * jq + cy, i = 2 * blockIdx.z + cx;
+    node_group<0, PARTS, SIDES>(d, tab, E, u, b, mask, u, i, j, k, live, role, lane, 1, part, sE);
+}
+template <int PARTS_A, bool SIDES>
+__global__ void __launch_bounds__(192, L1M_WAVES) k_l1_pair_rows_zs(Dims d, const double *__restrict__ tab, const double *__restrict__ E, double *u,
+                                                                    const double *__restrict__ b, const uint8_t *__restrict__ mask, int cx, int cy,
+                                                                    int nseg) {
+    static_assert(!(PARTS_A & 8), "the A nodes of a forward sweep have no relaxed z neighbour");
+    __shared__ double part[2][3][64];
+    __shared__ double sE[4][16][64];
+    const int lane = threadIdx.x, role = __builtin_amdgcn_readfirstlane(threadIdx.y);
+    const int i = 2 * blockIdx.z + cx, j = 2 * blockIdx.y + cy;
+#pragma unroll 1
+    for (int s = 0; s < 2 * nseg; ++s) {
+        const int k = 2 + 128 * (s >> 1) + 2 * lane - (s & 1);
+        const bool live = k >= 0 && k < d.NZ;
+        if (s & 1) node_group<0, PARTS_A | 8, SIDES>(d, tab, E, u, b, mask, u, i, j, live ? k : 0, live, role, lane, 1, part, sE);
+        else       node_group<0, PARTS_A, SIDES>(d, tab, E, u, b, mask, u, i, j, live ? k : 0, live, role, lane, 1, part, sE);
+        __builtin_amdgcn_fence(__ATOMIC_RELEASE, "workgroup");
+        __syncthreads();
+        __builtin_amdgcn_fence(__ATOMIC_ACQUIRE, "workgroup");
+    }
+}
+
+bool zero_start_parts(int lni, int &parts, bool &sides) {
+    const unsigned blocks = gs_zero_start_blocks(lni);
+    auto has = [&](int ox, int oy, int oz) { return (blocks >> (9 * (ox + 1) + 3 * (oy + 1) + (oz + 1))) & 1u; };
+    parts = (int) (has(0, -1, -1) | has(0, -1, 0) << 1 | has(0, 0, 0) << 2 | has(0, 0, -1) << 3);
+    sides = has(-1, 0, 0) != 0;
+    unsigned whole = 0;
+    for (int nb = 0; nb < 27; ++nb) {
+        const int oy = (nb / 3) % 3 - 1, oz = nb % 3 - 1;
+        const int part = oy && oz ? 0 : oy ? 1 : oz ? 3 : 2;
+        if (nb / 9 != 1 ? sides : (parts >> part) & 1) whole |= 1u << nb;
+    }
+    return whole == blocks && (parts & 4);
+}
+
+template <int... P, class F>
+bool with_zero_start_parts(int parts, bool sides, F &&f) {
+    auto pick = [&](auto p) {
+        if (sides) f(p, std::integral_constant<bool, true>{}); else f(p, std::integral_constant<bool, false>{});
+        return true;
+    };
+    return ((parts == P && pick(std::integral_constant<int, P>{})) || ...);
+}
+
 }
 
 void build_l1_merged_table(const double *cK0_0, double *tab ) { l1m::build_table(cK0_0, tab); }
@@ -232,7 +302,18 @@
 }
 
 void launch_l1_merged_sweep(const Dims &d, const double *tab, const double *E, double *u, const double *b, const uint8_t *mask,
-                            int forward, int xparity, int first, int count, hipStream_t s, int pair) {
+                            int forward, int xparity, int first, int count, hipStream_t s, int pair, bool from_zero) {
+    const dim3 blk(64, 3, 1);
+    auto colour = [&](const dim3 &grd, int lni, int cx, int cy, int cz, int ka, int kskip) {
+        int parts = 15;
+        bool sides = true;
+        if (from_zero && zero_start_parts(lni, parts, sides) &&
+            with_zero_start_parts<4, 12, 7, 15>(parts, sides, [&](auto P, auto S) {
+                if constexpr (decltype(P)::value == 15 && decltype(S)::value) k_l1_merged<0><<<grd, blk, 0, s>>>(d, tab, E, u, b, mask, u, cx, cy, cz, forward, ka, kskip);
+                else k_l1_merged_zs<decltype(P)::value, decltype(S)::value><<<grd, blk, 0, s>>>(d, tab, E, u, b, mask, cx, cy, cz, ka, kskip);
+            })) return;
+        k_l1_merged<0><<<grd, blk, 0, s>>>(d, tab, E, u, b, mask, u, cx, cy, cz, forward, ka, kskip);
+    };
     for (int ci = first; ci < first + count; ++ci) {
         const int lni = forward ? ci : 7 - ci;
         const int cx = ((lni >> 2) & 1) ^ (xparity & 1), cy = (lni >> 1) & 1, cz = lni & 1;
@@ -241,16 +322,23 @@
         const int fz = cz, ka = fz == 0 ? 1 : 0, nseg = (cntz - ka) / 64;
         if (pair && ci % 2 == 0 && ci + 1 < first + count && nseg >= 1) {
             const int walked = 64 * nseg, cntb = (d.NZ - 1 - (1 - fz)) / 2 + 1;
-            if (cntz > walked)
-                k_l1_merged<0><<<dim3((cnty * (cntz - walked) + 63) / 64, 1, cntx), dim3(64, 3, 1), 0, s>>>(d, tab, E, u, b, mask, u, cx, cy, fz, forward, ka, walked);
-            if (fz == 0) k_l1_pair_rows<0><<<dim3(1, cnty, cntx), dim3(64, 3, 1), 0, s>>>(d, tab, E, u, b, mask, cx, cy, nseg);
-            else         k_l1_pair_rows<1><<<dim3(1, cnty, cntx), dim3(64, 3, 1), 0, s>>>(d, tab, E, u, b, mask, cx, cy, nseg);
-            if (cntb > walked)
-                k_l1_merged<0><<<dim3((cnty * (cntb - walked) + 63) / 64, 1, cntx), dim3(64, 3, 1), 0, s>>>(d, tab, E, u, b, mask, u, cx, cy, 1 - fz, forward, 0, walked);
+            const int lnb = forward ? ci + 1 : 7 - (ci + 1);
+            if (cntz > walked) colour(dim3((cnty * (cntz - walked) + 63) / 64, 1, cntx), lni, cx, cy, fz, ka, walked);
+            const dim3 rows(1, cnty, cntx);
+            int pa = 15, pb = 15;
+            bool sa = true, sb = true;
+            if (!(from_zero && fz == 0 && zero_start_parts(lni, pa, sa) && zero_start_parts(lnb, pb, sb) && sa == sb && pb == (pa | 8) && !(pa & 8) &&
+                  with_zero_start_parts<4, 7>(pa, sa, [&](auto P, auto S) {
+                      k_l1_pair_rows_zs<decltype(P)::value, decltype(S)::value><<<rows, blk, 0, s>>>(d, tab, E, u, b, mask, cx, cy, nseg);
+                  }))) {
+                if (fz == 0) k_l1_pair_rows<0><<<rows, blk, 0, s>>>(d, tab, E, u, b, mask, cx, cy, nseg);
+                else         k_l1_pair_rows<1><<<rows, blk, 0, s>>>(d, tab, E, u, b, mask, cx, cy, nseg);
+            }
+            if (cntb > walked) colour(dim3((cnty * (cntb - walked) + 63) / 64, 1, cntx), lnb, cx, cy, 1 - fz, 0, walked);
             ++ci;
             continue;
         }
-        k_l1_merged<0><<<dim3((cnty * cntz + 63) / 64, 1, cntx), dim3(64, 3, 1), 0, s>>>(d, tab, E, u, b, mask, u, cx, cy, cz, forward, 0, 0);
+        colour(dim3((cnty * cntz + 63) / 64, 1, cntx), lni, cx, cy, cz, 0, 0);
     }
     VFEM_HIP(hipGetLastError());
 }
diff --git a/ndr_amd/csrc/kernels_mg.hip b/ndr_amd/csrc/kernels_mg.hip
--- a/ndr_amd/csrc/kernels_mg.hip
+++ b/ndr_amd/csrc/kernels_mg.hip
@@ -1,6 +1,7 @@
 #include "vfem_internal.h"
 #include "device_utils.h"
 #include "gs_coef.h"
+#include "gs_colors.h"
 
 
 #include <algorithm>
@@ -785,36 +786,44 @@
     for (int c = 0; c < 3; ++c) u[3 * n + c] = uself[c] + ud[c];
 }
 
-template <int W>
+template <int W, bool PRUNE = false>
 __device__ __forceinline__ void stencil_plane(const Dims &d, const double *__restrict__ St, const double *__restrict__ u, int i, int j, int k,
-                                              long long sbase, long long scnt, double S[3], double M[9], double uself[3]) {
+                                              long long sbase, long long scnt, double S[3], double M[9], double uself[3], unsigned blocks = 0x1ffu) {
     static_for<9>([&](auto tc) {
         constexpr int nb = 9 * W + decltype(tc)::value, di = W - 1, dj = (nb / 3) % 3 - 1, dk = nb % 3 - 1;
-        int ii = i + di, jj = j + dj, kk = k + dk;
-        if (di < 0) ii = ii < 0 ? 0 : ii;
-        if (di > 0) ii = ii > d.NX - 1 ? d.NX - 1 : ii;
-        if (dj < 0) jj = jj < 0 ? 0 : jj;
-        if (dj > 0) jj = jj > d.NY - 1 ? d.NY - 1 : jj;
-        if (dk < 0) kk = kk < 0 ? 0 : kk;
-        if (dk > 0) kk = kk > d.NZ - 1 ? d.NZ - 1 : kk;
-        const long long m = nidx(d, ii, jj, kk);
-        const double u0 = u[3 * m], u1 = u[3 * m + 1], u2 = u[3 * m + 2];
-        const double *a = St + sbase + (long long) nb * 9 * scnt;
-        double A[9];
-#pragma unroll
-        for (int q = 0; q < 9; ++q) A[q] = a[(long long) q * scnt];
-#pragma unroll
-        for (int r = 0; r < 3; ++r) S[r] += A[3 * r] * u0 + A[3 * r + 1] * u1 + A[3 * r + 2] * u2;
-        if (nb == 13) {
-#pragma unroll
-            for (int q = 0; q < 9; ++q) M[q] = A[q];
-            uself[0] = u0; uself[1] = u1; uself[2] = u2;
+        if (PRUNE && !((blocks >> decltype(tc)::value) & 1u)) return;
+        if constexpr (PRUNE && nb == 13) {
+            const double *a = St + sbase + (long long) nb * 9 * scnt;
+#pragma unroll
+            for (int q = 0; q < 9; ++q) M[q] = a[(long long) q * scnt];
+        } else {
+            int ii = i + di, jj = j + dj, kk = k + dk;
+            if (di < 0) ii = ii < 0 ? 0 : ii;
+            if (di > 0) ii = ii > d.NX - 1 ? d.NX - 1 : ii;
+            if (dj < 0) jj = jj < 0 ? 0 : jj;
+            if (dj > 0) jj = jj > d.NY - 1 ? d.NY - 1 : jj;
+            if (dk < 0) kk = kk < 0 ? 0 : kk;
+            if (dk > 0) kk = kk > d.NZ - 1 ? d.NZ - 1 : kk;
+            const long long m = nidx(d, ii, jj, kk);
+            const double u0 = u[3 * m], u1 = u[3 * m + 1], u2 = u[3 * m + 2];
+            const double *a = St + sbase + (long long) nb * 9 * scnt;
+            double A[9];
+#pragma unroll
+            for (int q = 0; q < 9; ++q) A[q] = a[(long long) q * scnt];
+#pragma unroll
+            for (int r = 0; r < 3; ++r) S[r] += A[3 * r] * u0 + A[3 * r + 1] * u1 + A[3 * r + 2] * u2;
+            if (nb == 13) {
+#pragma unroll
+                for (int q = 0; q < 9; ++q) M[q] = A[q];
+                uself[0] = u0; uself[1] = u1; uself[2] = u2;
+            }
         }
     });
 }
+template <bool ZERO_START>
 __global__ void __launch_bounds__(192) k_gs_color_stencil_split(Dims d, const double *__restrict__ St, double *__restrict__ u,
                                                                 const double *__restrict__ b, const uint8_t *__restrict__ mask,
-                                                                int cx, int cy, int cz, int forward) {
+                                                                int cx, int cy, int cz, int forward, unsigned blocks) {
     __shared__ double part[2][3][64];
     const int lane = threadIdx.x, w = __builtin_amdgcn_readfirstlane(threadIdx.y);
     const int cntx = (d.NX - 1 - cx) / 2 + 1, cnty = (d.NY - 1 - cy) / 2 + 1, cntz = (d.NZ - 1 - cz) / 2 + 1;
@@ -827,9 +836,16 @@
     long long sbase, scnt;
     cm_index(d, i, j, k, sbase, scnt);
     double S[3] = {0.0, 0.0, 0.0}, M[9], uself[3] = {0.0, 0.0, 0.0};
-    if (w == 0) stencil_plane<0>(d, St, u, i, j, k, sbase, scnt, S, M, uself);
-    else if (w == 1) stencil_plane<1>(d, St, u, i, j, k, sbase, scnt, S, M, uself);
-    else stencil_plane<2>(d, St, u, i, j, k, sbase, scnt, S, M, uself);
+    const unsigned pb = ZERO_START ? __builtin_amdgcn_readfirstlane((blocks >> (9 * w)) & 0x1ffu) : 0x1ffu;
+    if (!ZERO_START || pb == 0x1ffu) {
+        if (w == 0) stencil_plane<0>(d, St, u, i, j, k, sbase, scnt, S, M, uself);
+        else if (w == 1) stencil_plane<1>(d, St, u, i, j, k, sbase, scnt, S, M, uself);
+        else stencil_plane<2>(d, St, u, i, j, k, sbase, scnt, S, M, uself);
+    } else if (pb != 0u) {
+        if (w == 0) stencil_plane<0, true>(d, St, u, i, j, k, sbase, scnt, S, M, uself, pb);
+        else if (w == 1) stencil_plane<1, true>(d, St, u, i, j, k, sbase, scnt, S, M, uself, pb);
+        else stencil_plane<2, true>(d, St, u, i, j, k, sbase, scnt, S, M, uself, pb);
+    }
     if (w != 1) {
 #pragma unroll
         for (int c = 0; c < 3; ++c) part[w >> 1][c][lane] = S[c];
@@ -896,7 +912,7 @@
 }
 
 void launch_gs_sweep_stencil(const Dims &d, const double *S, double *u, const double *b, const uint8_t *mask,
-                             int forward, int xparity, int first, int count, hipStream_t s, const double *Sn, int stencil_split) {
+                             int forward, int xparity, int first, int count, hipStream_t s, const double *Sn, int stencil_split, bool from_zero) {
     for (int ci = first; ci < first + count; ++ci) {
         const int lni = forward ? ci : 7 - ci;
         const int cx = ((lni >> 2) & 1) ^ (xparity & 1), cy = (lni >> 1) & 1, cz = lni & 1;
@@ -905,7 +921,11 @@
         const long long cnt = (long long) cntx * cnty * cntz;
         dim3 blk(64, 4, 1), grd((unsigned) ((cnt + 255) / 256), 1, 1);
         if (Sn) k_gs_color_stencil_wave<<<dim3((unsigned) ((cntz + 3) / 4), (unsigned) cnty, (unsigned) cntx), blk, 0, s>>>(d, Sn, u, b, mask, cx, cy, cz, forward);
-        else if (stencil_split && cnt < (1LL << 31)) k_gs_color_stencil_split<<<dim3((unsigned) ((cnt + 63) / 64)), dim3(64, 3, 1), 0, s>>>(d, S, u, b, mask, cx, cy, cz, forward);
+        else if (stencil_split && cnt < (1LL << 31)) {
+            const dim3 g3((unsigned) ((cnt + 63) / 64)), b3(64, 3, 1);
+            if (from_zero) k_gs_color_stencil_split<true><<<g3, b3, 0, s>>>(d, S, u, b, mask, cx, cy, cz, forward, gs_zero_start_blocks(lni));
+            else k_gs_color_stencil_split<false><<<g3, b3, 0, s>>>(d, S, u, b, mask, cx, cy, cz, forward, GS_ALL_BLOCKS);
+        }
         else k_gs_color_stencil<<<grd, blk, 0, s>>>(d, S, u, b, mask, cx, cy, cz, forward);
     }
     VFEM_HIP(hipGetLastError());
diff --git a/ndr_amd/csrc/mg.hip b/ndr_amd/csrc/mg.hip
--- a/ndr_amd/csrc/mg.hip
+++ b/ndr_amd/csrc/mg.hip
@@ -95,12 +95,13 @@
     else launch_apply_gather(L.d, L.kind, level_K(mg, l), level_E(mg, l), u, b, L.maskp, res, out, s);
 }
 
-void vfem::mg_smooth(vfem_mg *mg, int l, double *u, const double *b, int forward, hipStream_t s, int first, int count) {
+void vfem::mg_smooth(vfem_mg *mg, int l, double *u, const double *b, int forward, hipStream_t s, int first, int count, bool from_zero) {
     MgLevel &L = mg->lv[l];
+    if (from_zero && !(forward && first == 0 && count == 8)) throw Error("a sweep from a zero iterate is a whole forward sweep");
     if (level_uses_half_stencil(mg, l)) launch_gs_sweep_stencil_half(L.d, L.Sh.p, u, b, L.maskp, forward, L.xparity, first, count, s);
-    else if (level_uses_stencil(mg, l)) launch_gs_sweep_stencil(L.d, L.S.p, u, b, L.maskp, forward, L.xparity, first, count, s, L.Sn.p, mg->fine->tune.stencil_split);
+    else if (level_uses_stencil(mg, l)) launch_gs_sweep_stencil(L.d, L.S.p, u, b, L.maskp, forward, L.xparity, first, count, s, L.Sn.p, mg->fine->tune.stencil_split, from_zero);
     else if (level_uses_merged_rows(mg, l)) launch_l1_merged_sweep(L.d, mg->l1mtab.p, level_E(mg, l), u, b, L.maskp, forward, L.xparity, first, count, s,
-                                                                   mg->fine->tune.l1_merged == 2);
+                                                                   mg->fine->tune.l1_merged == 2, from_zero && mg->fine->tune.l1_merged == 2);
     else launch_gs_sweep_mf(L.d, L.kind, level_K(mg, l), l == 0 ? mg->fine->dGsTab.p : mg->mf1diag.p, level_E(mg, l), u, b, L.maskp,
                             forward, L.xparity, first, count, s, mg->fine->tune, mg->mf1_sym,
                             (l == 1 && mg->fine->tune.l1_diag) ? L.Mdiag.p : nullptr);
@@ -130,12 +131,13 @@
     L.gs_sd_version = sim->operator_version;
 }
 
-static void mg_smooth_n(vfem_mg *mg, int l, double *u, const double *b, int forward, int n, hipStream_t s) {
+static void mg_smooth_n(vfem_mg *mg, int l, double *u, const double *b, int forward, int n, hipStream_t s, bool from_zero = false) {
     MgLevel &L = mg->lv[l];
     const vfem_sim *sim = mg->fine;
     const Tuning &t = sim->tune;
     if (!(level0_marches(mg, l) && n > 0)) {
-        for (int i = 0; i < n; ++i) mg_smooth(mg, l, u, b, forward, s);
+        const bool prune_first = from_zero && forward && l >= 1 && t.zero_start;
+        for (int i = 0; i < n; ++i) mg_smooth(mg, l, u, b, forward, s, 0, 8, prune_first && i == 0);
         return;
     }
     L.tmp.reserve((size_t) L.d.nn * 3);
@@ -262,7 +264,7 @@
         if (!(dirichlet_zeroed && residual_system))
             launch_enforce_dirichlet(lv(l).d.nn, lv(l).maskp, l == 0 ? mg->fine->dvals.p : nullptr, x(l), residual_system ? 1 : 0, s);
     }
-    void smooth(int l, int forward, int n) { mg_smooth_n(mg, l, x(l), b(l), forward, n, s); }
+    void smooth(int l, int forward, int n, bool from_zero) { mg_smooth_n(mg, l, x(l), b(l), forward, n, s, from_zero); }
     void residual(int l) { mg_apply(mg, l, x(l), b(l), 1, lv(l).r.p, s); }
     void restrict_residual(int l) { launch_restrict(lv(l + 1).d, lv(l).d.NX, lv(l + 1).xshift, lv(l).r.p, b(l + 1), s, x(l + 1)); }
     void restrict_rhs(int l) { launch_restrict(lv(l + 1).d, lv(l).d.NX, lv(l + 1).xshift, b(l), b(l + 1), s); }
@@ -524,6 +526,15 @@
     mg_smooth_n(mg, level, u, b, forward, sweeps, S(stream));
     VFEM_CATCH
 }
+int vfem_mg_smooth_sweeps_from_zero(vfem_mg *mg, int level, double *u_out, const double *b, int sweeps, void *stream) {
+    VFEM_TRY
+    check_level(mg, level);
+    if (sweeps < 0) throw Error("negative sweep count");
+    if (level >= 1) update_operators(mg, S(stream));
+    VFEM_HIP(hipMemsetAsync(u_out, 0, (size_t) mg->lv[(size_t) level].d.nn * 3 * sizeof(double), S(stream)));
+    mg_smooth_n(mg, level, u_out, b, 1, sweeps, S(stream), true);
+    VFEM_CATCH
+}
 int vfem_mg_zero_dirichlet(vfem_mg *mg, int level, double *u, void *stream) {
     VFEM_TRY
     check_level(mg, level);
diff --git a/ndr_amd/csrc/mg_cycle.h b/ndr_amd/csrc/mg_cycle.h
--- a/ndr_amd/csrc/mg_cycle.h
+++ b/ndr_amd/csrc/mg_cycle.h
@@ -8,15 +8,15 @@
 
 struct CgWork { long long n; double *d, *Ad, *sc; hipStream_t s; };
 
-template <class Ops> void vcycle(Ops &o, int l, int nsmooth, bool residual_system, bool dirichlet_zeroed = false) {
+template <class Ops> void vcycle(Ops &o, int l, int nsmooth, bool residual_system, bool dirichlet_zeroed = false, bool zero_start = false) {
     if (l == o.last_level()) { o.last_level_cycle(false); return; }
     o.enforce_dirichlet(l, residual_system, dirichlet_zeroed);
-    o.smooth(l, 1, nsmooth);
+    o.smooth(l, 1, nsmooth, zero_start);
     o.residual(l);
     o.restrict_residual(l);
-    vcycle(o, l + 1, nsmooth, true, true);
+    vcycle(o, l + 1, nsmooth, true, true, true);
     o.prolong_correction(l);
-    o.smooth(l, o.symmetric() ? 0 : 1, nsmooth);
+    o.smooth(l, o.symmetric() ? 0 : 1, nsmooth, false);
 }
 
 template <class Ops> void full_multigrid(Ops &o, int l, int nsmooth, bool residual_system) {
diff --git a/ndr_amd/csrc/mg_slab.hip b/ndr_amd/csrc/mg_slab.hip
--- a/ndr_amd/csrc/mg_slab.hip
+++ b/ndr_amd/csrc/mg_slab.hip
@@ -77,7 +77,7 @@
     double *x(int l) const { return g[l].x; }
     double *b(int l) const { return g[l].b; }
     void enforce_dirichlet(int l, bool, bool) { launch_zero_dirichlet(lv(l).d.nn, lv(l).maskp, x(l), s); }
-    void smooth(int l, int forward, int n) { for (int i = 0; i < n; ++i) smooth(l, x(l), b(l), forward); }
+    void smooth(int l, int forward, int n, bool ) { for (int i = 0; i < n; ++i) smooth(l, x(l), b(l), forward); }
     void residual(int l) { mg_apply(loc, l, x(l), b(l), 1, g[l].r, s); halo(l, g[l].r); }
     void restrict_residual(int l) { launch_restrict(lv(l + 1).d, lv(l).d.NX, lv(l + 1).xshift, g[l].r, b(l + 1), s, x(l + 1)); }
     void restrict_rhs(int l) { halo(l, b(l)); launch_restrict(lv(l + 1).d, lv(l).d.NX, lv(l + 1).xshift, b(l), b(l + 1), s); }
diff --git a/ndr_amd/csrc/sim.hip b/ndr_amd/csrc/sim.hip
--- a/ndr_amd/csrc/sim.hip
+++ b/ndr_amd/csrc/sim.hip
@@ -224,6 +224,7 @@
         case VFEM_OPT_GS_MARCH_CHUNKS: if (value < 0) throw Error("negative chunk count"); t.gs_march_chunks = value; break;
         case VFEM_OPT_L1_STORED:     if (value < 0 || value > 2) throw Error("level-1 storage mode 0..2"); t.l1_stored = value; ++sim->operator_version; break;
         case VFEM_OPT_L1_MERGED:     if (value < 0 || value > 2) throw Error("level-1 row mode 0..2"); t.l1_merged = value; break;
+        case VFEM_OPT_ZERO_START:    t.zero_start = value != 0; break;
         case VFEM_OPT_L1_DIAG:       t.l1_diag = value != 0; ++sim->operator_version; break;
         default: throw Error("unknown simulator option " + std::to_string(key));
     }
diff --git a/ndr_amd/csrc/vfem_host.h b/ndr_amd/csrc/vfem_host.h
--- a/ndr_amd/csrc/vfem_host.h
+++ b/ndr_amd/csrc/vfem_host.h
@@ -32,7 +32,7 @@
                             std::vector<uint8_t> &coarse_mask);
 
 void mg_apply(vfem_mg *mg, int l, const double *u, const double *b, int res, double *out, hipStream_t s);
-void mg_smooth(vfem_mg *mg, int l, double *u, const double *b, int forward, hipStream_t s, int first = 0, int count = 8);
+void mg_smooth(vfem_mg *mg, int l, double *u, const double *b, int forward, hipStream_t s, int first = 0, int count = 8, bool from_zero = false);
 bool mg_smooth_half(vfem_mg *mg, int l, double *u, const double *b, int forward, int half, hipStream_t s, int plane_lo = 0, int plane_hi = -1);
 void update_operators(vfem_mg *mg, hipStream_t s);
 void cycle_from_level(vfem_mg *mg, int l, int nsmooth, bool fmg, hipStream_t s);
diff --git a/ndr_amd/csrc/vfem_internal.h b/ndr_amd/csrc/vfem_internal.h
--- a/ndr_amd/csrc/vfem_internal.h
+++ b/ndr_amd/csrc/vfem_internal.h
@@ -81,6 +81,7 @@
     int gs_march_chunks = 0;
     int l1_stored = 0;
     int l1_merged = 2;
+    int zero_start = 1;
     int l1_diag = 0;
 };
 #ifdef VFEM_ABLATION
@@ -117,12 +118,12 @@
 void build_l1_merged_table(const double *cK0_0, double *tab );
 bool l1_merged_usable(const Dims &d);
 void launch_l1_merged_sweep(const Dims &d, const double *tab, const double *E, double *u, const double *b, const uint8_t *mask,
-                            int forward, int xparity, int first, int count, hipStream_t s, int pair = 1);
+                            int forward, int xparity, int first, int count, hipStream_t s, int pair = 1, bool from_zero = false);
 void launch_l1_merged_apply(const Dims &d, const double *tab, const double *E, const double *u, const double *b, const uint8_t *mask,
                             int res, double *out, hipStream_t s);
 void launch_gs_sweep_stencil(const Dims &d, const double *S, double *u, const double *b, const uint8_t *mask,
                              int forward, int xparity, int first, int count, hipStream_t s, const double *S_node_major = nullptr,
-                             int stencil_split = 1);
+                             int stencil_split = 1, bool from_zero = false);
 long long stencil_half_storage_doubles(const Dims &d);
 void launch_stencil_half_from_mf1(const Dims &d, const double *cK0, const double *Efine, double *Sh, hipStream_t s);
 void launch_gs_sweep_stencil_half(const Dims &d, const double *Sh, double *u, const double *b, const uint8_t *mask,
```

After: 79.68 GVoxel/s. About the same (-0.0%).
